# letitiabanana/PnP-OVSS

Hardware: AMD Instinct MI355X
Metric: images/sec (336^2, drop_iter=4, blur+CRF) (higher is better)
Workload: dtype bf16x3

## Files before the change

### pnp-ovss_amd/csrc/engine.hip

```cpp
#include <hip/hip_runtime.h>

#include <cmath>
#include <cstdarg>
#include <cstring>
#include <map>
#include <memory>
#include <string>
#include <utility>
#include <vector>

#include "../../include/pnp_hip.h"
#include "common.h"
#include "kernels.h"

using namespace pnp;

namespace {

struct Buf {
    void* p = nullptr;
    size_t bytes = 0;
};

struct Weight {
    void* p = nullptr;
    int rows = 0, cols = 0;
    int esz = 0;
    bool pair = false;
    void* hi(int r0 = 0) const { return (char*)p + (size_t)r0 * cols * esz; }
    void* lo(int r0 = 0) const { return pair ? (char*)p + ((size_t)rows + r0) * cols * esz : nullptr; }
};

struct Act {
    void* hi = nullptr;
    void* lo = nullptr;
};

struct TextLayerW {
    Weight qkv_w, so_w, cq_w, co_w, i_w, o_w;
    float *qkv_b = nullptr, *so_b = nullptr, *sln_w = nullptr, *sln_b = nullptr, *cq_b = nullptr, *co_b = nullptr,
          *cln_w = nullptr, *cln_b = nullptr, *i_b = nullptr, *o_b = nullptr, *oln_w = nullptr, *oln_b = nullptr;
    Weight o_wT, i_wT, co_wT, cq_wT, so_wT, qkv_wT;
};

struct TextLayerA {
    void* qkv = nullptr;
    float* Ps = nullptr;
    float *a_hat = nullptr, *a_rstd = nullptr, *a_out = nullptr;
    void* a_outT = nullptr;
    void* qc = nullptr;
    float* Pc = nullptr;
    float *c_hat = nullptr, *c_rstd = nullptr, *c_out = nullptr;
    void* c_outT = nullptr;
    float* u = nullptr;
    float *o_hat = nullptr, *o_rstd = nullptr, *h_out = nullptr;
    void* h_outT = nullptr;
};

struct VitLayerW {
    float *n1w, *n1b, *n2w, *n2b, *qkv_b, *proj_b, *fc1_b, *fc2_b;
    Weight qkv_w, proj_w, fc1_w, fc2_w;
};

struct WeightStore {
    int device = 0;
    std::vector<void*> allocs;
    size_t bytes = 0;
    ~WeightStore() {
        (void)hipSetDevice(device);
        for (void* p : allocs) (void)hipFree(p);
    }
};

}

struct pnp_engine {
    pnp_config c{};
    std::shared_ptr<WeightStore> wstore;
    bool to_store = false;
    bool shares_weights = false;
    int bf = 0;
    int x3 = 0;
    size_t esz = 4;
    int P = 0, PP = 0, N = 0, Npad = 0, D = 0, H = 0, I = 0, TL = 0, nh = 0, Nst = 0, SL = 0;
    char err[512] = {0};
    std::vector<void*> allocs;
    size_t alloc_bytes = 0;
    std::map<std::string, Buf> named;
    std::map<std::string, bool> loaded;
    bool finalized = false;

    float *cls = nullptr, *pos = nullptr, *patch_b = nullptr, *vnorm_w = nullptr, *vnorm_b = nullptr;
    Weight patch_w;
    std::vector<VitLayerW> vit;
    float *word = nullptr, *tpos = nullptr, *eln_w = nullptr, *eln_b = nullptr, *itm_w = nullptr, *itm_b = nullptr;
    std::vector<TextLayerW> txt;
    Weight proj_w[2];
    float* proj_b[2] = {nullptr, nullptr};
    int proj_E[2] = {0, 0};
    Weight ck_w, cv_w;
    float *ck_b = nullptr, *cv_b = nullptr;
    std::vector<Buf> staging;

    int ldq = 0;
    float* x0 = nullptr;
    struct { const float* images = nullptr; const int64_t* ids = nullptr; const int64_t* mask = nullptr; int B = 0, L = 0, ld = 0;
             bool vit = false, text = false; } reuse;
    void *patches = nullptr, *vt = nullptr;
    Act xn, qk, ctx, h1, embT;
    float *x = nullptr, *emb32 = nullptr;
    void *Knat = nullptr, *Vnat = nullptr, *Kt = nullptr, *Vt = nullptr;
    std::vector<TextLayerA> ta;
    float *temb = nullptr, *h0 = nullptr, *tmp = nullptr;
    void *h0T = nullptr, *ctx_s = nullptr, *ctx_c = nullptr, *g = nullptr;
    float *dh = nullptr, *d_pre = nullptr, *dc = nullptr, *d_cpre = nullptr, *da = nullptr, *d_apre = nullptr,
          *dctx_s = nullptr, *dS = nullptr, *dPc = nullptr;
    void *d_preT = nullptr, *dg = nullptr, *d_cpreT = nullptr, *dctxc = nullptr, *dqc = nullptr, *d_apreT = nullptr,
         *dqkv = nullptr;
    int grad_layer = -1;
    bool acts_text_only = false;
    float* G = nullptr;
    uint8_t* dropped = nullptr;
    float* logits_scratch = nullptr;

    struct Post {
        bool reserved = false, prepared = false, has_crf = false;
        int groups_cap = 1;
        int maxB = 0, maxK = 0, max_pix_img = 0, chunk = 0;
        int64_t max_total_pix = 0;
        int B = 0, Cmax = 0, Kmax = 0, maxHW = 0;
        int64_t total_pix = 0;
        std::vector<PostDesc> desc, desc_pair;
        PostDesc* d_desc = nullptr;
        PostDesc* d_desc_pair = nullptr;
        int32_t *d_img_cls_off = nullptr, *d_cls_off = nullptr, *d_tok_idx = nullptr, *d_cls_div = nullptr, *d_lut = nullptr;
        int lut_stride = 0;
        size_t* d_label_off = nullptr;
        double* d_wts = nullptr;
        int32_t* d_wt_off = nullptr;
        float *merged = nullptr, *thr = nullptr, *maps = nullptr, *maps2 = nullptr, *maps3 = nullptr, *stats = nullptr;
        float *unary = nullptr, *Q = nullptr, *va = nullptr, *vb = nullptr, *vga = nullptr, *vgb = nullptr, *norm[2] = {nullptr, nullptr};
        int Kpmax = 0, Kpmax_pair = 0, maxH = 0, maxW = 0, max_radius = 0, maxKp = 0;
        size_t valg_cap = 0;
        std::vector<int> gauss_sig;
        const uint8_t* d_rgb = nullptr;
        const float* d_gt = nullptr;
        CrfLattice lat[2]{};
        uint64_t *keys_a = nullptr, *keys_b = nullptr;
        uint32_t* vals_a = nullptr;
        int *n1k = nullptr, *n2k = nullptr;
        int *head = nullptr, *incl = nullptr, *range_err = nullptr;
        int range_err_host = 0;
        int lat_points[2] = {0, 0};
        std::vector<size_t> h_label_off;
        std::vector<int32_t> h_wt_off;
        std::vector<double> h_wts;
        void* sort_tmp = nullptr;
        size_t sort_tmp_bytes = 0;
        size_t cap[2] = {0, 0};
        size_t val_cap = 0;
        int lut_cap = 0, cls_cap = 0, tok_cap = 0, wts_cap = 0;
        bool maps_in_2 = false;
    } post;

    GemmProfile* gemm_prof = nullptr;
    StreamKWs sk_ws;
    struct StageProfile {
        bool on = false;
        std::vector<hipEvent_t> ev0, ev1;
        int used = 0;
        long long launches = 0;
        double work = 0;
        double lattice = 0;
    } crf_prof;
};

namespace {

int fail(pnp_engine* e, int code, const char* fmt, ...) {
    va_list ap;
    va_start(ap, fmt);
    vsnprintf(e->err, sizeof(e->err), fmt, ap);
    va_end(ap);
    return code;
}

#define HIPCHK(e, call)                                                                      \
    do {                                                                                     \
        hipError_t _s = (call);                                                              \
        if (_s != hipSuccess) return fail(e, PNP_ERR_HIP, "%s: %s", #call, hipGetErrorString(_s)); \
    } while (0)
#define KCHK(e, call)                                                         \
    do {                                                                      \
        int _r = (call);                                                      \
        if (_r != PNP_OK) return fail(e, _r, "%s failed (%d): %s", #call, _r, hipGetErrorString(hipGetLastError())); \
    } while (0)

template <typename T>
int dalloc(pnp_engine* e, T** out, size_t count, bool zero = false) {
    void* p = nullptr;
    const size_t bytes = (count * sizeof(T) + 255) / 256 * 256;
    if (hipMalloc(&p, bytes ? bytes : 256) != hipSuccess) return fail(e, PNP_ERR_NOMEM, "hipMalloc(%zu) failed", bytes);
    if (zero && hipMemset(p, 0, bytes ? bytes : 256) != hipSuccess) return fail(e, PNP_ERR_HIP, "hipMemset failed");
    if (e->to_store && e->wstore) {
        e->wstore->allocs.push_back(p);
        e->wstore->bytes += bytes;
    } else {
        e->allocs.push_back(p);
    }
    e->alloc_bytes += bytes;
    *out = reinterpret_cast<T*>(p);
    return PNP_OK;
}
int dalloc_t(pnp_engine* e, void** out, size_t count, bool zero = false) {
    char* p = nullptr;
    int r = dalloc<char>(e, &p, count * e->esz, zero);
    *out = p;
    return r;
}
int alloc_act(pnp_engine* e, Act* a, size_t rows, size_t ld) {
    KCHK(e, dalloc_t(e, &a->hi, rows * ld));
    a->lo = e->x3 ? (char*)a->hi + rows * ld * 2 : nullptr;
    return PNP_OK;
}
int launched() { return hipPeekAtLastError() == hipSuccess ? PNP_OK : PNP_ERR_HIP; }

bool ends_with(const std::string& s, const char* suf) {
    const size_t n = strlen(suf);
    return s.size() >= n && s.compare(s.size() - n, n, suf) == 0;
}

__global__ void transpose_cast_kernel_f32(const float* __restrict__ in, float* __restrict__ out, int rows, int cols) {
    __shared__ float t[32][33];
    const int bx = blockIdx.x * 32, by = blockIdx.y * 32;
    for (int i = threadIdx.y; i < 32; i += 8) {
        const int r = by + i, c = bx + threadIdx.x;
        t[i][threadIdx.x] = (r < rows && c < cols) ? in[(size_t)r * cols + c] : 0.f;
    }
    __syncthreads();
    for (int i = threadIdx.y; i < 32; i += 8) {
        const int c = bx + i, r = by + threadIdx.x;
        if (r < rows && c < cols) out[(size_t)c * rows + r] = t[threadIdx.x][i];
    }
}

__global__ void feat_to_tok_kernel(const float* __restrict__ src, int ld_src, int n_pad, float* __restrict__ dst, int R, int N) {
    __shared__ float t[32][33];
    const int b = blockIdx.z, r0 = blockIdx.x * 32, t0 = blockIdx.y * 32;
    for (int i = threadIdx.y; i < 32; i += 8) {
        const int r = r0 + i, tok = t0 + threadIdx.x;
        t[i][threadIdx.x] = (r < R && tok < N) ? src[(size_t)r * ld_src + (size_t)b * n_pad + tok] : 0.f;
    }
    __syncthreads();
    for (int i = threadIdx.y; i < 32; i += 8) {
        const int tok = t0 + i, r = r0 + threadIdx.x;
        if (r < R && tok < N) dst[((size_t)b * N + tok) * R + r] = t[threadIdx.x][i];
    }
}
__global__ void tok_to_feat_kernel(const float* __restrict__ src, int ld_src, float* __restrict__ dst, int ld_dst, int n_pad, int R, int N) {
    __shared__ float t[32][33];
    const int b = blockIdx.z, r0 = blockIdx.x * 32, t0 = blockIdx.y * 32;
    for (int i = threadIdx.y; i < 32; i += 8) {
        const int tok = t0 + i, r = r0 + threadIdx.x;
        t[i][threadIdx.x] = (r < R && tok < N) ? src[((size_t)b * N + tok) * ld_src + r] : 0.f;
    }
    __syncthreads();
    for (int i = threadIdx.y; i < 32; i += 8) {
        const int r = r0 + i, tok = t0 + threadIdx.x;
        if (r < R && tok < N) dst[(size_t)r * ld_dst + (size_t)b * n_pad + tok] = t[threadIdx.x][i];
    }
}

__global__ void embed_reuse_kernel(const float* __restrict__ x0, const uint8_t* __restrict__ dropped, const float* __restrict__ bias,
                                   const float* __restrict__ pos, float* __restrict__ x, int rows, int N, int D4) {
    const size_t total = (size_t)rows * D4;
    for (size_t i = (size_t)blockIdx.x * blockDim.x + threadIdx.x; i < total; i += (size_t)gridDim.x * blockDim.x) {
        const int m = (int)(i / D4), c = (int)(i - (size_t)m * D4);
        const int b = m / N, t = m - b * N;
        f32x4 v;
        if (t > 0 && dropped[(size_t)b * (N - 1) + (t - 1)]) {
            const f32x4 bv = reinterpret_cast<const f32x4*>(bias)[c];
            const f32x4 pv = reinterpret_cast<const f32x4*>(pos)[(size_t)t * D4 + c];
#pragma unroll
            for (int e = 0; e < 4; e++) v[e] = __fadd_rn(__fadd_rn(0.0f, bv[e]), pv[e]);
        } else {
            v = reinterpret_cast<const f32x4*>(x0)[i];
        }
        reinterpret_cast<f32x4*>(x)[i] = v;
    }
}

int new_weight(pnp_engine* e, int rows, int cols, bool pair, Weight* w) {
    *w = Weight{nullptr, rows, cols, pair ? 2 : (int)e->esz, pair};
    return dalloc_t(e, &w->p, (size_t)rows * cols);
}
int fill_weight(pnp_engine* e, const float* src32, const Weight& w, int r0, int n) {
    const size_t count = (size_t)n * w.cols;
    return w.pair ? split_f32(src32, w.hi(r0), w.lo(r0), count, 0) : cast_f32(e->bf, src32, w.hi(r0), count, 0);
}
int make_weight(pnp_engine* e, const float* src32, int rows, int cols, bool transpose, Weight* out, bool pair = false) {
    KCHK(e, new_weight(e, transpose ? cols : rows, transpose ? rows : cols, pair, out));
    const float* s = src32;
    float* tmp = nullptr;
    if (transpose) {
        HIPCHK(e, hipMalloc((void**)&tmp, (size_t)rows * cols * 4));
        hipLaunchKernelGGL(transpose_cast_kernel_f32, dim3((cols + 31) / 32, (rows + 31) / 32), dim3(32, 8), 0, 0, src32, tmp,
                           rows, cols);
        s = tmp;
    }
    int r = transpose ? launched() : PNP_OK;
    if (r == PNP_OK) r = fill_weight(e, s, *out, 0, out->rows);
    hipError_t st = hipDeviceSynchronize();
    if (tmp) (void)hipFree(tmp);
    if (r != PNP_OK || st != hipSuccess) return fail(e, PNP_ERR_HIP, "weight conversion failed");
    return PNP_OK;
}

GemmArgs G_(const void* A, int lda, const void* B, int ldb, int M, int N, int K) {
    GemmArgs g;
    g.A = A; g.lda = lda; g.B = B; g.ldb = ldb; g.M = M; g.N = N; g.K = K;
    return g;
}

GemmArgs linear(const void* a, int lda, const Weight& w, int M, int r0 = 0, int n = 0) {
    GemmArgs g = G_(a, lda, w.hi(r0), w.cols, M, n ? n : w.rows, w.cols);
    g.B_lo = w.lo(r0);
    g.a_f32 = w.pair;
    return g;
}
GemmArgs linear(const Act& a, int lda, const Weight& w, int M, int r0 = 0, int n = 0) {
    GemmArgs g = linear(a.hi, lda, w, M, r0, n);
    g.A_lo = a.lo;
    g.a_f32 = w.pair && !a.lo;
    return g;
}
GemmArgs linear_t(const Act& a, int lda, const Weight& w, int M, int r0 = 0, int n = 0) {
    GemmArgs g = linear(a, lda, w, M, r0, n);
    std::swap(g.A, g.B); std::swap(g.A_lo, g.B_lo); std::swap(g.lda, g.ldb); std::swap(g.M, g.N);
    return g;
}

int egemm(pnp_engine* e, GemmArgs g, hipStream_t s) {
    g.prof = e->gemm_prof;
    g.sk = e->sk_ws.part ? &e->sk_ws : nullptr;
    return gemm_nt(e->bf, g, s);
}

}


extern "C" size_t pnp_workspace_bytes(const pnp_config* c) {
    if (!c) return 0;
    const size_t es = c->compute_bf16 == 1 ? 2 : 4;
    const size_t P = c->img_size / c->patch, N = P * P + 1, Npad = (N + 63) / 64 * 64, D = c->vit_dim, H = c->txt_hidden,
                 I = c->txt_inter, TL = c->txt_layers, B = c->max_batch, L = c->max_text_len;
    const size_t M = B * N, R = B * L;
    size_t w = (size_t)c->vit_depth * (12 * D * D) * es + TL * (4 * H * H + 2 * H * D + 2 * H * I) * es * 2 +
               ((size_t)c->vocab + c->max_pos) * H * 4 + 256 * (D + H) * es + 2 * 256 * 4;
    size_t a = M * (768 + D * 2 + 3 * D + 64 + D + 4 * D) * es + M * D * 12 + D * B * Npad * es + M * TL * H * es * 2 +
               2 * TL * H * B * Npad * es;
    size_t t = TL * (R * (3 * H + 2 * H) * es + R * (H * 8 + I) * 4 + B * (H / 64) * L * (L + Npad) * 4) + R * I * (4 + es) * 2 +
               R * H * 64;
    return w + a + t + (64u << 20);
}

extern "C" const char* pnp_last_error(const pnp_engine* e) { return e ? e->err : "null engine"; }

extern "C" void pnp_destroy(pnp_engine* e) {
    if (!e) return;
    (void)hipSetDevice(e->c.device);
    (void)hipDeviceSynchronize();
    for (void* p : e->allocs) (void)hipFree(p);
    for (auto& b : e->staging) if (b.p) (void)hipFree(b.p);
    if (e->gemm_prof) {
        for (int i = 0; i < e->gemm_prof->created; i++) {
            (void)hipEventDestroy(e->gemm_prof->ev0[i]);
            (void)hipEventDestroy(e->gemm_prof->ev1[i]);
        }
        delete e->gemm_prof;
    }
    for (hipEvent_t ev : e->crf_prof.ev0) (void)hipEventDestroy(ev);
    for (hipEvent_t ev : e->crf_prof.ev1) (void)hipEventDestroy(ev);
    streamk_ws_destroy(&e->sk_ws);
    delete e;
}

static int create_impl(const pnp_config* cfg, pnp_engine* donor, pnp_engine** out) {
    if (!cfg || !out) return PNP_ERR_ARG;
    pnp_engine* e = new pnp_engine();
    *out = e;
    e->c = *cfg;
    if (donor) {
        const pnp_config& d = donor->c;
        if (!donor->finalized) return fail(e, PNP_ERR_STATE, "pnp_create_shared: the donor's weights are not finalized");
        if (d.device != cfg->device || d.compute_bf16 != cfg->compute_bf16 || d.img_size != cfg->img_size || d.patch != cfg->patch ||
            d.vit_dim != cfg->vit_dim || d.vit_depth != cfg->vit_depth || d.vit_heads != cfg->vit_heads ||
            d.vit_mlp_ratio != cfg->vit_mlp_ratio || d.txt_hidden != cfg->txt_hidden || d.txt_layers != cfg->txt_layers ||
            d.txt_heads != cfg->txt_heads || d.txt_inter != cfg->txt_inter || d.vocab != cfg->vocab || d.max_pos != cfg->max_pos ||
            d.vit_ln_eps != cfg->vit_ln_eps || d.txt_ln_eps != cfg->txt_ln_eps)
            return fail(e, PNP_ERR_ARG, "pnp_create_shared: device, compute mode and model geometry must equal the donor's");
        if (cfg->stash_layer < d.stash_layer)
            return fail(e, PNP_ERR_ARG, "pnp_create_shared: stash_layer %d below the donor's %d (its transposed backward weights "
                        "exist for layers >= %d only)", cfg->stash_layer, d.stash_layer, d.stash_layer);
    }
    const pnp_config& c = e->c;
    if (c.compute_bf16 < 0 || c.compute_bf16 > 2) return fail(e, PNP_ERR_ARG, "compute_bf16 must be 0 (fp32), 1 (bf16) or 2 (split-bf16)");
    e->bf = c.compute_bf16 == 1 ? 1 : 0;
    e->x3 = c.compute_bf16 == 2 ? 1 : 0;
    e->esz = e->bf ? 2 : 4;
    if (c.patch != 16) return fail(e, PNP_ERR_ARG, "patch must be 16");
    if (c.img_size % 16 || c.img_size <= 0) return fail(e, PNP_ERR_ARG, "img_size must be a positive multiple of 16");
    if (c.vit_dim != c.vit_heads * 64 || c.txt_hidden != c.txt_heads * 64)
        return fail(e, PNP_ERR_ARG, "head_dim must be 64 (vit_dim=%d heads=%d, txt_hidden=%d heads=%d)", c.vit_dim,
                    c.vit_heads, c.txt_hidden, c.txt_heads);
    if (c.vit_dim % 128 || c.txt_hidden % 128 || c.txt_inter % 128 || (c.vit_dim * c.vit_mlp_ratio) % 128)
        return fail(e, PNP_ERR_ARG, "widths must be multiples of 128");
    if (c.vit_dim > 1024 || c.txt_hidden > 1024) return fail(e, PNP_ERR_ARG, "LayerNorm width > 1024 unsupported");
    if (c.max_text_len < 5 || c.max_text_len > 512 || c.max_text_len > c.max_pos)
        return fail(e, PNP_ERR_ARG, "max_text_len must be in [5, min(512, max_pos = %d)]", c.max_pos);
    if (c.stash_layer < 0 || c.stash_layer >= c.txt_layers) return fail(e, PNP_ERR_ARG, "stash_layer out of range");
    if (c.max_batch <= 0) return fail(e, PNP_ERR_ARG, "max_batch must be positive");
    HIPCHK(e, hipSetDevice(c.device));
    e->P = c.img_size / 16;
    e->PP = e->P * e->P;
    e->N = e->PP + 1;
    e->Npad = (e->N + 63) / 64 * 64;
    e->Nst = e->Npad;
    e->D = c.vit_dim;
    e->H = c.txt_hidden;
    e->I = c.txt_inter;
    e->TL = c.txt_layers;
    e->nh = c.txt_heads;
    e->SL = c.stash_layer;
    if ((e->N + 15) / 16 > 160) return fail(e, PNP_ERR_ARG, "too many image tokens (%d) for the cross-attention kernel", e->N);
    const size_t B = c.max_batch, M = B * e->N, D = e->D, H = e->H, I = e->I, L = c.max_text_len, R = B * L, TL = e->TL;
    const size_t ldv = B * e->Npad;
    e->vit.resize(c.vit_depth);
    e->txt.resize(TL);
    e->ta.resize(TL);
    if (e->x3) {
        const int n_cu = device_cu_count();
        if (!n_cu || streamk_ws_create(&e->sk_ws, n_cu) != PNP_OK) return fail(e, PNP_ERR_HIP, "stream-K workspace allocation failed");
        e->alloc_bytes += (size_t)n_cu * 256 * 256 * 4;
    }
    KCHK(e, dalloc_t(e, &e->patches, B * e->PP * 768));
    KCHK(e, dalloc(e, &e->x, M * D));
    KCHK(e, dalloc(e, &e->x0, M * D));
    KCHK(e, alloc_act(e, &e->xn, M, D));
    e->ldq = 3 * (int)D + 64;
    KCHK(e, alloc_act(e, &e->qk, M, e->ldq));
    KCHK(e, dalloc_t(e, &e->vt, D * ldv, true));
    KCHK(e, alloc_act(e, &e->ctx, M, D));
    KCHK(e, alloc_act(e, &e->h1, M, D * c.vit_mlp_ratio));
    KCHK(e, alloc_act(e, &e->embT, M, D));
    KCHK(e, dalloc(e, &e->emb32, M * D));
    const int nVn = e->TL - e->SL, nKt = e->TL - e->SL - 1;
    KCHK(e, dalloc_t(e, &e->Knat, M * TL * H));
    KCHK(e, dalloc_t(e, &e->Vnat, M * (size_t)nVn * H));
    KCHK(e, dalloc_t(e, &e->Vt, TL * H * ldv, true));
    if (nKt > 0) KCHK(e, dalloc_t(e, &e->Kt, (size_t)nKt * H * ldv, true));
    KCHK(e, dalloc(e, &e->temb, R * H));
    KCHK(e, dalloc(e, &e->h0, R * H));
    KCHK(e, dalloc_t(e, &e->h0T, R * H));
    KCHK(e, dalloc(e, &e->tmp, R * H));
    KCHK(e, dalloc_t(e, &e->ctx_s, R * H));
    KCHK(e, dalloc_t(e, &e->ctx_c, R * H));
    KCHK(e, dalloc_t(e, &e->g, R * I));
    for (size_t i = 0; i < TL; i++) {
        TextLayerA& a = e->ta[i];
        KCHK(e, dalloc_t(e, &a.qkv, R * 3 * H));
        KCHK(e, dalloc(e, &a.a_hat, R * H));
        KCHK(e, dalloc(e, &a.a_rstd, R));
        KCHK(e, dalloc(e, &a.a_out, R * H));
        KCHK(e, dalloc_t(e, &a.a_outT, R * H));
        KCHK(e, dalloc_t(e, &a.qc, R * H));
        KCHK(e, dalloc(e, &a.c_hat, R * H));
        KCHK(e, dalloc(e, &a.c_rstd, R));
        KCHK(e, dalloc(e, &a.c_out, R * H));
        KCHK(e, dalloc_t(e, &a.c_outT, R * H));
        KCHK(e, dalloc(e, &a.u, R * I));
        KCHK(e, dalloc(e, &a.o_hat, R * H));
        KCHK(e, dalloc(e, &a.o_rstd, R));
        KCHK(e, dalloc(e, &a.h_out, R * H));
        KCHK(e, dalloc_t(e, &a.h_outT, R * H));
        if ((int)i >= e->SL) {
            KCHK(e, dalloc(e, &a.Ps, B * e->nh * L * L));
            KCHK(e, dalloc(e, &a.Pc, B * e->nh * L * (size_t)e->Nst, true));
        }
    }
    KCHK(e, dalloc(e, &e->dh, R * H));
    KCHK(e, dalloc(e, &e->d_pre, R * H));
    KCHK(e, dalloc_t(e, &e->d_preT, R * H));
    KCHK(e, dalloc_t(e, &e->dg, R * I));
    KCHK(e, dalloc(e, &e->dc, R * H));
    KCHK(e, dalloc(e, &e->d_cpre, R * H));
    KCHK(e, dalloc_t(e, &e->d_cpreT, R * H));
    KCHK(e, dalloc_t(e, &e->dctxc, R * H));
    KCHK(e, dalloc_t(e, &e->dqc, R * H));
    KCHK(e, dalloc(e, &e->da, R * H));
    KCHK(e, dalloc(e, &e->d_apre, R * H));
    KCHK(e, dalloc_t(e, &e->d_apreT, R * H));
    KCHK(e, dalloc(e, &e->dctx_s, R * H));
    KCHK(e, dalloc(e, &e->dS, B * e->nh * L * L));
    KCHK(e, dalloc(e, &e->dPc, B * e->nh * L * (size_t)e->Nst, true));
    KCHK(e, dalloc_t(e, &e->dqkv, R * 3 * H));
    KCHK(e, dalloc(e, &e->G, B * L * (size_t)e->PP));
    KCHK(e, dalloc(e, &e->dropped, B * (size_t)e->PP, true));
    KCHK(e, dalloc(e, &e->logits_scratch, B * 2));
    if (donor) {
        e->wstore = donor->wstore;
        e->shares_weights = true;
        e->cls = donor->cls; e->pos = donor->pos; e->patch_b = donor->patch_b; e->vnorm_w = donor->vnorm_w; e->vnorm_b = donor->vnorm_b;
        e->word = donor->word; e->tpos = donor->tpos; e->eln_w = donor->eln_w; e->eln_b = donor->eln_b;
        e->itm_w = donor->itm_w; e->itm_b = donor->itm_b; e->ck_b = donor->ck_b; e->cv_b = donor->cv_b;
        e->patch_w = donor->patch_w; e->ck_w = donor->ck_w; e->cv_w = donor->cv_w;
        e->vit = donor->vit;
        e->txt = donor->txt;
        for (int i = 0; i < 2; i++) { e->proj_w[i] = donor->proj_w[i]; e->proj_b[i] = donor->proj_b[i]; e->proj_E[i] = donor->proj_E[i]; }
        e->finalized = true;
        return PNP_OK;
    }
    e->wstore = std::make_shared<WeightStore>();
    e->wstore->device = c.device;
    e->to_store = true;
    KCHK(e, dalloc(e, &e->cls, D));
    KCHK(e, dalloc(e, &e->pos, (size_t)e->N * D));
    KCHK(e, dalloc(e, &e->patch_b, D));
    KCHK(e, dalloc(e, &e->vnorm_w, D));
    KCHK(e, dalloc(e, &e->vnorm_b, D));
    KCHK(e, dalloc(e, &e->word, (size_t)c.vocab * H));
    KCHK(e, dalloc(e, &e->tpos, (size_t)c.max_pos * H));
    KCHK(e, dalloc(e, &e->eln_w, H));
    KCHK(e, dalloc(e, &e->eln_b, H));
    KCHK(e, dalloc(e, &e->itm_w, 2 * H));
    KCHK(e, dalloc(e, &e->itm_b, 2));
    KCHK(e, dalloc(e, &e->ck_b, TL * H));
    KCHK(e, dalloc(e, &e->cv_b, TL * H));
    for (auto& v : e->vit) {
        KCHK(e, dalloc(e, &v.n1w, D)); KCHK(e, dalloc(e, &v.n1b, D)); KCHK(e, dalloc(e, &v.n2w, D)); KCHK(e, dalloc(e, &v.n2b, D));
        KCHK(e, dalloc(e, &v.qkv_b, 3 * D)); KCHK(e, dalloc(e, &v.proj_b, D));
        KCHK(e, dalloc(e, &v.fc1_b, D * c.vit_mlp_ratio)); KCHK(e, dalloc(e, &v.fc2_b, D));
    }
    for (auto& t : e->txt) {
        KCHK(e, dalloc(e, &t.qkv_b, 3 * H)); KCHK(e, dalloc(e, &t.so_b, H)); KCHK(e, dalloc(e, &t.sln_w, H)); KCHK(e, dalloc(e, &t.sln_b, H));
        KCHK(e, dalloc(e, &t.cq_b, H)); KCHK(e, dalloc(e, &t.co_b, H)); KCHK(e, dalloc(e, &t.cln_w, H)); KCHK(e, dalloc(e, &t.cln_b, H));
        KCHK(e, dalloc(e, &t.i_b, I)); KCHK(e, dalloc(e, &t.o_b, H)); KCHK(e, dalloc(e, &t.oln_w, H)); KCHK(e, dalloc(e, &t.oln_b, H));
    }
    e->to_store = false;
    return PNP_OK;
}
extern "C" int pnp_create(const pnp_config* cfg, pnp_engine** out) { return create_impl(cfg, nullptr, out); }
extern "C" int pnp_create_shared(const pnp_config* cfg, pnp_engine* donor, pnp_engine** out) {
    if (!donor) return PNP_ERR_ARG;
    return create_impl(cfg, donor, out);
}


namespace {

struct Key {
    const char* name = "";
    float* small = nullptr;
    size_t small_off = 0;
    int rows = 1, cols = 0;
    int id = 0;
};
Key small(const char* name, float* p, int count, size_t off = 0) { return {name, p, off, 1, count, 0}; }
Key gemm(const char* name, int id, int rows, int cols) { return {name, nullptr, 0, rows, cols, id}; }

enum { W_PATCH };
enum { W_QKV, W_PROJ, W_FC1, W_FC2 };
enum { W_Q, W_K, W_V, W_SO, W_CQ, W_CK, W_CV, W_CO, W_I, W_O, W_MAX };

std::vector<Key> top_keys(pnp_engine* e) {
    const int D = e->D, H = e->H;
    return {small("visual_encoder.cls_token", e->cls, D),
            small("visual_encoder.pos_embed", e->pos, e->N * D),
            gemm("visual_encoder.patch_embed.proj.weight", W_PATCH, D, 768),
            small("visual_encoder.patch_embed.proj.bias", e->patch_b, D),
            small("visual_encoder.norm.weight", e->vnorm_w, D),
            small("visual_encoder.norm.bias", e->vnorm_b, D),
            small("text_encoder.embeddings.word_embeddings.weight", e->word, e->c.vocab * H),
            small("text_encoder.embeddings.position_embeddings.weight", e->tpos, e->c.max_pos * H),
            small("text_encoder.embeddings.LayerNorm.weight", e->eln_w, H),
            small("text_encoder.embeddings.LayerNorm.bias", e->eln_b, H),
            small("itm_head.weight", e->itm_w, 2 * H),
            small("itm_head.bias", e->itm_b, 2)};
}
const char* const kVitPrefix = "visual_encoder.blocks.";
std::vector<Key> vit_keys(pnp_engine* e, int li) {
    VitLayerW& v = e->vit[li];
    const int D = e->D, F = D * e->c.vit_mlp_ratio;
    return {small("norm1.weight", v.n1w, D),       small("norm1.bias", v.n1b, D),
            gemm("attn.qkv.weight", W_QKV, 3 * D, D),   small("attn.qkv.bias", v.qkv_b, 3 * D),
            gemm("attn.proj.weight", W_PROJ, D, D),     small("attn.proj.bias", v.proj_b, D),
            small("norm2.weight", v.n2w, D),       small("norm2.bias", v.n2b, D),
            gemm("mlp.fc1.weight", W_FC1, F, D),        small("mlp.fc1.bias", v.fc1_b, F),
            gemm("mlp.fc2.weight", W_FC2, D, F),        small("mlp.fc2.bias", v.fc2_b, D)};
}
const char* const kTextPrefix = "text_encoder.encoder.layer.";
std::vector<Key> text_keys(pnp_engine* e, int li) {
    TextLayerW& t = e->txt[li];
    const int D = e->D, H = e->H, I = e->I;
    const size_t l = (size_t)li * H;
    return {gemm("attention.self.query.weight", W_Q, H, H),            small("attention.self.query.bias", t.qkv_b, H, 0),
            gemm("attention.self.key.weight", W_K, H, H),              small("attention.self.key.bias", t.qkv_b, H, H),
            gemm("attention.self.value.weight", W_V, H, H),            small("attention.self.value.bias", t.qkv_b, H, 2 * H),
            gemm("attention.output.dense.weight", W_SO, H, H),         small("attention.output.dense.bias", t.so_b, H),
            small("attention.output.LayerNorm.weight", t.sln_w, H),    small("attention.output.LayerNorm.bias", t.sln_b, H),
            gemm("crossattention.self.query.weight", W_CQ, H, H),      small("crossattention.self.query.bias", t.cq_b, H),
            gemm("crossattention.self.key.weight", W_CK, H, D),        small("crossattention.self.key.bias", e->ck_b, H, l),
            gemm("crossattention.self.value.weight", W_CV, H, D),      small("crossattention.self.value.bias", e->cv_b, H, l),
            gemm("crossattention.output.dense.weight", W_CO, H, H),    small("crossattention.output.dense.bias", t.co_b, H),
            small("crossattention.output.LayerNorm.weight", t.cln_w, H), small("crossattention.output.LayerNorm.bias", t.cln_b, H),
            gemm("intermediate.dense.weight", W_I, I, H),              small("intermediate.dense.bias", t.i_b, I),
            gemm("output.dense.weight", W_O, H, I),                    small("output.dense.bias", t.o_b, H),
            small("output.LayerNorm.weight", t.oln_w, H),              small("output.LayerNorm.bias", t.oln_b, H)};
}

bool find_key(const std::vector<Key>& keys, const char* name, Key& out) {
    for (const Key& k : keys)
        if (!strcmp(k.name, name)) {
            out = k;
            return true;
        }
    return false;
}

bool resolve(pnp_engine* e, const std::string& n, Key& s) {
    int li = -1;
    char rest[128];
    auto layer_of = [&](const char* prefix, int depth) {
        const size_t len = strlen(prefix);
        return n.compare(0, len, prefix) == 0 && sscanf(n.c_str() + len, "%d.%127s", &li, rest) == 2 && li >= 0 && li < depth;
    };
    if (layer_of(kVitPrefix, e->c.vit_depth)) return find_key(vit_keys(e, li), rest, s);
    if (layer_of(kTextPrefix, e->TL)) return find_key(text_keys(e, li), rest, s);
    return find_key(top_keys(e), n.c_str(), s);
}

const char* const kProj[2] = {"vision_proj", "text_proj"};
int resolve_proj(pnp_engine* e, const std::string& n, const int64_t* shape, int ndim, Key& s) {
    int which = -1;
    bool bias = false;
    for (int i = 0; i < 2; i++) {
        if (n == std::string(kProj[i]) + ".weight") which = i;
        if (n == std::string(kProj[i]) + ".bias") which = i, bias = true;
    }
    if (which < 0) return 0;
    const int K = which == 0 ? e->D : e->H;
    if (ndim != (bias ? 1 : 2) || (!bias && shape[1] != K))
        return fail(e, PNP_ERR_ARG, "%s: expected %s, second dimension %d", n.c_str(), bias ? "a vector" : "a matrix", K);
    const int64_t E = shape[0];
    if (E <= 0 || E > 1024 || E % 64) return fail(e, PNP_ERR_ARG, "%s: embedding width %lld must be a multiple of 64 up to 1024", n.c_str(), (long long)E);
    if (e->proj_E[which] && e->proj_E[which] != (int)E)
        return fail(e, PNP_ERR_ARG, "%s: %lld rows, but the other tensor of this projection has %d", n.c_str(), (long long)E, e->proj_E[which]);
    e->proj_E[which] = (int)E;
    s.rows = (int)E;
    s.cols = bias ? 1 : K;
    return 1;
}

const float* staged(pnp_engine* e, const std::string& n) {
    auto it = e->named.find("stage:" + n);
    return it == e->named.end() ? nullptr : (const float*)it->second.p;
}

int collect(pnp_engine* e, const std::string& prefix, const std::vector<Key>& keys, const float** st) {
    for (const Key& k : keys) {
        const std::string n = prefix + k.name;
        if (k.small ? !e->loaded.count(n) : !(st[k.id] = staged(e, n))) return fail(e, PNP_ERR_STATE, "missing weight %s", n.c_str());
    }
    return PNP_OK;
}

}

extern "C" int pnp_load_weight(pnp_engine* e, const char* name, const float* data, const int64_t* shape, int32_t ndim,
                               int32_t on_device) {
    if (!e || !name || !data || !shape) return PNP_ERR_ARG;
    if (e->shares_weights) return fail(e, PNP_ERR_STATE, "this engine uses a donor's weights (pnp_create_shared)");
    if (e->finalized) return fail(e, PNP_ERR_STATE, "weights already finalized");
    HIPCHK(e, hipSetDevice(e->c.device));
    Key s;
    const int pj = resolve_proj(e, name, shape, ndim, s);
    if (pj < 0) return pj;
    if (!pj && !resolve(e, name, s)) return PNP_OK;
    size_t count = 1;
    for (int i = 0; i < ndim; i++) count *= (size_t)shape[i];
    if (count != (size_t)s.rows * s.cols) return fail(e, PNP_ERR_ARG, "%s: expected %d elements, got %zu", name, s.rows * s.cols, count);
    const hipMemcpyKind kind = on_device ? hipMemcpyDeviceToDevice : hipMemcpyHostToDevice;
    if (s.small) {
        HIPCHK(e, hipMemcpy(s.small + s.small_off, data, count * 4, kind));
    } else {
        Buf b;
        b.bytes = count * 4;
        HIPCHK(e, hipMalloc(&b.p, b.bytes));
        HIPCHK(e, hipMemcpy(b.p, data, b.bytes, kind));
        e->staging.push_back(b);
        e->named[std::string("stage:") + name] = b;
    }
    e->loaded[name] = true;
    return PNP_OK;
}

extern "C" int pnp_finalize_weights(pnp_engine* e) {
    if (!e) return PNP_ERR_ARG;
    if (e->finalized) return PNP_OK;
    HIPCHK(e, hipSetDevice(e->c.device));
    e->to_store = true;
    struct StoreOff { pnp_engine* e; ~StoreOff() { e->to_store = false; } } store_off{e};
    const int D = e->D, H = e->H, I = e->I, TL = e->TL, F = D * e->c.vit_mlp_ratio;
    const float* st[W_MAX];
    if (int r = collect(e, "", top_keys(e), st)) return r;
    KCHK(e, make_weight(e, st[W_PATCH], D, 768, false, &e->patch_w));
    for (int i = 0; i < e->c.vit_depth; i++) {
        VitLayerW& v = e->vit[i];
        if (int r = collect(e, kVitPrefix + std::to_string(i) + ".", vit_keys(e, i), st)) return r;
        KCHK(e, make_weight(e, st[W_QKV], 3 * D, D, false, &v.qkv_w, e->x3));
        KCHK(e, make_weight(e, st[W_PROJ], D, D, false, &v.proj_w, e->x3));
        KCHK(e, make_weight(e, st[W_FC1], F, D, false, &v.fc1_w, e->x3));
        KCHK(e, make_weight(e, st[W_FC2], D, F, false, &v.fc2_w, e->x3));
    }
    KCHK(e, new_weight(e, TL * H, D, e->x3, &e->ck_w));
    KCHK(e, new_weight(e, TL * H, D, e->x3, &e->cv_w));
    for (int i = 0; i < TL; i++) {
        TextLayerW& t = e->txt[i];
        if (int r = collect(e, kTextPrefix + std::to_string(i) + ".", text_keys(e, i), st)) return r;
        float* fused = nullptr;
        HIPCHK(e, hipMalloc((void**)&fused, (size_t)3 * H * H * 4));
        HIPCHK(e, hipMemcpy(fused, st[W_Q], (size_t)H * H * 4, hipMemcpyDeviceToDevice));
        HIPCHK(e, hipMemcpy(fused + (size_t)H * H, st[W_K], (size_t)H * H * 4, hipMemcpyDeviceToDevice));
        HIPCHK(e, hipMemcpy(fused + (size_t)2 * H * H, st[W_V], (size_t)H * H * 4, hipMemcpyDeviceToDevice));
        int r = make_weight(e, fused, 3 * H, H, false, &t.qkv_w, e->x3);
        if (r == PNP_OK && i > e->SL) r = make_weight(e, fused, 3 * H, H, true, &t.qkv_wT, e->x3);
        (void)hipFree(fused);
        if (r != PNP_OK) return r;
        KCHK(e, make_weight(e, st[W_SO], H, H, false, &t.so_w, e->x3));
        KCHK(e, make_weight(e, st[W_CQ], H, H, false, &t.cq_w, e->x3));
        KCHK(e, make_weight(e, st[W_CO], H, H, false, &t.co_w, e->x3));
        KCHK(e, make_weight(e, st[W_I], I, H, false, &t.i_w, e->x3));
        KCHK(e, make_weight(e, st[W_O], H, I, false, &t.o_w, e->x3));
        KCHK(e, fill_weight(e, st[W_CK], e->ck_w, i * H, H));
        KCHK(e, fill_weight(e, st[W_CV], e->cv_w, i * H, H));
        if (i >= e->SL) {
            KCHK(e, make_weight(e, st[W_O], H, I, true, &t.o_wT, e->x3));
            KCHK(e, make_weight(e, st[W_I], I, H, true, &t.i_wT, e->x3));
            KCHK(e, make_weight(e, st[W_CO], H, H, true, &t.co_wT, e->x3));
        }
        if (i > e->SL) {
            KCHK(e, make_weight(e, st[W_CQ], H, H, true, &t.cq_wT, e->x3));
            KCHK(e, make_weight(e, st[W_SO], H, H, true, &t.so_wT, e->x3));
        }
    }
    for (int i = 0; i < 2; i++) {
        const float *w = staged(e, std::string(kProj[i]) + ".weight"), *bs = staged(e, std::string(kProj[i]) + ".bias");
        if (!w || !bs) {
            e->proj_E[i] = 0;
            continue;
        }
        KCHK(e, make_weight(e, w, e->proj_E[i], i == 0 ? D : H, false, &e->proj_w[i], e->x3));
        KCHK(e, dalloc(e, &e->proj_b[i], (size_t)e->proj_E[i]));
        HIPCHK(e, hipMemcpy(e->proj_b[i], bs, (size_t)e->proj_E[i] * 4, hipMemcpyDeviceToDevice));
    }
    HIPCHK(e, hipDeviceSynchronize());
    for (auto& b : e->staging) if (b.p) (void)hipFree(b.p);
    e->staging.clear();
    for (auto it = e->named.begin(); it != e->named.end();) {
        if (it->first.rfind("stage:", 0) == 0) it = e->named.erase(it);
        else ++it;
    }
    e->finalized = true;
    return PNP_OK;
}


static int vit_forward_impl(pnp_engine* e, const float* d_images, const uint8_t* d_dropped, int32_t B, void* stream, int embed) {
    if (!e || !d_images) return PNP_ERR_ARG;
    if (!e->finalized) return fail(e, PNP_ERR_STATE, "weights not finalized");
    if (B <= 0 || B > e->c.max_batch) return fail(e, PNP_ERR_ARG, "batch %d out of range (max %d)", B, e->c.max_batch);
    hipStream_t s = (hipStream_t)stream;
    const int D = e->D, N = e->N, M = B * N, F = D * e->c.vit_mlp_ratio, bf = e->bf;
    const int ldv = e->c.max_batch * e->Npad;
    if (embed == 2 && !(e->reuse.vit && e->reuse.images == d_images && e->reuse.B == B)) embed = 0;
    if (embed == 2 && d_dropped) {
        hipLaunchKernelGGL(embed_reuse_kernel, dim3(2048), dim3(256), 0, s, (const float*)e->x0, d_dropped, (const float*)e->patch_b,
                           (const float*)e->pos, e->x, M, N, D / 4);
        KCHK(e, launched());
    } else {
        KCHK(e, patchify(bf, d_images, d_dropped, e->patches, B, e->c.img_size, e->P, s));
        KCHK(e, cls_rows(e->cls, e->pos, e->x, B, N, D, s));
        {
            GemmArgs g = linear(e->patches, 768, e->patch_w, B * e->PP);
            g.bias = e->patch_b; g.resid = e->pos; g.ldr = D; g.out_f32 = e->x; g.ldo = D; g.row_div = e->PP;
            KCHK(e, egemm(e, g, s));
        }
        if (embed == 1) {
            HIPCHK(e, hipMemcpyAsync(e->x0, e->x, (size_t)M * D * sizeof(float), hipMemcpyDeviceToDevice, s));
            e->reuse.images = d_images;
            e->reuse.B = B;
            e->reuse.vit = true;
        }
    }
    const float scale = 1.0f / sqrtf(64.f);
    const int ln = bf | e->x3;
    for (int l = 0; l < e->c.vit_depth; l++) {
        const VitLayerW& w = e->vit[l];
        KCHK(e, layernorm(ln, e->x, w.n1w, w.n1b, e->c.vit_ln_eps, M, D, nullptr, e->xn.hi, nullptr, nullptr, s, e->xn.lo));
        if (bf || e->x3) {
            GemmArgs g = linear(e->xn, D, w.qkv_w, M);
            g.bias = w.qkv_b; g.out_t = e->qk.hi; g.out_lo = e->qk.lo; g.ldo_t = e->ldq;
            KCHK(e, egemm(e, g, s));
            if (e->x3)
                KCHK(e, vit_attention_x3(e->qk.hi, e->qk.lo, e->ldq, D, e->ctx.hi, e->ctx.lo, B, e->c.vit_heads, N, scale, s));
            else
                KCHK(e, vit_attention(bf, e->qk.hi, e->ldq, D, (const char*)e->qk.hi + (size_t)2 * D * e->esz, e->ldq, e->Npad, e->ctx.hi,
                                      B, e->c.vit_heads, N, scale, s));
        } else {
            {
                GemmArgs g = linear(e->xn, D, w.qkv_w, M, 0, 2 * D);
                g.bias = w.qkv_b; g.out_t = e->qk.hi; g.ldo_t = 2 * D;
                KCHK(e, egemm(e, g, s));
            }
            {
                GemmArgs g = linear_t(e->xn, D, w.qkv_w, M, 2 * D, D);
                g.bias = w.qkv_b + 2 * D; g.bias_on_rows = 1; g.out_t = e->vt; g.ldo_t = ldv; g.col_div = N; g.col_pad = e->Npad;
                KCHK(e, egemm(e, g, s));
            }
            KCHK(e, vit_attention(bf, e->qk.hi, 2 * D, D, e->vt, ldv, e->Npad, e->ctx.hi, B, e->c.vit_heads, N, scale, s));
        }
        {
            GemmArgs g = linear(e->ctx, D, w.proj_w, M);
            g.bias = w.proj_b; g.resid = e->x; g.ldr = D; g.out_f32 = e->x; g.ldo = D;
            KCHK(e, egemm(e, g, s));
        }
        KCHK(e, layernorm(ln, e->x, w.n2w, w.n2b, e->c.vit_ln_eps, M, D, nullptr, e->xn.hi, nullptr, nullptr, s, e->xn.lo));
        {
            GemmArgs g = linear(e->xn, D, w.fc1_w, M);
            g.bias = w.fc1_b; g.mode = GEMM_EPI_GELU; g.out_t = e->h1.hi; g.out_lo = e->h1.lo; g.ldo_t = F;
            KCHK(e, egemm(e, g, s));
        }
        {
            GemmArgs g = linear(e->h1, F, w.fc2_w, M);
            g.bias = w.fc2_b; g.resid = e->x; g.ldr = D; g.out_f32 = e->x; g.ldo = D;
            KCHK(e, egemm(e, g, s));
        }
    }
    KCHK(e, layernorm(ln, e->x, e->vnorm_w, e->vnorm_b, e->c.vit_ln_eps, M, D, e->emb32, e->embT.hi, nullptr, nullptr, s, e->embT.lo));
    return pnp_cross_kv(e, B, stream);
}
extern "C" int pnp_vit_forward(pnp_engine* e, const float* d_images, const uint8_t* d_dropped, int32_t B, void* stream) {
    if (e) e->reuse.vit = false;
    return vit_forward_impl(e, d_images, d_dropped, B, stream, 0);
}

extern "C" int pnp_cross_kv(pnp_engine* e, int32_t B, void* stream) {
    if (!e) return PNP_ERR_ARG;
    if (!e->finalized) return fail(e, PNP_ERR_STATE, "weights not finalized");
    if (B <= 0 || B > e->c.max_batch) return fail(e, PNP_ERR_ARG, "batch %d out of range (max %d)", B, e->c.max_batch);
    hipStream_t s = (hipStream_t)stream;
    const int D = e->D, N = e->N, M = B * N;
    const int ldv = e->c.max_batch * e->Npad;
    const int H = e->H, TL = e->TL, SL = e->SL, nVn = TL - SL, nKt = TL - SL - 1;
    auto out = [&](GemmArgs& g, void* p, int ld) {
        if (e->x3) { g.out_f32 = (float*)p; g.ldo = ld; }
        else { g.out_t = p; g.ldo_t = ld; }
    };
    {
        GemmArgs g = linear(e->embT, D, e->ck_w, M);
        g.bias = e->ck_b; out(g, e->Knat, TL * H);
        KCHK(e, egemm(e, g, s));
    }
    {
        GemmArgs g = linear_t(e->embT, D, e->cv_w, M);
        g.bias = e->cv_b; g.bias_on_rows = 1; out(g, e->Vt, ldv); g.col_div = N; g.col_pad = e->Npad;
        KCHK(e, egemm(e, g, s));
    }
    if (e->x3) {
        hipLaunchKernelGGL(feat_to_tok_kernel, dim3((nVn * H + 31) / 32, (N + 31) / 32, B), dim3(32, 8), 0, s,
                           (const float*)e->Vt + (size_t)SL * H * ldv, ldv, e->Npad, (float*)e->Vnat, nVn * H, N);
        KCHK(e, launched());
        if (nKt > 0) {
            hipLaunchKernelGGL(tok_to_feat_kernel, dim3((nKt * H + 31) / 32, (N + 31) / 32, B), dim3(32, 8), 0, s,
                               (const float*)e->Knat + (size_t)(SL + 1) * H, TL * H, (float*)e->Kt, ldv, e->Npad, nKt * H, N);
            KCHK(e, launched());
        }
        return PNP_OK;
    }
    {
        GemmArgs g = linear(e->embT, D, e->cv_w, M, SL * H, nVn * H);
        g.bias = e->cv_b + (size_t)SL * H; g.out_t = e->Vnat; g.ldo_t = nVn * H;
        KCHK(e, egemm(e, g, s));
    }
    if (nKt > 0) {
        GemmArgs g = linear_t(e->embT, D, e->ck_w, M, (SL + 1) * H, nKt * H);
        g.bias = e->ck_b + (size_t)(SL + 1) * H; g.bias_on_rows = 1; g.out_t = e->Kt; g.ldo_t = ldv; g.col_div = N; g.col_pad = e->Npad;
        KCHK(e, egemm(e, g, s));
    }
    return PNP_OK;
}

static int text_layer(pnp_engine* e, int i, const int64_t* d_mask, int32_t ld, int32_t B, int32_t L, bool cross, bool self_in_place,
                      hipStream_t s) {
    const int H = e->H, I = e->I, TL = e->TL, R = B * L, bf = e->bf, N = e->N;
    const int ldv = e->c.max_batch * e->Npad;
    const TextLayerW& w = e->txt[i];
    TextLayerA& a = e->ta[i];
    const float* h = i ? e->ta[i - 1].h_out : e->h0;
    const void* hT = i ? e->ta[i - 1].h_outT : e->h0T;
    const bool keep_p = cross && i >= e->SL;
    auto keep = [&](float* p) -> float* { return cross ? p : nullptr; };
    if (!self_in_place) {
        {
            GemmArgs g = linear(hT, H, w.qkv_w, R);
            g.bias = w.qkv_b; g.out_t = a.qkv; g.ldo_t = 3 * H;
            KCHK(e, egemm(e, g, s));
        }
        KCHK(e, text_self_attn(bf, a.qkv, d_mask, ld, e->ctx_s, keep_p ? a.Ps : nullptr, e->dS, B, L, H, s));
        {
            GemmArgs g = linear(e->ctx_s, H, w.so_w, R);
            g.bias = w.so_b; g.resid = h; g.ldr = H; g.out_f32 = e->tmp; g.ldo = H;
            KCHK(e, egemm(e, g, s));
        }
        KCHK(e, layernorm(bf, e->tmp, w.sln_w, w.sln_b, e->c.txt_ln_eps, R, H, a.a_out, a.a_outT, keep(a.a_hat), keep(a.a_rstd), s));
    }
    const float* f = a.a_out;
    const void* fT = a.a_outT;
    if (cross) {
        {
            GemmArgs g = linear(a.a_outT, H, w.cq_w, R);
            g.bias = w.cq_b; g.out_t = a.qc; g.ldo_t = H;
            KCHK(e, egemm(e, g, s));
        }
        KCHK(e, xattn(bf, 0, (const char*)e->Knat + (size_t)i * H * e->esz, TL * H,
                      (const char*)e->Vt + (size_t)i * H * ldv * e->esz, ldv, e->Npad, a.qc, H, e->ctx_c, H,
                      keep_p ? a.Pc : nullptr, e->Nst, B, L, N, e->nh, s));
        {
            GemmArgs g = linear(e->ctx_c, H, w.co_w, R);
            g.bias = w.co_b; g.resid = a.a_out; g.ldr = H; g.out_f32 = e->tmp; g.ldo = H;
            KCHK(e, egemm(e, g, s));
        }
        KCHK(e, layernorm(bf, e->tmp, w.cln_w, w.cln_b, e->c.txt_ln_eps, R, H, a.c_out, a.c_outT, a.c_hat, a.c_rstd, s));
        f = a.c_out;
        fT = a.c_outT;
    }
    {
        GemmArgs g = linear(fT, H, w.i_w, R);
        g.bias = w.i_b; g.mode = GEMM_EPI_GELU; g.out_t = e->g; g.ldo_t = I;
        if (cross) { g.aux = a.u; g.ld_aux = I; }
        KCHK(e, egemm(e, g, s));
    }
    {
        GemmArgs g = linear(e->g, I, w.o_w, R);
        g.bias = w.o_b; g.resid = f; g.ldr = H; g.out_f32 = e->tmp; g.ldo = H;
        KCHK(e, egemm(e, g, s));
    }
    KCHK(e, layernorm(bf, e->tmp, w.oln_w, w.oln_b, e->c.txt_ln_eps, R, H, a.h_out, a.h_outT, keep(a.o_hat), keep(a.o_rstd), s));
    return PNP_OK;
}

static int text_forward_impl(pnp_engine* e, const int64_t* d_ids, const int64_t* d_mask, int32_t ld, int32_t B, int32_t L,
                             float* d_logits, void* stream, bool reuse_prefix) {
    if (!e || !d_ids || !d_mask) return PNP_ERR_ARG;
    if (!e->finalized) return fail(e, PNP_ERR_STATE, "weights not finalized");
    if (B <= 0 || B > e->c.max_batch || L < 5 || L > e->c.max_text_len || ld < L)
        return fail(e, PNP_ERR_ARG, "text batch %d x %d (ld %d) out of range (max %d x %d)", B, L, ld, e->c.max_batch, e->c.max_text_len);
    hipStream_t s = (hipStream_t)stream;
    const int H = e->H, TL = e->TL, R = B * L;
    e->acts_text_only = false;
    if (reuse_prefix && !(e->reuse.text && e->reuse.ids == d_ids && e->reuse.mask == d_mask && e->reuse.B == B && e->reuse.L == L &&
                          e->reuse.ld == ld))
        reuse_prefix = false;
    if (!reuse_prefix) {
        KCHK(e, text_embed(d_ids, ld, e->word, e->tpos, e->temb, B, L, H, e->c.enc_token_id, e->c.vocab, s));
        KCHK(e, layernorm(e->bf, e->temb, e->eln_w, e->eln_b, e->c.txt_ln_eps, R, H, e->h0, e->h0T, nullptr, nullptr, s));
    }
    for (int i = 0; i < TL; i++) {
        int r = text_layer(e, i, d_mask, ld, B, L, true, reuse_prefix && i == 0, s);
        if (r) return r;
    }
    KCHK(e, itm_head(e->ta[TL - 1].h_out, e->itm_w, e->itm_b, d_logits ? d_logits : e->logits_scratch, B, L, H, s));
    return PNP_OK;
}
extern "C" int pnp_text_forward_xattn(pnp_engine* e, const int64_t* d_ids, const int64_t* d_mask, int32_t ld, int32_t B,
                                      int32_t L, float* d_logits, void* stream) {
    if (e) e->reuse.text = false;
    return text_forward_impl(e, d_ids, d_mask, ld, B, L, d_logits, stream, false);
}

extern "C" int pnp_text_forward_text(pnp_engine* e, const int64_t* d_ids, const int64_t* d_mask, int32_t ld, int32_t T, int32_t L,
                                     float* d_hidden, void* stream) {
    if (!e || !d_ids || !d_mask) return PNP_ERR_ARG;
    if (T <= 0 || L < 2 || L > e->c.max_text_len || ld < L)
        return fail(e, PNP_ERR_ARG, "text batch %d x %d (ld %d) out of range (2 <= L <= %d, T > 0)", T, L, ld, e->c.max_text_len);
    if (!e->finalized) return fail(e, PNP_ERR_STATE, "weights not finalized");
    hipStream_t s = (hipStream_t)stream;
    const int H = e->H, TL = e->TL;
    e->reuse.text = false;
    e->grad_layer = -1;
    e->acts_text_only = true;
    for (int t0 = 0; t0 < T; t0 += e->c.max_batch) {
        const int B = T - t0 < e->c.max_batch ? T - t0 : e->c.max_batch, R = B * L;
        const int64_t* ids = d_ids + (size_t)t0 * ld;
        const int64_t* mask = d_mask + (size_t)t0 * ld;
        KCHK(e, text_embed(ids, ld, e->word, e->tpos, e->temb, B, L, H, -1, e->c.vocab, s));
        KCHK(e, layernorm(e->bf, e->temb, e->eln_w, e->eln_b, e->c.txt_ln_eps, R, H, e->h0, e->h0T, nullptr, nullptr, s));
        for (int i = 0; i < TL; i++) {
            int r = text_layer(e, i, mask, ld, B, L, false, false, s);
            if (r) return r;
        }
        if (d_hidden)
            HIPCHK(e, hipMemcpyAsync(d_hidden + (size_t)t0 * L * H, e->ta[TL - 1].h_out, (size_t)R * H * sizeof(float),
                                     hipMemcpyDeviceToDevice, s));
    }
    return PNP_OK;
}

extern "C" int pnp_project_normalize(pnp_engine* e, int32_t which, const float* d_x, int64_t row_stride, int32_t rows, float* d_out,
                                     void* stream) {
    if (!e || !d_x || !d_out) return PNP_ERR_ARG;
    if (which < 0 || which > 1) return fail(e, PNP_ERR_ARG, "which = %d: 0 (vision_proj) or 1 (text_proj)", which);
    if (rows <= 0) return fail(e, PNP_ERR_ARG, "rows = %d", rows);
    const int K = which == 0 ? e->D : e->H;
    if (row_stride < K || row_stride % 4 || row_stride > (int64_t)1 << 30)
        return fail(e, PNP_ERR_ARG, "row_stride %lld: a multiple of 4 elements, at least %d", (long long)row_stride, K);
    if ((int64_t)rows * row_stride * 4 >= (int64_t)1 << 32)
        return fail(e, PNP_ERR_ARG, "rows %d x row_stride %lld: the input must span less than 4 GiB", rows, (long long)row_stride);
    if (!e->finalized) return fail(e, PNP_ERR_STATE, "weights not finalized");
    const Weight& w = e->proj_w[which];
    if (!w.p || !e->proj_b[which])
        return fail(e, PNP_ERR_STATE, "missing weight %s.weight (the state dict held no %s.weight / .bias)", kProj[which], kProj[which]);
    hipStream_t s = (hipStream_t)stream;
    const int E = e->proj_E[which];
    if (e->bf) {
        size_t cap = (size_t)e->c.max_batch * e->N * e->D / K;
        cap = cap < 16384 ? cap : 16384;
        for (size_t r0 = 0; r0 < (size_t)rows; r0 += cap) {
            const int n = (int)((size_t)rows - r0 < cap ? (size_t)rows - r0 : cap);
            KCHK(e, cast_rows_bf16(d_x + r0 * row_stride, (int)row_stride, e->xn.hi, n, K, s));
            GemmArgs g = linear(e->xn.hi, K, w, n);
            g.bias = e->proj_b[which]; g.out_f32 = d_out + r0 * E; g.ldo = E;
            KCHK(e, egemm(e, g, s));
        }
    } else {
        GemmArgs g = linear(d_x, (int)row_stride, w, rows);
        g.bias = e->proj_b[which]; g.out_f32 = d_out; g.ldo = E;
        KCHK(e, egemm(e, g, s));
    }
    KCHK(e, l2_normalize_rows(d_out, rows, E, 1e-12f, s));
    return PNP_OK;
}

extern "C" int pnp_itc_similarity(const float* d_img_feat, const float* d_txt_feat, int32_t B, int32_t T, int32_t E, float* d_sim,
                                  void* stream) {
    if (!d_img_feat || !d_txt_feat || !d_sim || B <= 0 || T <= 0 || E <= 0 || E % 4) return PNP_ERR_ARG;
    return itc_similarity(d_img_feat, d_txt_feat, d_sim, B, T, E, (hipStream_t)stream);
}

extern "C" int pnp_xattn_grad(pnp_engine* e, int32_t B, int32_t L, void* stream) {
    return pnp_xattn_grad_layer(e, B, L, e ? e->SL : 0, stream);
}

extern "C" int pnp_xattn_grad_layer(pnp_engine* e, int32_t B, int32_t L, int32_t layer, void* stream) {
    if (!e) return PNP_ERR_ARG;
    if (!e->finalized) return fail(e, PNP_ERR_STATE, "weights not finalized");
    if (B <= 0 || B > e->c.max_batch || L < 5 || L > e->c.max_text_len) return fail(e, PNP_ERR_ARG, "bad B/L");
    if (layer < e->SL || layer >= e->TL)
        return fail(e, PNP_ERR_ARG, "layer %d: cross-attention maps are kept for text layers %d..%d (stash_layer)", layer, e->SL, e->TL - 1);
    if (e->acts_text_only)
        return fail(e, PNP_ERR_STATE, "the text activations in place are those of pnp_text_forward_text: run pnp_text_forward_xattn first");
    hipStream_t s = (hipStream_t)stream;
    const int H = e->H, I = e->I, TL = e->TL, R = B * L, bf = e->bf, N = e->N, SL = e->SL;
    const int ldv = e->c.max_batch * e->Npad, nVn = TL - SL;
    e->grad_layer = layer;
    KCHK(e, itm_grad_seed(e->itm_w, e->dh, B, L, H, s));
    for (int i = TL - 1; i >= layer; i--) {
        const TextLayerW& w = e->txt[i];
        TextLayerA& a = e->ta[i];
        KCHK(e, layernorm_bwd(bf, e->dh, w.oln_w, a.o_hat, a.o_rstd, R, H, e->d_pre, e->d_preT, s));
        {
            GemmArgs g = linear(e->d_preT, H, w.o_wT, R);
            g.mode = GEMM_EPI_GELU_GRAD; g.aux = a.u; g.ld_aux = I; g.out_t = e->dg; g.ldo_t = I;
            KCHK(e, egemm(e, g, s));
        }
        {
            GemmArgs g = linear(e->dg, I, w.i_wT, R);
            g.resid = e->d_pre; g.ldr = H; g.out_f32 = e->dc; g.ldo = H;
            KCHK(e, egemm(e, g, s));
        }
        KCHK(e, layernorm_bwd(bf, e->dc, w.cln_w, a.c_hat, a.c_rstd, R, H, e->d_cpre, e->d_cpreT, s));
        {
            GemmArgs g = linear(e->d_cpreT, H, w.co_wT, R);
            g.out_t = e->dctxc; g.ldo_t = H;
            KCHK(e, egemm(e, g, s));
        }
        const char* vnat = (const char*)e->Vnat + (size_t)(i - SL) * H * e->esz;
        if (i == layer) {
            KCHK(e, xattn(bf, 2, vnat, nVn * H, nullptr, 0, e->Npad, e->dctxc, H, nullptr, 0, e->dPc, e->Nst, B, L, N, e->nh, s));
            break;
        }
        KCHK(e, xattn(bf, 1, vnat, nVn * H, (const char*)e->Kt + (size_t)(i - SL - 1) * H * ldv * e->esz, ldv, e->Npad,
                      e->dctxc, H, e->dqc, H, a.Pc, e->Nst, B, L, N, e->nh, s));
        {
            GemmArgs g = linear(e->dqc, H, w.cq_wT, R);
            g.resid = e->d_cpre; g.ldr = H; g.out_f32 = e->da; g.ldo = H;
            KCHK(e, egemm(e, g, s));
        }
        KCHK(e, layernorm_bwd(bf, e->da, w.sln_w, a.a_hat, a.a_rstd, R, H, e->d_apre, e->d_apreT, s));
        {
            GemmArgs g = linear(e->d_apreT, H, w.so_wT, R);
            g.out_f32 = e->dctx_s; g.ldo = H;
            KCHK(e, egemm(e, g, s));
        }
        KCHK(e, text_self_attn_bwd(bf, a.qkv, e->dctx_s, a.Ps, e->dS, e->dqkv, B, L, H, s));
        {
            GemmArgs g = linear(e->dqkv, 3 * H, w.qkv_wT, R);
            g.resid = e->d_apre; g.ldr = H; g.out_f32 = e->dh; g.ldo = H;
            KCHK(e, egemm(e, g, s));
        }
    }
    return PNP_OK;
}

extern "C" int pnp_gradcam_gather(pnp_engine* e, const int64_t* d_mask, int32_t ld, int32_t B, int32_t L, int32_t head,
                                  float* d_out, void* stream) {
    if (!e || !d_mask || !d_out) return PNP_ERR_ARG;
    if (head < 0 || head >= e->nh) return fail(e, PNP_ERR_ARG, "head %d out of range", head);
    if (B <= 0 || B > e->c.max_batch || L < 5 || L > e->c.max_text_len || ld < L) return fail(e, PNP_ERR_ARG, "bad B/L/ld");
    if (e->grad_layer < 0) return fail(e, PNP_ERR_STATE, "call pnp_xattn_grad first");
    KCHK(e, gradcam_gather(e->ta[e->grad_layer].Pc, e->dPc, d_mask, ld, d_out, B, e->nh, head, L, e->Nst, e->PP, (hipStream_t)stream));
    return PNP_OK;
}

static int compute_gradcam_impl(pnp_engine* e, const float* d_images, const uint8_t* d_dropped, const int64_t* d_ids,
                                const int64_t* d_mask, int32_t ld, int32_t B, int32_t L, int32_t layer, int32_t head,
                                float* d_out, float* d_logits, void* stream, int embed) {
    int r = vit_forward_impl(e, d_images, d_dropped, B, stream, embed);
    if (r) return r;
    r = text_forward_impl(e, d_ids, d_mask, ld, B, L, d_logits, stream, embed == 2);
    if (r) return r;
    if (embed == 1) {
        e->reuse.ids = d_ids; e->reuse.mask = d_mask; e->reuse.L = L; e->reuse.ld = ld;
        e->reuse.text = true;
    } else if (embed == 0) {
        e->reuse.text = false;
    }
    r = pnp_xattn_grad_layer(e, B, L, layer, stream);
    if (r) return r;
    return pnp_gradcam_gather(e, d_mask, ld, B, L, head, d_out, stream);
}
extern "C" int pnp_compute_gradcam_layer(pnp_engine* e, const float* d_images, const uint8_t* d_dropped, const int64_t* d_ids,
                                         const int64_t* d_mask, int32_t ld, int32_t B, int32_t L, int32_t layer, int32_t head,
                                         float* d_out, float* d_logits, void* stream) {
    return compute_gradcam_impl(e, d_images, d_dropped, d_ids, d_mask, ld, B, L, layer, head, d_out, d_logits, stream, 0);
}

extern "C" int pnp_compute_gradcam(pnp_engine* e, const float* d_images, const uint8_t* d_dropped, const int64_t* d_ids,
                                   const int64_t* d_mask, int32_t ld, int32_t B, int32_t L, int32_t head, float* d_out,
                                   float* d_logits, void* stream) {
    return pnp_compute_gradcam_layer(e, d_images, d_dropped, d_ids, d_mask, ld, B, L, e ? e->SL : 0, head, d_out, d_logits, stream);
}

extern "C" int pnp_drop_step(pnp_engine* e, const float* d_gradcam, float* d_g0, float* d_agg, uint8_t* d_dropped,
                             int32_t* d_picks, int32_t iter, int32_t B, int32_t T, int32_t npick, int32_t max_picks,
                             void* stream) {
    if (!e || !d_gradcam || !d_agg || !d_dropped || (npick > 0 && !d_picks)) return PNP_ERR_ARG;
    if (T < 4) return fail(e, PNP_ERR_ARG, "T=%d too short", T);
    KCHK(e, drop_step(d_gradcam, d_g0, d_agg, d_dropped, d_picks, iter, B, T, e->PP, npick, max_picks, (hipStream_t)stream));
    return PNP_OK;
}

extern "C" int pnp_drop_loop(pnp_engine* e, const float* d_images, const int64_t* d_ids, const int64_t* d_mask, int32_t ld,
                             int32_t B, int32_t L, int32_t head, int32_t drop_iter, int32_t npick, float* d_g0,
                             float* d_agg, int32_t* d_picks, float* d_logits, void* stream) {
    return pnp_drop_loop_layer(e, d_images, d_ids, d_mask, ld, B, L, e ? e->SL : 0, head, drop_iter, npick, d_g0, d_agg, d_picks,
                               d_logits, stream);
}

extern "C" int pnp_drop_loop_layer(pnp_engine* e, const float* d_images, const int64_t* d_ids, const int64_t* d_mask, int32_t ld,
                                   int32_t B, int32_t L, int32_t layer, int32_t head, int32_t drop_iter, int32_t npick, float* d_g0,
                                   float* d_agg, int32_t* d_picks, float* d_logits, void* stream) {
    if (!e || !d_images || !d_ids || !d_mask || !d_g0) return PNP_ERR_ARG;
    if (drop_iter < 1) return fail(e, PNP_ERR_ARG, "drop_iter must be >= 1");
    if (drop_iter == 1)
        return pnp_compute_gradcam_layer(e, d_images, nullptr, d_ids, d_mask, ld, B, L, layer, head, d_g0, d_logits, stream);
    if (!d_agg || !d_picks) return PNP_ERR_ARG;
    hipStream_t s = (hipStream_t)stream;
    HIPCHK(e, hipMemsetAsync(e->dropped, 0, (size_t)B * e->PP, s));
    for (int it = 0; it < drop_iter; it++) {
        int r = compute_gradcam_impl(e, d_images, e->dropped, d_ids, d_mask, ld, B, L, layer, head, e->G, d_logits, stream, it == 0 ? 1 : 2);
        if (r) return r;
        r = pnp_drop_step(e, e->G, d_g0, d_agg, e->dropped, d_picks, it, B, L - 1, npick, drop_iter * npick, stream);
        if (r) return r;
    }
    return PNP_OK;
}


extern "C" int pnp_post_reserve(pnp_engine* e, int32_t max_batch, int64_t max_total_pixels, int32_t max_pixels_per_image,
                                int32_t max_channels, int32_t crf_chunk) {
    if (!e) return PNP_ERR_ARG;
    if (e->post.reserved) return fail(e, PNP_ERR_STATE, "post-process workspace already reserved");
    if (max_batch <= 0 || max_batch > 64 || max_total_pixels <= 0 || max_pixels_per_image <= 0 || max_channels <= 0 ||
        max_channels > 255)
        return fail(e, PNP_ERR_ARG, "bad post-process bounds (at most 64 images per batch, 255 channels)");
    HIPCHK(e, hipSetDevice(e->c.device));
    auto& p = e->post;
    p.maxB = max_batch;
    p.max_total_pix = max_total_pixels;
    p.max_pix_img = max_pixels_per_image;
    p.maxK = max_channels;
    p.chunk = crf_chunk > 0 ? crf_chunk : max_batch;
    const size_t TP = (size_t)max_total_pixels, K = max_channels, B = max_batch;
    KCHK(e, dalloc(e, &p.d_desc, B));
    KCHK(e, dalloc(e, &p.d_desc_pair, B));
    KCHK(e, dalloc(e, &p.d_img_cls_off, B + 1));
    p.cls_cap = (int)(B * K + 1);
    p.tok_cap = (int)(B * e->c.max_text_len + 1);
    KCHK(e, dalloc(e, &p.d_cls_off, p.cls_cap + 1));
    KCHK(e, dalloc(e, &p.d_cls_div, p.cls_cap));
    KCHK(e, dalloc(e, &p.d_tok_idx, p.tok_cap));
    p.lut_cap = (int)(B * (K + 1));
    KCHK(e, dalloc(e, &p.d_lut, p.lut_cap));
    KCHK(e, dalloc(e, &p.d_label_off, B + 1));
    p.wts_cap = (int)(B * 4096);
    KCHK(e, dalloc(e, &p.d_wts, p.wts_cap));
    KCHK(e, dalloc(e, &p.d_wt_off, B + 1));
    KCHK(e, dalloc(e, &p.merged, B * K * e->PP));
    KCHK(e, dalloc(e, &p.thr, B * K * e->PP));
    KCHK(e, dalloc(e, &p.maps, TP * K));
    KCHK(e, dalloc(e, &p.maps2, TP * K));
    KCHK(e, dalloc(e, &p.maps3, TP * K));
    KCHK(e, dalloc(e, &p.stats, B * K * 2));
    const size_t Kp = (K + 3) / 4 * 4;
    p.maxKp = (int)Kp;
    {
        const size_t chunk_pix0 = (size_t)std::min<int64_t>((int64_t)(crf_chunk > 0 ? crf_chunk : B) * max_pixels_per_image, max_total_pixels);
        const size_t single = (2 * TP * Kp + 2 * chunk_pix0 * 6 * Kp + 2 * chunk_pix0 * 3 * Kp) * sizeof(float);
        size_t free_b = 0, total_b = 0;
        if (hipMemGetInfo(&free_b, &total_b) != hipSuccess) free_b = (size_t)96 << 30;
        p.groups_cap = 2 * single <= free_b / 3 ? 2 : 1;
    }
    const size_t G2 = (size_t)p.groups_cap;
    KCHK(e, dalloc(e, &p.unary, TP * Kp * G2));
    KCHK(e, dalloc(e, &p.Q, TP * Kp * G2));
    KCHK(e, dalloc(e, &p.norm[0], TP));
    KCHK(e, dalloc(e, &p.norm[1], TP));
    for (int t = 0; t < 2; t++) {
        const int D1 = t == 0 ? 3 : 6;
        const size_t cap = TP * D1;
        p.cap[t] = cap;
        CrfLattice& L = p.lat[t];
        L.D1 = D1;
        L.which = t;
        L.cap = cap;
        KCHK(e, dalloc(e, &L.bary, cap));
        KCHK(e, dalloc(e, &L.vals, cap));
        KCHK(e, dalloc(e, &L.ent, cap));
        KCHK(e, dalloc(e, &L.offset, cap));
        KCHK(e, dalloc(e, &L.seg_start, cap + 1));
        KCHK(e, dalloc(e, &L.seg_lo, cap));
        KCHK(e, dalloc(e, &L.seg_hi, cap));
        KCHK(e, dalloc(e, &L.ukeys, cap));
        KCHK(e, dalloc(e, &L.idbase, B + 1));
        KCHK(e, dalloc(e, &L.n1, cap * D1));
        KCHK(e, dalloc(e, &L.n2, cap * D1));
        KCHK(e, dalloc(e, &L.nbr8, cap * (D1 / 2)));
    }
    const size_t cap6 = p.cap[1];
    KCHK(e, dalloc(e, &p.keys_a, cap6));
    KCHK(e, dalloc(e, &p.keys_b, cap6));
    KCHK(e, dalloc(e, &p.vals_a, cap6));
    KCHK(e, dalloc(e, &p.head, cap6));
    KCHK(e, dalloc(e, &p.incl, cap6));
    KCHK(e, dalloc(e, &p.n1k, cap6 * 6));
    KCHK(e, dalloc(e, &p.n2k, cap6 * 6));
    KCHK(e, dalloc(e, &p.range_err, 1, true));
    p.sort_tmp_bytes = crf_sort_temp_bytes(cap6, max_batch);
    char* st = nullptr;
    KCHK(e, dalloc(e, &st, p.sort_tmp_bytes));
    p.sort_tmp = st;
    const size_t chunk_pix = (size_t)std::min<int64_t>((int64_t)p.chunk * max_pixels_per_image, max_total_pixels);
    p.val_cap = std::max(chunk_pix * 6 * Kp * G2, cap6);
    KCHK(e, dalloc(e, &p.va, p.val_cap));
    KCHK(e, dalloc(e, &p.vb, p.val_cap));
    p.valg_cap = chunk_pix * 3 * Kp * G2;
    KCHK(e, dalloc(e, &p.vga, p.valg_cap));
    KCHK(e, dalloc(e, &p.vgb, p.valg_cap));
    p.reserved = true;
    return PNP_OK;
}

extern "C" int pnp_post_prepare(pnp_engine* e, const pnp_post_batch* b, int32_t want_crf, void* stream) {
    if (!e || !b) return PNP_ERR_ARG;
    auto& p = e->post;
    if (!p.reserved) return fail(e, PNP_ERR_STATE, "call pnp_post_reserve first");
    if (b->B <= 0 || b->B > p.maxB) return fail(e, PNP_ERR_ARG, "post batch %d out of range", b->B);
    if (!b->H || !b->W || !b->n_classes || !b->has_bg || !b->img_cls_off || !b->cls_off || !b->tok_idx || !b->cls_div || !b->lut)
        return fail(e, PNP_ERR_ARG, "post batch has null tables");
    if (want_crf && !b->d_rgb) return fail(e, PNP_ERR_ARG, "CRF needs d_rgb");
    hipStream_t s = (hipStream_t)stream;
    const int B = b->B;
    p.prepared = false;
    p.desc.assign(B, PostDesc{});
    std::vector<size_t>& label_off = p.h_label_off;
    std::vector<int32_t>& wt_off = p.h_wt_off;
    std::vector<double>& wts = p.h_wts;
    label_off.assign(B + 1, 0);
    wt_off.assign(B + 1, 0);
    wts.clear();
    size_t off = 0, qoff = 0;
    int64_t pix = 0;
    p.Cmax = p.Kmax = p.maxHW = p.Kpmax = p.maxH = p.maxW = p.max_radius = 0;
    for (int i = 0; i < B; i++) {
        PostDesc& d = p.desc[i];
        d.H = b->H[i]; d.W = b->W[i]; d.C = b->n_classes[i]; d.has_bg = b->has_bg[i] ? 1 : 0; d.K = d.C + d.has_bg;
        if (d.H <= 0 || d.W <= 0 || d.C <= 0 || d.K > p.maxK) return fail(e, PNP_ERR_ARG, "image %d: bad H/W/classes (K=%d max %d)", i, d.K, p.maxK);
        if ((int64_t)d.H * d.W > p.max_pix_img) return fail(e, PNP_ERR_ARG, "image %d: %dx%d exceeds max_pixels_per_image", i, d.H, d.W);
        if (b->img_cls_off[i + 1] - b->img_cls_off[i] != d.C) return fail(e, PNP_ERR_ARG, "image %d: merge plan has %d classes, expected %d", i, b->img_cls_off[i + 1] - b->img_cls_off[i], d.C);
        d.pix0 = (int)pix;
        d.off = off;
        d.Kp = (d.K + 3) / 4 * 4;
        d.G = 1;
        d.Kg = d.K;
        d.qoff = qoff;
        label_off[i] = (size_t)pix;
        off += (size_t)d.K * d.H * d.W;
        qoff += (size_t)d.Kp * d.H * d.W;
        p.Kpmax = std::max(p.Kpmax, d.Kp);
        p.maxH = std::max(p.maxH, d.H);
        p.maxW = std::max(p.maxW, d.W);
        pix += (int64_t)d.H * d.W;
        p.Cmax = std::max(p.Cmax, d.C);
        p.Kmax = std::max(p.Kmax, d.K);
        p.maxHW = std::max(p.maxHW, d.H * d.W);
        const double sigma = 0.05 * (double)std::max(d.H, d.W);
        const int radius = (int)(4.0 * sigma + 0.5);
        std::vector<double> phi(2 * radius + 1);
        double sum = 0;
        for (int x = -radius; x <= radius; x++) {
            phi[x + radius] = std::exp(-0.5 / (sigma * sigma) * (double)(x * x));
            sum += phi[x + radius];
        }
        p.max_radius = std::max(p.max_radius, (b->blur_wts && b->blur_wt_off) ? b->blur_wt_off[i + 1] - b->blur_wt_off[i] - 1 : radius);
        wt_off[i] = (int32_t)wts.size();
        if (b->blur_wts && b->blur_wt_off) {
            for (int j = b->blur_wt_off[i]; j < b->blur_wt_off[i + 1]; j++) wts.push_back(b->blur_wts[j]);
        } else {
            for (int j = 0; j <= radius; j++) wts.push_back(phi[radius - j] / sum);
        }
    }
    wt_off[B] = (int32_t)wts.size();
    label_off[B] = (size_t)pix;
    if (pix > p.max_total_pix) return fail(e, PNP_ERR_ARG, "batch has %lld pixels, reserved %lld", (long long)pix, (long long)p.max_total_pix);
    if ((int)wts.size() > p.wts_cap) return fail(e, PNP_ERR_ARG, "blur taps exceed reserved capacity");
    const int ncls = b->img_cls_off[B], ntok = b->cls_off[ncls];
    if (ncls > p.cls_cap || ntok > p.tok_cap) return fail(e, PNP_ERR_ARG, "merge plan exceeds reserved capacity");
    if (b->lut_stride < p.Kmax || B * b->lut_stride > p.lut_cap) return fail(e, PNP_ERR_ARG, "bad lut_stride");
    std::vector<size_t> voff_pair(2 * (size_t)B, 0);
    for (int c0 = 0; c0 < B; c0 += p.chunk) {
        size_t v[2] = {0, 0}, v2[2] = {0, 0};
        for (int i = c0; i < std::min(B, c0 + p.chunk); i++)
            for (int t = 0; t < 2; t++) {
                p.desc[i].voff[t] = v[t];
                v[t] += (size_t)p.desc[i].H * p.desc[i].W * (t == 0 ? 3 : 6) * p.desc[i].Kp;
                voff_pair[2 * (size_t)i + t] = v2[t];
                v2[t] += (size_t)p.desc[i].H * p.desc[i].W * (t == 0 ? 3 : 6) * ((2 * p.desc[i].K + 3) / 4 * 4);
            }
        if (p.groups_cap * v[1] > p.val_cap || p.groups_cap * v[0] > p.valg_cap)
            return fail(e, PNP_ERR_ARG, "CRF chunk needs %zu value floats, reserved %zu", p.groups_cap * v[1], p.val_cap);
    }
    p.B = B;
    p.total_pix = pix;
    p.lut_stride = b->lut_stride;
    p.d_rgb = b->d_rgb;
    p.d_gt = b->d_gt;
    HIPCHK(e, hipMemcpyAsync(p.d_desc, p.desc.data(), sizeof(PostDesc) * B, hipMemcpyHostToDevice, s));
    p.desc_pair = p.desc;
    p.Kpmax_pair = 0;
    {
        size_t qoff2 = 0;
        for (int i = 0; i < B; i++) {
            PostDesc& d = p.desc_pair[i];
            d.G = 2;
            d.Kp = (2 * d.K + 3) / 4 * 4;
            d.qoff = qoff2;
            qoff2 += (size_t)d.Kp * d.H * d.W;
            d.voff[0] = voff_pair[2 * (size_t)i];
            d.voff[1] = voff_pair[2 * (size_t)i + 1];
            p.Kpmax_pair = std::max(p.Kpmax_pair, d.Kp);
        }
    }
    HIPCHK(e, hipMemcpyAsync(p.d_desc_pair, p.desc_pair.data(), sizeof(PostDesc) * B, hipMemcpyHostToDevice, s));
    HIPCHK(e, hipMemcpyAsync(p.d_img_cls_off, b->img_cls_off, 4 * (B + 1), hipMemcpyHostToDevice, s));
    HIPCHK(e, hipMemcpyAsync(p.d_cls_off, b->cls_off, 4 * (ncls + 1), hipMemcpyHostToDevice, s));
    HIPCHK(e, hipMemcpyAsync(p.d_cls_div, b->cls_div, 4 * std::max(ncls, 1), hipMemcpyHostToDevice, s));
    HIPCHK(e, hipMemcpyAsync(p.d_tok_idx, b->tok_idx, 4 * std::max(ntok, 1), hipMemcpyHostToDevice, s));
    HIPCHK(e, hipMemcpyAsync(p.d_lut, b->lut, 4 * (size_t)B * b->lut_stride, hipMemcpyHostToDevice, s));
    HIPCHK(e, hipMemcpyAsync(p.d_label_off, label_off.data(), sizeof(size_t) * (B + 1), hipMemcpyHostToDevice, s));
    HIPCHK(e, hipMemcpyAsync(p.d_wts, wts.data(), 8 * wts.size(), hipMemcpyHostToDevice, s));
    HIPCHK(e, hipMemcpyAsync(p.d_wt_off, wt_off.data(), 4 * (B + 1), hipMemcpyHostToDevice, s));
    p.has_crf = false;
    bool synced = false;
    if (want_crf) {
        std::vector<int> sig;
        for (int i = 0; i < B; i++) { sig.push_back(p.desc[i].H); sig.push_back(p.desc[i].W); }
        for (int t = 0; t < 2; t++) {
            if (t == 0 && sig == p.gauss_sig) continue;
            const int D1 = t == 0 ? 3 : 6;
            KCHK(e, crf_build_lattice(D1 - 1, p.lat[t], p.d_desc, p.desc.data(), p.d_rgb, t == 0 ? 3.0f : 50.0f, 5.0f, B, (size_t)pix * D1,
                                      p.maxHW, p.keys_a, p.keys_b, p.vals_a, p.head, p.incl,
                                      p.n1k, p.n2k, p.sort_tmp, p.sort_tmp_bytes, p.range_err, &p.range_err_host, &p.lat_points[t], s));
            KCHK(e, crf_lattice_norm(p.lat[t], p.d_desc, B, p.maxHW, (size_t)pix * D1, p.va, p.vb, p.norm[t], s));
            synced = true;
        }
        if (p.range_err_host) {
            p.range_err_host = 0;
            p.gauss_sig.clear();
            (void)hipMemsetAsync(p.range_err, 0, 4, s);
            return fail(e, PNP_ERR_ARG, "lattice key out of packing range (image too large for the 64-bit key)");
        }
        p.gauss_sig = sig;
        p.has_crf = true;
    }
    if (!synced) HIPCHK(e, hipStreamSynchronize(s));
    p.prepared = true;
    return PNP_OK;
}

#define POST_READY(e)                                                                     \
    if (!(e)) return PNP_ERR_ARG;                                                         \
    if (!(e)->post.prepared) return fail(e, PNP_ERR_STATE, "call pnp_post_prepare first");

extern "C" int pnp_merge_tokens(pnp_engine* e, const float* d_gradcam, int32_t T, void* stream) {
    POST_READY(e);
    auto& p = e->post;
    if (!d_gradcam || T < 5) return fail(e, PNP_ERR_ARG, "bad gradcam / T");
    KCHK(e, merge_tokens(d_gradcam, p.d_cls_off, p.d_tok_idx, p.d_cls_div, p.d_img_cls_off, p.merged, p.B, T, e->PP, p.Cmax,
                         (hipStream_t)stream));
    return PNP_OK;
}

extern "C" int pnp_threshold_upsample(pnp_engine* e, float threshold, int32_t scale01, void* stream) {
    POST_READY(e);
    auto& p = e->post;
    hipStream_t s = (hipStream_t)stream;
    KCHK(e, threshold_maps(p.merged, p.d_img_cls_off, p.thr, threshold, p.B, e->PP, p.Cmax, s));
    KCHK(e, upsample_maps(p.thr, p.d_desc, p.maps, p.B, e->P, p.Cmax, p.maxHW, s));
    if (scale01) KCHK(e, minmax_normalize(p.maps, p.d_desc, p.stats, p.B, p.Cmax, p.maxHW, 1, s));
    KCHK(e, background_channel(p.maps, p.d_desc, p.B, p.maxHW, s));
    p.maps_in_2 = false;
    return PNP_OK;
}

extern "C" int pnp_blur_minmax(pnp_engine* e, void* stream) {
    POST_READY(e);
    auto& p = e->post;
    hipStream_t s = (hipStream_t)stream;
    KCHK(e, blur_maps(p.maps, p.maps3, p.maps2, p.d_desc, p.d_wts, p.d_wt_off, p.B, p.Kmax, p.maxH, p.maxW, p.max_radius, s));
    KCHK(e, minmax_normalize(p.maps2, p.d_desc, p.stats, p.B, p.Kmax, p.maxHW, 0, s));
    p.maps_in_2 = true;
    return PNP_OK;
}

static int crf_iterate_body(pnp_engine* e, const PostDesc* desc, int kp_max, int32_t iters, float pos_w, float bi_w, hipStream_t s,
                            const CrfLabelOut& labels);

static int crf_iterate(pnp_engine* e, const PostDesc* desc, int kp_max, int32_t iters, float pos_w, float bi_w, hipStream_t s,
                       const CrfLabelOut& labels = CrfLabelOut()) {
    auto& pf = e->crf_prof;
    const bool timed = pf.on && pf.used < 4096;
    if (timed) {
        if ((int)pf.ev0.size() <= pf.used) {
            hipEvent_t a, b;
            if (hipEventCreate(&a) != hipSuccess || hipEventCreate(&b) != hipSuccess) return fail(e, PNP_ERR_HIP, "hipEventCreate failed");
            pf.ev0.push_back(a);
            pf.ev1.push_back(b);
        }
        (void)hipEventRecord(pf.ev0[pf.used], s);
    }
    const int r = crf_iterate_body(e, desc, kp_max, iters, pos_w, bi_w, s, labels);
    if (timed) {
        (void)hipEventRecord(pf.ev1[pf.used], s);
        pf.used++;
        pf.launches++;
        const auto& p = e->post;
        const int groups = desc == p.d_desc_pair ? 2 : 1;
        double kpix = 0, pix = 0;
        for (int i = 0; i < p.B; i++) {
            kpix += (double)p.desc[i].K * p.desc[i].H * p.desc[i].W;
            pix += (double)p.desc[i].H * p.desc[i].W;
        }
        const double kavg = pix > 0 ? kpix / pix : 0;
        pf.work += (double)iters * 20.0 * 4.0 * groups * kpix;
        pf.lattice += (double)iters * 2.0 * 4.0 * groups * kavg * (2.0 * p.lat_points[0] + 3.0 * p.lat_points[1]);
    }
    return r;
}

static int crf_iterate_body(pnp_engine* e, const PostDesc* desc, int kp_max, int32_t iters, float pos_w, float bi_w, hipStream_t s,
                            const CrfLabelOut& labels) {
    auto& p = e->post;
    const int groups = desc == p.d_desc_pair ? 2 : 1;
    for (int c0 = 0; c0 < p.B; c0 += p.chunk) {
        const int n = std::min(p.chunk, p.B - c0);
        KCHK(e, crf_update(p.lat[0], p.lat[1], desc, c0, n, p.vga, p.va, p.norm[0], p.norm[1], p.unary, p.Q, pos_w, bi_w, 0,
                           p.maxHW, kp_max, groups, s));
        for (int it = 0; it < iters; it++) {
            const float *rg = nullptr, *rb = nullptr;
            KCHK(e, crf_filter(p.lat[0], desc, c0, n, p.Q, p.vga, p.vgb, &rg, kp_max, s));
            KCHK(e, crf_filter(p.lat[1], desc, c0, n, p.Q, p.va, p.vb, &rb, kp_max, s));
            KCHK(e, crf_update(p.lat[0], p.lat[1], desc, c0, n, rg, rb, p.norm[0], p.norm[1], p.unary, p.Q, pos_w, bi_w, 1,
                               p.maxHW, kp_max, groups, s, it == iters - 1 ? labels : CrfLabelOut()));
        }
    }
    return PNP_OK;
}

extern "C" int pnp_densecrf(pnp_engine* e, int32_t iters, float pos_w, float pos_xy, float bi_w, float bi_xy, float bi_rgb,
                            void* stream) {
    POST_READY(e);
    auto& p = e->post;
    if (!p.has_crf) return fail(e, PNP_ERR_STATE, "batch was prepared without CRF lattices");
    if (pos_xy != 3.0f || bi_xy != 50.0f || bi_rgb != 5.0f)
        return fail(e, PNP_ERR_ARG, "lattices are built for sxy=3 / sxy=50, srgb=5 (PnP.py:1036-1041)");
    hipStream_t s = (hipStream_t)stream;
    const float* maps = p.maps_in_2 ? p.maps2 : p.maps;
    KCHK(e, unary_from_maps(maps, p.d_desc, p.unary, p.B, p.maxHW, p.maxKp, 0, s));
    return crf_iterate(e, p.d_desc, p.Kpmax, iters, pos_w, bi_w, s);
}

extern "C" int pnp_remap_hist(pnp_engine* e, int32_t from_crf, uint8_t* d_labels, unsigned long long* d_hist, int32_t n_class,
                              void* stream) {
    POST_READY(e);
    auto& p = e->post;
    if (!d_labels) return fail(e, PNP_ERR_ARG, "d_labels is null");
    hipStream_t s = (hipStream_t)stream;
    const float* src = from_crf ? p.Q : (p.maps_in_2 ? p.maps2 : p.maps);
    KCHK(e, argmax_remap(src, p.d_desc, p.d_lut, p.lut_stride, d_labels, p.d_label_off, from_crf ? 1 : 0, 0, p.B, p.maxHW, s));
    if (d_hist && p.d_gt) KCHK(e, confusion_hist(d_labels, p.d_gt, p.d_desc, p.d_label_off, d_hist, n_class, p.B, p.maxHW, s));
    return PNP_OK;
}

extern "C" int pnp_postprocess(pnp_engine* e, const float* d_gradcam, int32_t T, float threshold, int32_t scale01, int32_t mode,
                               uint8_t* d_labels, unsigned long long* d_hist, int32_t n_class, void* stream) {
    int r = pnp_merge_tokens(e, d_gradcam, T, stream);
    if (r) return r;
    r = pnp_threshold_upsample(e, threshold, scale01, stream);
    if (r) return r;
    if (mode & 1) {
        r = pnp_blur_minmax(e, stream);
        if (r) return r;
    }
    if (mode & 2) {
        r = pnp_densecrf(e, 10, 7.0f, 3.0f, 10.0f, 50.0f, 5.0f, stream);
        if (r) return r;
    }
    return pnp_remap_hist(e, (mode & 2) ? 1 : 0, d_labels, d_hist, n_class, stream);
}

extern "C" int pnp_postprocess_pair(pnp_engine* e, const float* d_gradcam_1drop, const float* d_gradcam_ndrop, int32_t T,
                                    float threshold, int32_t scale01_mask, uint8_t* d_labels_1drop, unsigned long long* d_hist_1drop,
                                    uint8_t* d_labels_ndrop, unsigned long long* d_hist_ndrop, int32_t n_class, void* stream) {
    POST_READY(e);
    auto& p = e->post;
    if (!p.has_crf) return fail(e, PNP_ERR_STATE, "batch was prepared without CRF lattices");
    if (!d_labels_1drop || !d_labels_ndrop) return fail(e, PNP_ERR_ARG, "label outputs are null");
    if (p.groups_cap < 2) {
        int r = pnp_postprocess(e, d_gradcam_1drop, T, threshold, scale01_mask & 1, 3, d_labels_1drop, d_hist_1drop, n_class, stream);
        if (r) return r;
        return pnp_postprocess(e, d_gradcam_ndrop, T, threshold, (scale01_mask >> 1) & 1, 3, d_labels_ndrop, d_hist_ndrop, n_class, stream);
    }
    hipStream_t s = (hipStream_t)stream;
    for (int grp = 0; grp < 2; grp++) {
        int r = pnp_merge_tokens(e, grp == 0 ? d_gradcam_1drop : d_gradcam_ndrop, T, stream);
        if (r) return r;
        r = pnp_threshold_upsample(e, threshold, (scale01_mask >> grp) & 1, stream);
        if (r) return r;
        r = pnp_blur_minmax(e, stream);
        if (r) return r;
        KCHK(e, unary_from_maps(p.maps2, p.d_desc_pair, p.unary, p.B, p.maxHW, p.maxKp, grp, s));
    }
    CrfLabelOut lout;
    lout.lab[0] = d_labels_1drop;
    lout.lab[1] = d_labels_ndrop;
    lout.lut = p.d_lut;
    lout.lut_stride = p.lut_stride;
    lout.label_off = p.d_label_off;
    int r = crf_iterate(e, p.d_desc_pair, p.Kpmax_pair, 10, 7.0f, 10.0f, s, lout);
    if (r) return r;
    for (int grp = 0; grp < 2; grp++) {
        uint8_t* lab = grp == 0 ? d_labels_1drop : d_labels_ndrop;
        unsigned long long* hist = grp == 0 ? d_hist_1drop : d_hist_ndrop;
        if (hist && p.d_gt) KCHK(e, confusion_hist(lab, p.d_gt, p.d_desc, p.d_label_off, hist, n_class, p.B, p.maxHW, s));
    }
    return PNP_OK;
}


extern "C" int pnp_get_buffer(pnp_engine* e, const char* name, void** d_ptr, size_t* bytes) {
    if (!e || !name || !d_ptr || !bytes) return PNP_ERR_ARG;
    const std::string n(name);
    const size_t B = e->c.max_batch, L = e->c.max_text_len;
    auto& p = e->post;
    auto set = [&](void* ptr, size_t b) { *d_ptr = ptr; *bytes = b; return PNP_OK; };
    if (n == "image_embeds") return set(e->emb32, B * e->N * (size_t)e->D * 4);
    if (n == "image_embeds_t") return set(e->embT.hi, B * e->N * (size_t)e->D * e->esz);
    if (n == "x") return set(e->x, B * e->N * (size_t)e->D * 4);
    if (n == "P") return set(e->ta[e->grad_layer >= 0 ? e->grad_layer : e->SL].Pc, B * e->nh * L * (size_t)e->Nst * 4);
    if (n == "dP") return set(e->dPc, B * e->nh * L * (size_t)e->Nst * 4);
    if (n == "text_hidden") return set(e->ta[e->TL - 1].h_out, B * L * (size_t)e->H * 4);
    if (n == "h_last") return set(e->ta[e->TL - 1].h_out, B * L * (size_t)e->H * 4);
    if (n == "dropped") return set(e->dropped, B * (size_t)e->PP);
    if (n == "P_last" && e->ta[e->TL - 1].Pc) return set(e->ta[e->TL - 1].Pc, B * e->nh * L * (size_t)e->Nst * 4);
    if (n == "Kt" && e->Kt) return set(e->Kt, (size_t)(e->TL - e->SL - 1) * e->H * B * e->Npad * e->esz);
    if (n == "Vt") return set(e->Vt, (size_t)e->TL * e->H * B * e->Npad * e->esz);
    if (n == "dq_xattn") return set(e->dqc, B * L * (size_t)e->H * e->esz);
    if (n == "dctx_xattn") return set(e->dctxc, B * L * (size_t)e->H * e->esz);
    if (p.reserved) {
        const size_t mk = (size_t)p.max_total_pix * p.maxK * 4;
        const size_t mq = (size_t)p.max_total_pix * p.maxKp * 4 * p.groups_cap;
        if (n == "merged") return set(p.merged, (size_t)p.maxB * p.maxK * e->PP * 4);
        if (n == "maps") return set(p.maps_in_2 ? p.maps2 : p.maps, mk);
        if (n == "maps_pre_blur") return set(p.maps, mk);
        if (n == "unary") return set(p.unary, mq);
        if (n == "crf_q") return set(p.Q, mq);
        if (n == "crf_idbase_gauss") return set(p.lat[0].idbase, ((size_t)p.maxB + 1) * 4);
        if (n == "crf_idbase_bilateral") return set(p.lat[1].idbase, ((size_t)p.maxB + 1) * 4);
        if (n == "crf_norm_gauss") return set(p.norm[0], (size_t)p.max_total_pix * 4);
        if (n == "crf_norm_bilateral") return set(p.norm[1], (size_t)p.max_total_pix * 4);
        if (n == "crf_offset_gauss") return set(p.lat[0].offset, (size_t)p.max_total_pix * 3 * 4);
        if (n == "crf_offset_bilateral") return set(p.lat[1].offset, (size_t)p.max_total_pix * 6 * 4);
        if (n == "crf_nbr8_gauss") return set(p.lat[0].nbr8, (size_t)(p.lat[0].D1 / 2) * p.lat[0].cap * sizeof(CrfNbr8));
        if (n == "crf_nbr8_bilateral") return set(p.lat[1].nbr8, (size_t)(p.lat[1].D1 / 2) * p.lat[1].cap * sizeof(CrfNbr8));
    }
    return fail(e, PNP_ERR_ARG, "unknown buffer %s", name);
}

extern "C" size_t pnp_allocated_bytes(const pnp_engine* e) { return e ? e->alloc_bytes : 0; }

extern "C" int pnp_profile_enable(pnp_engine* e, int32_t on) {
    if (!e) return PNP_ERR_ARG;
    if (!e->gemm_prof) {
        if (!on) {
            e->crf_prof.on = false;
            return PNP_OK;
        }
        e->gemm_prof = new GemmProfile();
    }
    GemmProfile& pf = *e->gemm_prof;
    pf.on = on != 0;
    pf.period = on > 1 ? on : 1;
    pf.seq = 0;
    pf.used = 0;
    pf.launches = 0;
    pf.flops = 0;
    e->crf_prof.on = on != 0;
    e->crf_prof.used = 0;
    e->crf_prof.launches = 0;
    e->crf_prof.work = 0;
    e->crf_prof.lattice = 0;
    return PNP_OK;
}

extern "C" int pnp_profile_read_stage(pnp_engine* e, int32_t stage, int64_t* launches, double* work, double* ms) {
    if (!e || !launches || !work || !ms) return PNP_ERR_ARG;
    if (stage == 0) return pnp_profile_read(e, launches, work, ms);
    if (stage != 1 && stage != 2) return fail(e, PNP_ERR_ARG, "unknown profile stage %d", stage);
    auto& pf = e->crf_prof;
    double total = 0;
    for (int i = 0; i < pf.used; i++) {
        HIPCHK(e, hipEventSynchronize(pf.ev1[i]));
        float t = 0;
        HIPCHK(e, hipEventElapsedTime(&t, pf.ev0[i], pf.ev1[i]));
        total += t;
    }
    *launches = pf.launches;
    *work = stage == 1 ? pf.work : pf.lattice;
    *ms = total;
    return PNP_OK;
}

extern "C" int pnp_profile_read(pnp_engine* e, int64_t* launches, double* flops, double* ms) {
    if (!e || !launches || !flops || !ms) return PNP_ERR_ARG;
    if (!e->gemm_prof) {
        *launches = 0; *flops = 0; *ms = 0;
        return PNP_OK;
    }
    GemmProfile& pf = *e->gemm_prof;
    double total = 0;
    for (int i = 0; i < pf.used; i++) {
        HIPCHK(e, hipEventSynchronize(pf.ev1[i]));
        float t = 0;
        HIPCHK(e, hipEventElapsedTime(&t, pf.ev0[i], pf.ev1[i]));
        total += t;
    }
    *launches = pf.launches;
    *flops = pf.flops;
    *ms = total;
    return PNP_OK;
}

extern "C" int pnp_op_gemm(int32_t bf, const void* d_A, int32_t lda, const void* d_B, int32_t ldb, int32_t M, int32_t N,
                           int32_t K, const float* d_bias, const float* d_resid, int32_t ldr, float* d_out_f32, int32_t ldo,
                           int32_t gelu, void* stream) {
    GemmArgs g = G_(d_A, lda, d_B, ldb, M, N, K);
    g.bias = d_bias; g.resid = d_resid; g.ldr = ldr; g.out_f32 = d_out_f32; g.ldo = ldo;
    g.mode = gelu ? GEMM_EPI_GELU : GEMM_EPI_LINEAR;
    return gemm_nt(bf, g, (hipStream_t)stream);
}

extern "C" int pnp_op_gemm_ex(int32_t bf, const void* d_A, int32_t lda, const void* d_B, int32_t ldb, int32_t M, int32_t N,
                              int32_t K, const float* d_bias, const float* d_resid, int32_t ldr, float* d_out_f32, int32_t ldo,
                              void* d_out_t, int32_t ldo_t, int32_t mode, void* stream) {
    GemmArgs g = G_(d_A, lda, d_B, ldb, M, N, K);
    g.bias = d_bias; g.resid = d_resid; g.ldr = ldr; g.out_f32 = d_out_f32; g.ldo = ldo; g.out_t = d_out_t; g.ldo_t = ldo_t;
    g.mode = mode ? GEMM_EPI_GELU : GEMM_EPI_LINEAR;
    return gemm_nt(bf, g, (hipStream_t)stream);
}

extern "C" int pnp_op_split(const float* d_in, void* d_hi, void* d_lo, int64_t n, void* stream) {
    if (!d_in || !d_hi || !d_lo || n <= 0) return PNP_ERR_ARG;
    return split_f32(d_in, d_hi, d_lo, (size_t)n, (hipStream_t)stream);
}

extern "C" int pnp_op_gemm_x3(const void* d_A_hi, const void* d_A_lo, int32_t lda, const void* d_B_hi, const void* d_B_lo,
                              int32_t ldb, int32_t M, int32_t N, int32_t K, const float* d_bias, int32_t bias_on_rows,
                              const float* d_resid, int32_t ldr, float* d_out_f32, int32_t ldo, void* d_out_hi, void* d_out_lo,
                              int32_t ldo_t, int32_t gelu, int32_t col_div, int32_t col_pad, void* stream) {
    if (!d_A_hi || !d_A_lo || !d_B_hi || !d_B_lo) return PNP_ERR_ARG;
    GemmArgs g = G_(d_A_hi, lda, d_B_hi, ldb, M, N, K);
    g.A_lo = d_A_lo; g.B_lo = d_B_lo;
    g.bias = d_bias; g.bias_on_rows = bias_on_rows; g.resid = d_resid; g.ldr = ldr; g.out_f32 = d_out_f32; g.ldo = ldo;
    g.out_t = d_out_hi; g.out_lo = d_out_lo; g.ldo_t = ldo_t; g.col_div = col_div; g.col_pad = col_pad;
    g.mode = gelu ? GEMM_EPI_GELU : GEMM_EPI_LINEAR;
    g.sk = streamk_mode() ? streamk_ws_default() : nullptr;
    return gemm_nt(1, g, (hipStream_t)stream);
}

extern "C" int pnp_set_tuning(const char* key, int32_t value) {
    if (!key) return PNP_ERR_ARG;
    if (!strcmp(key, "streamk")) {
        if (value < 0 || value > 2) return PNP_ERR_ARG;
        set_streamk_mode(value);
        return PNP_OK;
    }
    if (!strcmp(key, "text_rows")) {
        if (value < 0 || value > 4) return PNP_ERR_ARG;
        set_text_rows(value);
        return PNP_OK;
    }
    if (!strcmp(key, "gemm_stamps")) {
        if (value < 0 || value > 1) return PNP_ERR_ARG;
        return gemm_set_stamps(value);
    }
    return PNP_ERR_ARG;
}

extern "C" int pnp_streamk_status(pnp_engine* e, int64_t* launches, uint32_t* gave_up) {
    if (!launches || !gave_up) return PNP_ERR_ARG;
    StreamKWs* ws = e ? &e->sk_ws : streamk_ws_default();
    *launches = ws ? ws->launches : 0;
    *gave_up = 0;
    if (!ws || !ws->part) return PNP_OK;
    if (e) HIPCHK(e, hipSetDevice(e->c.device));
    if (hipDeviceSynchronize() != hipSuccess) return PNP_ERR_HIP;
    return streamk_ws_timeouts(ws, gave_up);
}

extern "C" int pnp_op_gemm_x3a(const float* d_A, int32_t lda, const void* d_B_hi, const void* d_B_lo, int32_t ldb, int32_t M,
                               int32_t N, int32_t K, const float* d_bias, const float* d_resid, int32_t ldr, float* d_out_f32,
                               int32_t ldo, int32_t mode, float* d_aux, int32_t ld_aux, void* stream) {
    if (!d_A || !d_B_hi || !d_B_lo || !d_out_f32 || mode < 0 || mode > 2) return PNP_ERR_ARG;
    GemmArgs g = G_(d_A, lda, d_B_hi, ldb, M, N, K);
    g.B_lo = d_B_lo; g.a_f32 = 1;
    g.bias = d_bias; g.resid = d_resid; g.ldr = ldr; g.out_f32 = d_out_f32; g.ldo = ldo;
    g.mode = mode; g.aux = d_aux; g.ld_aux = ld_aux;
    return gemm_nt(0, g, (hipStream_t)stream);
}

extern "C" int pnp_op_gemm_tokcols(int32_t bf, const void* d_A, int32_t lda, const void* d_B, int32_t ldb, int32_t M, int32_t N,
                                   int32_t K, const float* d_bias_rows, void* d_out_t, int32_t ldo_t, int32_t col_div,
                                   int32_t col_pad, void* stream) {
    if (!d_out_t || col_div < 0 || (col_div > 0 && col_pad < col_div)) return PNP_ERR_ARG;
    GemmArgs g = G_(d_A, lda, d_B, ldb, M, N, K);
    g.bias = d_bias_rows; g.bias_on_rows = 1; g.out_t = d_out_t; g.ldo_t = ldo_t; g.col_div = col_div; g.col_pad = col_pad;
    return gemm_nt(bf, g, (hipStream_t)stream);
}

extern "C" int pnp_op_gemm_args(int32_t bf, const void* d_A, int32_t lda, const void* d_B, int32_t ldb, int32_t M, int32_t N,
                                int32_t K, const float* d_bias, int32_t bias_on_rows, const float* d_resid, int32_t ldr,
                                float* d_out_f32, int32_t ldo, void* d_out_t, int32_t ldo_t, int32_t mode, float* d_aux,
                                int32_t ld_aux, int32_t row_div, int32_t col_div, int32_t col_pad, void* stream) {
    if (!d_A || !d_B || (!d_out_f32 && !d_out_t) || M <= 0 || N <= 0 || K <= 0 || lda < K || ldb < K) return PNP_ERR_ARG;
    if (mode < 0 || mode > 2 || (mode == GEMM_EPI_GELU_GRAD && !d_aux)) return PNP_ERR_ARG;
    if (row_div < 0 || col_div < 0 || (col_div > 0 && col_pad < col_div)) return PNP_ERR_ARG;
    GemmArgs g = G_(d_A, lda, d_B, ldb, M, N, K);
    g.bias = d_bias; g.bias_on_rows = bias_on_rows ? 1 : 0; g.resid = d_resid; g.ldr = ldr;
    g.out_f32 = d_out_f32; g.ldo = ldo; g.out_t = d_out_t; g.ldo_t = ldo_t;
    g.mode = mode; g.aux = d_aux; g.ld_aux = ld_aux; g.row_div = row_div; g.col_div = col_div; g.col_pad = col_pad;
    return gemm_nt(bf ? 1 : 0, g, (hipStream_t)stream);
}

extern "C" int pnp_op_vit_attention(int32_t bf, const void* d_qk, int32_t ld_qk, int32_t D, const void* d_vt, int32_t ld_vt,
                                    int32_t n_pad, void* d_ctx, int32_t B, int32_t heads, int32_t N, float scale, void* stream) {
    if (!d_qk || !d_vt || !d_ctx || B <= 0 || heads <= 0 || N <= 0) return PNP_ERR_ARG;
    return vit_attention(bf, d_qk, ld_qk, D, d_vt, ld_vt, n_pad, d_ctx, B, heads, N, scale, (hipStream_t)stream);
}

extern "C" int pnp_op_vit_attention_x3(const void* d_qkv_hi, const void* d_qkv_lo, int32_t ld_qkv, int32_t D, void* d_ctx_hi,
                                       void* d_ctx_lo, int32_t B, int32_t heads, int32_t N, float scale, void* stream) {
    if (B <= 0 || heads <= 0 || N <= 0 || ld_qkv < 3 * D) return PNP_ERR_ARG;
    return vit_attention_x3(d_qkv_hi, d_qkv_lo, ld_qkv, D, d_ctx_hi, d_ctx_lo, B, heads, N, scale, (hipStream_t)stream);
}

extern "C" int pnp_op_layernorm(const float* d_x, const float* d_w, const float* d_b, float eps, int32_t rows, int32_t D,
                                float* d_y, void* stream) {
    return layernorm(0, d_x, d_w, d_b, eps, rows, D, d_y, nullptr, nullptr, nullptr, (hipStream_t)stream);
}

extern "C" int pnp_op_xattn(int32_t bf16, int32_t mode, const void* d_nat, int32_t ld_nat, const void* d_tr, int32_t ld_tr,
                            int32_t n_pad, const void* d_x, int32_t ldx, void* d_out, int32_t ldo, float* d_probs,
                            int32_t n_stride, int32_t B, int32_t L, int32_t N, int32_t heads, void* stream) {
    if (!d_nat || !d_x || !d_probs || mode < 0 || mode > 2 || (mode != 2 && (!d_tr || !d_out))) return PNP_ERR_ARG;
    if (B <= 0 || L <= 0 || N <= 0 || heads <= 0) return PNP_ERR_ARG;
    return xattn(bf16, mode, d_nat, ld_nat, d_tr, ld_tr, n_pad, d_x, ldx, d_out, ldo, d_probs, n_stride, B, L, N, heads,
                 (hipStream_t)stream);
}

extern "C" int pnp_op_text_self_attn(int32_t bf16, const void* d_qkv, const int64_t* d_mask, int32_t ld_mask, void* d_ctx,
                                     float* d_probs, float* d_scratch, int32_t B, int32_t L, int32_t H, void* stream) {
    if (!d_qkv || !d_mask || !d_ctx || B <= 0 || L <= 0 || H <= 0 || ld_mask < L) return PNP_ERR_ARG;
    return text_self_attn(bf16, d_qkv, d_mask, ld_mask, d_ctx, d_probs, d_scratch, B, L, H, (hipStream_t)stream);
}

extern "C" int pnp_op_text_self_attn_bwd(int32_t bf16, const void* d_qkv, const float* d_dctx, const float* d_probs,
                                         float* d_ds_scratch, void* d_dqkv, int32_t B, int32_t L, int32_t H, void* stream) {
    if (!d_qkv || !d_dctx || !d_probs || !d_ds_scratch || !d_dqkv || B <= 0 || L <= 0 || H <= 0) return PNP_ERR_ARG;
    return text_self_attn_bwd(bf16, d_qkv, d_dctx, d_probs, d_ds_scratch, d_dqkv, B, L, H, (hipStream_t)stream);
}

extern "C" int pnp_op_layernorm_ex(int32_t bf16, const float* d_x, const float* d_w, const float* d_b, float eps, int32_t rows,
                                   int32_t D, float* d_y, void* d_yt, void* d_yt_lo, float* d_xhat, float* d_rstd, void* stream) {
    if (!d_x || !d_w || !d_b || rows <= 0 || D <= 0 || (d_yt_lo && !d_yt)) return PNP_ERR_ARG;
    return layernorm(bf16, d_x, d_w, d_b, eps, rows, D, d_y, d_yt, d_xhat, d_rstd, (hipStream_t)stream, d_yt_lo);
}

extern "C" int pnp_op_layernorm_bwd(int32_t bf16, const float* d_dy, const float* d_w, const float* d_xhat, const float* d_rstd,
                                    int32_t rows, int32_t D, float* d_dx, void* d_dxt, void* stream) {
    if (!d_dy || !d_w || !d_xhat || !d_rstd || rows <= 0 || D <= 0) return PNP_ERR_ARG;
    return layernorm_bwd(bf16, d_dy, d_w, d_xhat, d_rstd, rows, D, d_dx, d_dxt, (hipStream_t)stream);
}

extern "C" int pnp_op_text_embed(const int64_t* d_ids, int32_t ld_ids, const float* d_word, const float* d_pos, float* d_out,
                                 int32_t B, int32_t L, int32_t H, int32_t enc_id, int32_t vocab, void* stream) {
    if (!d_ids || !d_word || !d_pos || !d_out || B <= 0 || L <= 0 || H <= 0 || H % 4 || vocab <= 0 || ld_ids < L || enc_id >= vocab)
        return PNP_ERR_ARG;
    return text_embed(d_ids, ld_ids, d_word, d_pos, d_out, B, L, H, enc_id, vocab, (hipStream_t)stream);
}

extern "C" int pnp_op_itm_head(const float* d_hlast, const float* d_w, const float* d_bias, float* d_logits, int32_t B, int32_t L,
                               int32_t H, void* stream) {
    if (!d_hlast || !d_w || !d_bias || !d_logits || B <= 0 || L <= 0 || H <= 0) return PNP_ERR_ARG;
    return itm_head(d_hlast, d_w, d_bias, d_logits, B, L, H, (hipStream_t)stream);
}

extern "C" int pnp_op_itm_grad_seed(const float* d_w, float* d_dh, int32_t B, int32_t L, int32_t H, void* stream) {
    if (!d_w || !d_dh || B <= 0 || L <= 0 || H <= 0) return PNP_ERR_ARG;
    return itm_grad_seed(d_w, d_dh, B, L, H, (hipStream_t)stream);
}

extern "C" int pnp_op_patchify(int32_t bf16, const float* d_img, const uint8_t* d_dropped, void* d_out, int32_t B, int32_t S,
                               int32_t P, void* stream) {
    if (!d_img || !d_out || B <= 0 || P <= 0 || S != P * 16) return PNP_ERR_ARG;
    return patchify(bf16, d_img, d_dropped, d_out, B, S, P, (hipStream_t)stream);
}

extern "C" int pnp_op_cls_rows(const float* d_cls, const float* d_pos, float* d_x, int32_t B, int32_t N, int32_t D, void* stream) {
    if (!d_cls || !d_pos || !d_x || B <= 0 || N <= 0 || D <= 0) return PNP_ERR_ARG;
    return cls_rows(d_cls, d_pos, d_x, B, N, D, (hipStream_t)stream);
}

extern "C" int pnp_dbg_gemm_stamps(uint64_t* host_out, int32_t max_blocks) {
    return gemm_read_stamps((unsigned long long*)host_out, max_blocks);
}

extern "C" int pnp_preprocess_images(const uint8_t* d_rgb, const pnp_pre_image* d_desc, int32_t B, int32_t S, int32_t max_H,
                                     const int32_t* d_coef, uint8_t* d_tmp, const float* mean3, const float* std3,
                                     float* d_out, void* stream) {
    if (!d_rgb || !d_desc || !d_coef || !d_tmp || !mean3 || !std3 || !d_out) return PNP_ERR_ARG;
    static_assert(sizeof(pnp_pre_image) == 40, "pnp_pre_image layout is part of the ABI");
    return preprocess_images(d_rgb, d_desc, B, S, max_H, d_coef, d_tmp, mean3, std3, d_out, (hipStream_t)stream);
}

extern "C" int pnp_jpeg_decode(const uint8_t* d_data, const pnp_jpeg_image* d_images, const pnp_jpeg_tables* d_tables,
                               const pnp_jpeg_segment* d_segments, int32_t n_images, int32_t n_segments, uint8_t* d_clean,
                               int32_t* d_seg_bits, int16_t* d_coef, int64_t coef_elems, uint8_t* d_planes, uint8_t* d_rgb,
                               int32_t max_blocks_per_image, int32_t max_pixels_per_image, int32_t* d_err, void* stream) {
    if (!d_data || !d_images || !d_tables || !d_segments || !d_clean || !d_seg_bits || !d_coef || !d_planes || !d_rgb || !d_err ||
        coef_elems <= 0)
        return PNP_ERR_ARG;
    static_assert(sizeof(pnp_jpeg_image) == sizeof(JpegImage) && sizeof(pnp_jpeg_tables) == sizeof(JpegTables) &&
                      sizeof(pnp_jpeg_segment) == sizeof(JpegSegment), "JPEG descriptor layouts are part of the ABI");
    return jpeg_decode(d_data, reinterpret_cast<const JpegImage*>(d_images), reinterpret_cast<const JpegTables*>(d_tables),
                       reinterpret_cast<const JpegSegment*>(d_segments), n_images, n_segments, d_clean, d_seg_bits, d_coef,
                       (size_t)coef_elems, d_planes, d_rgb, max_blocks_per_image, max_pixels_per_image, d_err, (hipStream_t)stream);
}

extern "C" int pnp_op_sort_pairs(uint64_t* d_keys_in, uint64_t* d_keys_out, uint32_t* d_vals_in, uint32_t* d_vals_out, int64_t n,
                                 int32_t begin_bit, int32_t end_bit, const size_t* h_seg_off, int32_t n_seg, void* stream) {
    if (n < 0 || (n && (!d_keys_in || !d_keys_out || !d_vals_in || !d_vals_out))) return PNP_ERR_ARG;
    if (!n) return PNP_OK;
    const size_t tb = sort_temp_bytes((size_t)n);
    void* temp = nullptr;
    if (hipMalloc(&temp, tb) != hipSuccess) return PNP_ERR_NOMEM;
    int r = radix_sort_pairs(d_keys_in, d_keys_out, d_vals_in, d_vals_out, (size_t)n, begin_bit, end_bit, h_seg_off, n_seg, temp, tb, (hipStream_t)stream);
    if (hipStreamSynchronize((hipStream_t)stream) != hipSuccess && r == PNP_OK) r = PNP_ERR_HIP;
    (void)hipFree(temp);
    return r;
}
extern "C" int pnp_op_scan_i32(const int32_t* d_in, int32_t* d_out, int64_t n, int32_t inclusive, void* stream) {
    if (n < 0 || (n && (!d_in || !d_out))) return PNP_ERR_ARG;
    if (!n) return PNP_OK;
    const size_t tb = sort_temp_bytes((size_t)n);
    void* temp = nullptr;
    if (hipMalloc(&temp, tb) != hipSuccess) return PNP_ERR_NOMEM;
    int r = device_scan_i32(d_in, d_out, (size_t)n, inclusive != 0, temp, tb, (hipStream_t)stream);
    if (hipStreamSynchronize((hipStream_t)stream) != hipSuccess && r == PNP_OK) r = PNP_ERR_HIP;
    (void)hipFree(temp);
    return r;
}

extern "C" int pnp_op_cast(int32_t to_bf16, const float* d_in, void* d_out, int64_t n, void* stream) {
    return cast_f32(to_bf16, d_in, d_out, (size_t)n, (hipStream_t)stream);
}
```

### pnp-ovss_amd/csrc/kernels.h

```cpp
#pragma once
#include <hip/hip_runtime.h>
#include <stdint.h>
#include <stddef.h>
#include "gemm.h"

namespace pnp {

struct PostDesc {
    int H, W, K, C, has_bg, pix0;
    int Kp;
    int G, Kg;
    size_t off;
    size_t qoff;
    size_t voff[2];
};

struct alignas(16) CrfEntry {
    uint32_t pixel;
    float w;
    float nr;
    uint32_t pad;
};

struct alignas(16) CrfNbr8 {
    int ia, id;
    int pa, pd;
    int aa, ad;
    int da, dd;
};

struct CrfLattice {
    int D1;
    int which;
    size_t cap;
    float* bary;
    uint32_t* vals;
    CrfEntry* ent;
    int* offset;
    int* seg_start;
    int* seg_lo;
    int* seg_hi;
    uint64_t* ukeys;
    int* idbase;
    int* n1;
    int* n2;
    CrfNbr8* nbr8;
};

int patchify(int bf, const float* img, const uint8_t* dropped, void* out, int B, int S, int P, hipStream_t s);
int cls_rows(const float* cls, const float* pos, float* x, int B, int N, int D, hipStream_t s);
int layernorm(int bf, const float* x, const float* w, const float* b, float eps, int rows, int D, float* y, void* yt,
              float* xhat, float* rstd, hipStream_t s, void* yt_lo = nullptr);
int vit_attention(int bf, const void* qk, int ld_qk, int D, const void* vt, int ld_vt, int Npad, void* ctx, int B,
                  int H, int N, float scale, hipStream_t s, void* ctx_lo = nullptr);

int vit_attention_x3(const void* qkv_hi, const void* qkv_lo, int ld_qk, int D, void* ctx_hi, void* ctx_lo, int B, int H, int N,
                     float scale, hipStream_t s);

int text_embed(const int64_t* ids, int ld_ids, const float* word, const float* pos, float* out, int B, int L, int H,
               int enc_id, int vocab, hipStream_t s);
int text_self_attn(int bf, const void* qkv, const int64_t* mask, int ld_mask, void* ctx, float* probs, float* scratch, int B, int L,
                   int H, hipStream_t s);
void set_text_rows(int n);
int text_self_attn_bwd(int bf, const void* qkv, const float* dctx, const float* probs, float* ds_scratch, void* dqkv,
                       int B, int L, int H, hipStream_t s);
int xattn(int bf, int mode, const void* a1, int ld1, const void* a2t, int ld2, int Npad, const void* x, int ldx,
          void* out, int ldo, float* pbuf, int Nst, int B, int L, int N, int nheads, hipStream_t s);
int layernorm_bwd(int bf, const float* dy, const float* w, const float* xhat, const float* rstd, int rows, int D,
                  float* dx, void* dxt, hipStream_t s);
int itm_head(const float* hlast, const float* w, const float* bias, float* logits, int B, int L, int H, hipStream_t s);
int itm_grad_seed(const float* w, float* dh, int B, int L, int H, hipStream_t s);
int cast_f32(int bf, const float* in, void* out, size_t n, hipStream_t s);
int split_f32(const float* in, void* hi, void* lo, size_t n, hipStream_t s);

int l2_normalize_rows(float* x, int rows, int E, float eps, hipStream_t s);
int itc_similarity(const float* img, const float* txt, float* sim, int B, int T, int E, hipStream_t s);
int cast_rows_bf16(const float* in, int ld_in, void* out, int rows, int K, hipStream_t s);

int gradcam_gather(const float* P, const float* dP, const int64_t* mask, int ld_mask, float* out, int B, int nheads,
                   int head, int L, int Nst, int PP, hipStream_t s);
int drop_step(const float* G, float* g0, float* agg, uint8_t* dropped, int32_t* picks, int iter, int B, int T, int PP,
              int npick, int max_picks, hipStream_t s);
int merge_tokens(const float* src, const int32_t* cls_off, const int32_t* tok_idx, const int32_t* cls_div,
                 const int32_t* img_cls_off, float* out, int B, int T, int PP, int Cmax, hipStream_t s);
int threshold_maps(const float* merged, const int32_t* img_cls_off, float* out, float threshold, int B, int PP, int Cmax,
                   hipStream_t s);
int upsample_maps(const float* src, const PostDesc* desc, float* maps, int B, int P, int Cmax, int maxHW, hipStream_t s);
int minmax_normalize(float* maps, const PostDesc* desc, float* stats, int B, int Kmax, int maxHW, int class_channels_only,
                     hipStream_t s);
int background_channel(float* maps, const PostDesc* desc, int B, int maxHW, hipStream_t s);
int blur_maps(const float* in, float* tmp, float* out, const PostDesc* desc, const double* wts, const int32_t* wt_off,
              int B, int Kmax, int maxH, int maxW, int max_radius, hipStream_t s);
int preprocess_images(const uint8_t* rgb, const void* desc, int B, int S, int max_H, const int32_t* coef, uint8_t* tmp,
                      const float* mean3, const float* std3, float* out, hipStream_t s);
int unary_from_maps(const float* maps, const PostDesc* desc, float* unary, int B, int maxHW, int max_kp, int group, hipStream_t s);
int argmax_remap(const float* q, const PostDesc* desc, const int32_t* lut, int lut_stride, uint8_t* labels,
                 const size_t* label_off, int pixel_major, int group, int B, int maxHW, hipStream_t s);
int confusion_hist(const uint8_t* labels, const float* gt, const PostDesc* desc, const size_t* label_off,
                   unsigned long long* hist, int n_class, int B, int maxHW, hipStream_t s);

struct JpegImage {
    int64_t data_off;
    int64_t coef_off[3];
    int64_t plane_off[3];
    int64_t rgb_off;
    int32_t data_len, H, W, ncomp, hmax, vmax, mcux, mcuy;
    int32_t h[3], v[3], tq[3], td[3], ta[3], bx[3], by[3];
    int32_t tab, pad[2];
};
struct JpegTables {
    uint8_t counts[4][16];
    uint8_t vals[4][256];
    int32_t quant[4][64];
};
struct JpegSegment {
    int64_t byte_off;
    int64_t clean_off;
    int32_t image, mcu0, nmcu;
    int32_t raw_len;
    int32_t clean_cap;
    int32_t sub_bits;
    int32_t pad[2];
};
int jpeg_decode(const uint8_t* d_data, const JpegImage* d_imgs, const JpegTables* d_tabs, const JpegSegment* d_segs, int n_images,
                int n_segments, uint8_t* d_clean, int* d_seg_bits, int16_t* d_coef, size_t coef_elems, uint8_t* d_planes, uint8_t* d_rgb,
                int max_blocks, int max_pixels, int* d_err, hipStream_t s);

size_t sort_temp_bytes(size_t n);
int radix_sort_pairs(uint64_t* keys_in, uint64_t* keys_out, uint32_t* vals_in, uint32_t* vals_out, size_t n, int begin_bit, int end_bit,
                     const size_t* seg_off, int nseg, void* temp, size_t temp_bytes, hipStream_t s);
int device_scan_i32(const int* in, int* out, size_t n, bool inclusive, void* temp, size_t temp_bytes, hipStream_t s);
size_t crf_sort_temp_bytes(size_t max_entries, int max_images);
int crf_build_lattice(int D, const CrfLattice& L, const PostDesc* d_imgs, const PostDesc* h_imgs, const uint8_t* d_rgb, float sxy, float srgb,
                      int B, size_t ent_total, int max_pixels,
                      uint64_t* keys_a, uint64_t* keys_b, uint32_t* vals_a, int* head, int* incl, int* n1k, int* n2k,
                      void* temp, size_t temp_bytes, int* d_range_err, int* h_range_err, int* h_points, hipStream_t s);
int crf_lattice_norm(const CrfLattice& L, const PostDesc* d_imgs, int B, int max_pixels, size_t ent_total, float* va, float* vb,
                     float* norm_out, hipStream_t s);
int crf_filter(const CrfLattice& L, const PostDesc* d_imgs, int img0, int nimg, const float* Q,
               float* va, float* vb, const float** result, int max_kp, hipStream_t s);
struct CrfLabelOut {
    uint8_t* lab[2] = {nullptr, nullptr};
    const int32_t* lut = nullptr;
    int lut_stride = 0;
    const size_t* label_off = nullptr;
};
int crf_update(const CrfLattice& Lg, const CrfLattice& Lb, const PostDesc* d_imgs, int img0, int nimg, const float* vg,
               const float* vb, const float* norm_g, const float* norm_b, const float* unary, float* Q, float w_g,
               float w_b, int pairwise, int max_pixels, int max_kp, int groups, hipStream_t s, const CrfLabelOut& labels = CrfLabelOut());

}
```

### pnp-ovss_amd/csrc/pipeline_kernels.hip

```cpp
#include "common.h"
#include "kernels.h"
#include "../../include/pnp_math.h"

namespace pnp {

__global__ void gradcam_gather_kernel(const float* __restrict__ P, const float* __restrict__ dP,
                                      const int64_t* __restrict__ mask, int ld_mask, float* __restrict__ out, int B,
                                      int nheads, int head, int L, int Nst, int PP) {
    const int idx = blockIdx.x * blockDim.x + threadIdx.x;
    const int T = L - 1;
    if (idx >= B * T * PP) return;
    const int p = idx % PP, t = (idx / PP) % T, b = idx / (PP * T);
    const size_t o = (((size_t)b * nheads + head) * L + (t + 1)) * Nst + 1 + p;
    const float g = P[o] * fmaxf(dP[o], 0.f) * (float)mask[(size_t)b * ld_mask + t + 1];
    out[idx] = g < 0.f ? 0.f : g;
}

__device__ __forceinline__ uint64_t sal_key(float v, int idx) {
    uint32_t u = __float_as_uint(v);
    u = (v != v) ? 0xffffffffu : ((u & 0x80000000u) ? ~u : (u | 0x80000000u));
    return ((uint64_t)u << 32) | (uint32_t)idx;
}

__global__ __launch_bounds__(256) void drop_accumulate_kernel(const float* __restrict__ G, float* __restrict__ g0,
                                                              float* __restrict__ agg, const uint8_t* __restrict__ dropped,
                                                              int iter, int T, int PP) {
    const int b = blockIdx.y;
    const uint8_t* dr = dropped + (size_t)b * PP;
    for (int i = blockIdx.x * 256 + threadIdx.x; i < T * PP; i += gridDim.x * 256) {
        const int p = i % PP;
        const size_t o = (size_t)b * T * PP + i;
        const float v = dr[p] ? 0.f : G[o];
        if (iter == 0) {
            if (g0) g0[o] = v;
            agg[o] = v + v;
        } else {
            agg[o] += v;
        }
    }
}

__global__ __launch_bounds__(256) void drop_step_kernel(const float* __restrict__ G, uint8_t* __restrict__ dropped,
                                                        int32_t* __restrict__ picks, int iter, int T, int PP,
                                                        int npick, int max_picks) {
    extern __shared__ __attribute__((aligned(16))) char smem[];
    float* sal = reinterpret_cast<float*>(smem);
    __shared__ uint64_t red[4];
    const int b = blockIdx.x, tid = threadIdx.x;
    const float* Gb = G + (size_t)b * T * PP;
    uint8_t* dr = dropped + (size_t)b * PP;
    for (int p = tid; p < PP; p += 256) {
        float s = 0.f;
        int t = 3;
        for (; t + 8 <= T - 1; t += 8) {
            float v[8];
#pragma unroll
            for (int u = 0; u < 8; u++) v[u] = Gb[(size_t)(t + u) * PP + p];
#pragma unroll
            for (int u = 0; u < 8; u++) s += v[u];
        }
        for (; t < T - 1; t++) s += Gb[(size_t)t * PP + p];
        sal[p] = dr[p] ? 0.f : s;
    }
    __syncthreads();
    if (npick <= 0) return;
    for (int k = 0; k < npick; k++) {
        uint64_t best = 0;
        for (int p = tid; p < PP; p += 256) {
            const uint64_t key = sal_key(sal[p], p);
            const bool taken = (__float_as_uint(sal[p]) == 0xffc00001u);
            if (!taken && key > best) best = key;
        }
        for (int o = 32; o > 0; o >>= 1) {
            const uint64_t other = __shfl_xor(best, o, 64);
            best = other > best ? other : best;
        }
        if ((tid & 63) == 0) red[tid >> 6] = best;
        __syncthreads();
        if (tid == 0) {
            uint64_t m = red[0];
            for (int w = 1; w < 4; w++) m = red[w] > m ? red[w] : m;
            const int p = (int)(m & 0xffffffffu);
            const int slot = iter * npick + (npick - 1 - k);
            if (slot < max_picks) picks[(size_t)b * max_picks + slot] = p;
            sal[p] = __uint_as_float(0xffc00001u);
        }
        __syncthreads();
    }
    for (int k = tid; k < npick; k += 256) {
        const int slot = iter * npick + k;
        if (slot < max_picks) dr[picks[(size_t)b * max_picks + slot]] = 1;
    }
}

__global__ void merge_tokens_kernel(const float* __restrict__ src, const int32_t* __restrict__ cls_off,
                                    const int32_t* __restrict__ tok_idx, const int32_t* __restrict__ cls_div,
                                    const int32_t* __restrict__ img_cls_off, float* __restrict__ out, int T, int PP,
                                    int Cmax) {
    const int b = blockIdx.y, c = blockIdx.x;
    const int c0 = img_cls_off[b], nc = img_cls_off[b + 1] - c0;
    if (c >= nc) return;
    const int k0 = cls_off[c0 + c], k1 = cls_off[c0 + c + 1];
    const int div = cls_div[c0 + c];
    const float* sb = src + (size_t)b * T * PP;
    for (int p = threadIdx.x; p < PP; p += blockDim.x) {
        float acc = 0.f;
        if (k1 > k0) {
            acc = sb[(size_t)(3 + tok_idx[k0]) * PP + p];
            for (int k = k0 + 1; k < k1; k++) acc += sb[(size_t)(3 + tok_idx[k]) * PP + p];
            if (div != 1) acc = acc / (float)div;
        }
        out[((size_t)b * Cmax + c) * PP + p] = acc;
    }
}

__global__ __launch_bounds__(256) void threshold_kernel(const float* __restrict__ merged, const int32_t* __restrict__ img_cls_off,
                                                        float* __restrict__ out, float threshold, int PP, int Cmax) {
    const int b = blockIdx.y, c = blockIdx.x, tid = threadIdx.x;
    const int nc = img_cls_off[b + 1] - img_cls_off[b];
    if (c >= nc) return;
    __shared__ float smn[4], smx[4];
    const float* m = merged + ((size_t)b * Cmax + c) * PP;
    float mn = INFINITY, mx = -INFINITY;
    int nan = 0;
    for (int p = tid; p < PP; p += 256) {
        const float v = m[p];
        nan |= (v != v);
        mn = fminf(mn, v);
        mx = fmaxf(mx, v);
    }
    for (int o = 32; o > 0; o >>= 1) {
        mn = fminf(mn, __shfl_xor(mn, o, 64));
        mx = fmaxf(mx, __shfl_xor(mx, o, 64));
    }
    if ((tid & 63) == 0) { smn[tid >> 6] = mn; smx[tid >> 6] = mx; }
    nan = __syncthreads_or(nan);
    mn = fminf(fminf(smn[0], smn[1]), fminf(smn[2], smn[3]));
    mx = fmaxf(fmaxf(smx[0], smx[1]), fmaxf(smx[2], smx[3]));
    const float den = nan ? __uint_as_float(0x7fc00000u) : mx - mn;
    for (int p = tid; p < PP; p += 256) {
        const float v = m[p];
        const float nrm = (v - mn) / den;
        out[((size_t)b * Cmax + c) * PP + p] = (nrm >= threshold) ? v : v * 0.0f;
    }
}

__device__ __forceinline__ void src_index(int dst, int in_size, float scale, int& i0, int& i1, float& w0, float& w1) {
    const float real = __fmul_rn(scale, (float)dst);
    int f = (int)floorf(real);
    f = f < in_size - 1 ? f : in_size - 1;
    float lam = __fsub_rn(real, (float)f);
    lam = fminf(fmaxf(lam, 0.f), 1.f);
    i0 = f;
    i1 = f + (f < in_size - 1 ? 1 : 0);
    w1 = lam;
    w0 = __fsub_rn(1.f, lam);
}

__global__ void upsample_kernel(const float* __restrict__ src, const PostDesc* __restrict__ desc, float* __restrict__ maps,
                                int P, int Cmax) {
    const int b = blockIdx.z, c = blockIdx.y;
    const PostDesc d = desc[b];
    if (c >= d.C) return;
    const int H = d.H, W = d.W;
    const float sh = H > 1 ? __fdiv_rn((float)(P - 1), (float)(H - 1)) : 0.f;
    const float sw = W > 1 ? __fdiv_rn((float)(P - 1), (float)(W - 1)) : 0.f;
    const float* s = src + ((size_t)b * Cmax + c) * P * P;
    float* o = maps + d.off + (size_t)(c + d.has_bg) * H * W;
    for (int i = blockIdx.x * blockDim.x + threadIdx.x; i < H * W; i += gridDim.x * blockDim.x) {
        const int y = i / W, x = i - y * W;
        int h0, h1, w0i, w1i;
        float a, bb, cc, dd;
        src_index(y, P, sh, h0, h1, a, bb);
        src_index(x, P, sw, w0i, w1i, cc, dd);
        const float v00 = s[h0 * P + w0i], v01 = s[h0 * P + w1i], v10 = s[h1 * P + w0i], v11 = s[h1 * P + w1i];
        const float top = fmaf(v00, cc, __fmul_rn(v01, dd));
        const float bot = fmaf(v10, cc, __fmul_rn(v11, dd));
        o[i] = fmaf(top, a, __fmul_rn(bot, bb));
    }
}

__global__ __launch_bounds__(256) void minmax_kernel(const float* __restrict__ maps, const PostDesc* __restrict__ desc,
                                                     float* __restrict__ stats, int Kmax, int first_k_is_class) {
    const int b = blockIdx.y, k = blockIdx.x, tid = threadIdx.x;
    const PostDesc d = desc[b];
    const int kk = first_k_is_class ? k + d.has_bg : k;
    if (kk >= d.K) return;
    if (first_k_is_class && d.C == 1) return;
    __shared__ float smn[4], smx[4];
    const float* m = maps + d.off + (size_t)kk * d.H * d.W;
    float mn = INFINITY, mx = -INFINITY;
    bool nan = false;
    const int n = d.H * d.W;
    for (int p0 = tid; p0 < n; p0 += 8 * 256) {
        float v[8];
#pragma unroll
        for (int u = 0; u < 8; u++) {
            const int p = p0 + u * 256;
            v[u] = p < n ? m[p] : m[p0];
        }
#pragma unroll
        for (int u = 0; u < 8; u++) {
            nan |= (v[u] != v[u]);
            mn = fminf(mn, v[u]);
            mx = fmaxf(mx, v[u]);
        }
    }
    for (int o = 32; o > 0; o >>= 1) {
        mn = fminf(mn, __shfl_xor(mn, o, 64));
        mx = fmaxf(mx, __shfl_xor(mx, o, 64));
        nan |= (bool)__shfl_xor((int)nan, o, 64);
    }
    __shared__ int snan[4];
    if ((tid & 63) == 0) { smn[tid >> 6] = mn; smx[tid >> 6] = mx; snan[tid >> 6] = nan; }
    __syncthreads();
    if (tid == 0) {
        mn = fminf(fminf(smn[0], smn[1]), fminf(smn[2], smn[3]));
        mx = fmaxf(fmaxf(smx[0], smx[1]), fmaxf(smx[2], smx[3]));
        if (snan[0] | snan[1] | snan[2] | snan[3]) mn = mx = __uint_as_float(0x7fc00000u);
        stats[((size_t)b * Kmax + kk) * 2 + 0] = mn;
        stats[((size_t)b * Kmax + kk) * 2 + 1] = mx;
    }
}

__global__ void normalize_kernel(float* __restrict__ maps, const PostDesc* __restrict__ desc, const float* __restrict__ stats,
                                 int Kmax, int first_k_is_class) {
    const int b = blockIdx.z, k = blockIdx.y;
    const PostDesc d = desc[b];
    const int kk = first_k_is_class ? k + d.has_bg : k;
    if (kk >= d.K) return;
    if (first_k_is_class && d.C == 1) return;
    const float mn = stats[((size_t)b * Kmax + kk) * 2], mx = stats[((size_t)b * Kmax + kk) * 2 + 1];
    const float den = __fsub_rn(mx, mn);
    float* m = maps + d.off + (size_t)kk * d.H * d.W;
    const int n = d.H * d.W;
    for (int i = blockIdx.x * blockDim.x + threadIdx.x; i < n; i += gridDim.x * blockDim.x)
        m[i] = __fdiv_rn(__fsub_rn(m[i], mn), den);
}

__global__ void background_kernel(float* __restrict__ maps, const PostDesc* __restrict__ desc) {
    const int b = blockIdx.y;
    const PostDesc d = desc[b];
    if (!d.has_bg) return;
    const int n = d.H * d.W;
    float* m = maps + d.off;
    for (int i = blockIdx.x * blockDim.x + threadIdx.x; i < n; i += gridDim.x * blockDim.x) {
        float mx = m[(size_t)n + i];
        bool nan = mx != mx;
        int c = 1;
        for (; c + 8 <= d.C; c += 8) {
            float v[8];
#pragma unroll
            for (int u = 0; u < 8; u++) v[u] = m[(size_t)(1 + c + u) * n + i];
#pragma unroll
            for (int u = 0; u < 8; u++) {
                nan |= (v[u] != v[u]);
                mx = fmaxf(mx, v[u]);
            }
        }
        for (; c < d.C; c++) {
            const float v = m[(size_t)(1 + c) * n + i];
            nan |= (v != v);
            mx = fmaxf(mx, v);
        }
        m[i] = (!nan && mx == 0.f) ? 1.f : 0.f;
    }
}

__device__ __forceinline__ int reflect_idx(int i, int n) {
    const int period = 2 * n;
    int m = i % period;
    if (m < 0) m += period;
    return m >= n ? period - 1 - m : m;
}

__device__ __forceinline__ void blur_window8(const float* __restrict__ ctr, int S, const double* __restrict__ wl, int radius,
                                             double* __restrict__ acc) {
    constexpr int R = 8;
    double lo[R], hi[R];
#pragma unroll
    for (int i = 0; i < R; i++) {
        acc[i] = __dmul_rn((double)ctr[i * S], wl[0]);
        lo[i] = (double)ctr[(i - radius) * S];
        hi[i] = (double)ctr[(i + radius) * S];
    }
    for (int j = radius; j >= 1; j -= R) {
#pragma unroll
        for (int jj = 0; jj < R; jj++) {
            const int jc = j - jj;
            if (jc >= 1) {
                const double wj = wl[jc];
                double t8[R];
#pragma unroll
                for (int i = 0; i < R; i++)
                    t8[i] = __dadd_rn(lo[(i + jj) % R], hi[(i - jj + R) % R]);
#pragma unroll
                for (int i = 0; i < R; i++) t8[i] = __dmul_rn(t8[i], wj);
#pragma unroll
                for (int i = 0; i < R; i++) acc[i] = __dadd_rn(acc[i], t8[i]);
                lo[jj % R] = (double)ctr[(R - jc) * S];
                hi[(R - 1 - jj) % R] = (double)ctr[(jc - 1) * S];
            }
        }
    }
}

__device__ __forceinline__ int reflect_fast(int i, int n) {
    if (i >= 0 && i < n) return i;
    const int m = i < 0 ? -i - 1 : 2 * n - 1 - i;
    return (m >= 0 && m < n) ? m : reflect_idx(i, n);
}

template <int AXIS>
__global__ __launch_bounds__(1024) void blur_axis_kernel(const float* __restrict__ in, float* __restrict__ out,
                                                        const PostDesc* __restrict__ desc, const double* __restrict__ wts,
                                                        const int32_t* __restrict__ wt_off, int max_radius, int NT) {
    constexpr int axis = AXIS;
    constexpr int TH = 32, TW = 64;
    extern __shared__ __attribute__((aligned(16))) double tile[];
    double* wl = tile;
    float* xs = reinterpret_cast<float*>(tile + ((max_radius + 3) & ~1));
    const int b = blockIdx.z, k = blockIdx.y;
    const PostDesc d = desc[b];
    if (k >= d.K) return;
    const int H = d.H, W = d.W;
    const int THe = axis == 0 ? TH * NT : TH, TWe = axis == 1 ? TW * NT : TW;
    const int tiles_x = (W + TWe - 1) / TWe, tiles_y = (H + THe - 1) / THe;
    const double* w = wts + wt_off[b];
    const int radius = wt_off[b + 1] - wt_off[b] - 1;
    const float* src = in + d.off + (size_t)k * H * W;
    float* dst = out + d.off + (size_t)k * H * W;
    const int tid = threadIdx.x, nthr = blockDim.x;
    const int sub = tid >> 8, t = tid & 255;
    for (int j = tid; j <= radius; j += nthr) wl[j] = w[j];
    const int colsP = (TWe + 2 * radius) | 1;
    for (int tl = blockIdx.x; tl < tiles_x * tiles_y; tl += gridDim.x) {
        const int ty = tl / tiles_x, tx = tl - ty * tiles_x;
        const int y0 = ty * THe, x0 = tx * TWe;
        __syncthreads();
        double acc[8];
        if constexpr (AXIS == 0) {
            const int rows = THe + 2 * radius;
            const int c = tid & 63;
            const int x = x0 + c < W ? x0 + c : W - 1;
            if ((W & 3) == 0 && x0 + TW <= W && (reinterpret_cast<uintptr_t>(src) & 15) == 0) {
                const int c4 = (tid & 15) * 4;
                const int rp = nthr >> 4;
                for (int r0 = tid >> 4; r0 < rows; r0 += 8 * rp) {
                    f32x4 v[8];
#pragma unroll
                    for (int u = 0; u < 8; u++) {
                        const int r = r0 + rp * u;
                        v[u] = r < rows ? *reinterpret_cast<const f32x4*>(src + (size_t)reflect_fast(y0 - radius + r, H) * W + x0 + c4)
                                        : f32x4{0.f, 0.f, 0.f, 0.f};
                    }
#pragma unroll
                    for (int u = 0; u < 8; u++) {
                        const int r = r0 + rp * u;
                        if (r < rows) *reinterpret_cast<f32x4*>(xs + r * TW + c4) = v[u];
                    }
                }
            } else {
            const int rp = nthr >> 6;
            for (int r0 = tid >> 6; r0 < rows; r0 += 8 * rp) {
                float v[8];
#pragma unroll
                for (int u = 0; u < 8; u++) {
                    const int r = r0 + rp * u;
                    v[u] = r < rows ? src[(size_t)reflect_fast(y0 - radius + r, H) * W + x] : 0.f;
                }
#pragma unroll
                for (int u = 0; u < 8; u++) {
                    const int r = r0 + rp * u;
                    if (r < rows) xs[r * TW + c] = v[u];
                }
            }
            }
            __syncthreads();
            {
                const int rg = sub * 4 + (t >> 6);
                if (y0 + rg * 8 >= H) continue;
                blur_window8(xs + (size_t)(rg * 8 + radius) * TW + c, TW, wl, radius, acc);
                if (x0 + c < W) {
#pragma unroll
                    for (int i = 0; i < 8; i++)
                        if (y0 + rg * 8 + i < H) dst[(size_t)(y0 + rg * 8 + i) * W + x0 + c] = (float)acc[i];
                }
            }
        } else {
            const int total = TH * colsP;
            constexpr int NF = 16;
            for (int i0 = tid; i0 < total; i0 += NF * nthr) {
                float v[NF];
#pragma unroll
                for (int u = 0; u < NF; u++) {
                    const int i = i0 + u * nthr;
                    const int r = i / colsP, c = i - r * colsP;
                    const int y = y0 + r < H ? y0 + r : H - 1;
                    v[u] = i < total ? src[(size_t)y * W + reflect_fast(x0 - radius + c, W)] : 0.f;
                }
#pragma unroll
                for (int u = 0; u < NF; u++) {
                    const int i = i0 + u * nthr;
                    if (i < total) xs[i] = v[u];
                }
            }
            __syncthreads();
            const int rr = t & 31;
            {
                const int cg = sub * 8 + (t >> 5);
                if (x0 + cg * 8 >= W) continue;
                blur_window8(xs + (size_t)rr * colsP + radius + cg * 8, 1, wl, radius, acc);
                if (y0 + rr < H) {
                    float* o = dst + (size_t)(y0 + rr) * W + x0 + cg * 8;
                    if (x0 + cg * 8 + 7 < W && ((reinterpret_cast<uintptr_t>(o) & 15) == 0)) {
                        reinterpret_cast<f32x4*>(o)[0] = f32x4{(float)acc[0], (float)acc[1], (float)acc[2], (float)acc[3]};
                        reinterpret_cast<f32x4*>(o)[1] = f32x4{(float)acc[4], (float)acc[5], (float)acc[6], (float)acc[7]};
                    } else {
#pragma unroll
                        for (int i = 0; i < 8; i++)
                            if (x0 + cg * 8 + i < W) o[i] = (float)acc[i];
                    }
                }
            }
        }
    }
}

struct PreImage {
    int64_t src_off, tmp_off;
    int32_t H, W, kx_off, kx_size, ky_off, ky_size;
};
__device__ __forceinline__ int clip8_fixed(int acc) {
    const int v = (acc + (1 << 21)) >> 22;
    return v < 0 ? 0 : (v > 255 ? 255 : v);
}
__global__ __launch_bounds__(256) void pre_resize_h_kernel(const uint8_t* __restrict__ rgb, const PreImage* __restrict__ desc,
                                                           int S, const int32_t* __restrict__ coef, uint8_t* __restrict__ tmp) {
    const PreImage d = desc[blockIdx.z];
    const int xo = blockIdx.x * 64 + (threadIdx.x & 63), y = blockIdx.y * 4 + (threadIdx.x >> 6);
    if (xo >= S || y >= d.H) return;
    const int32_t* t = coef + d.kx_off + (size_t)xo * (2 + d.kx_size);
    const int x0 = t[0], n = t[1];
    const uint8_t* row = rgb + d.src_off + ((size_t)y * d.W + x0) * 3;
    int a0 = 0, a1 = 0, a2 = 0;
    for (int i = 0; i < n; i++) {
        const int w = t[2 + i];
        a0 += w * row[3 * i];
        a1 += w * row[3 * i + 1];
        a2 += w * row[3 * i + 2];
    }
    uint8_t* o = tmp + d.tmp_off + ((size_t)y * S + xo) * 3;
    o[0] = (uint8_t)clip8_fixed(a0);
    o[1] = (uint8_t)clip8_fixed(a1);
    o[2] = (uint8_t)clip8_fixed(a2);
}
__global__ __launch_bounds__(256) void pre_resize_v_kernel(const uint8_t* __restrict__ tmp, const PreImage* __restrict__ desc,
                                                           int S, const int32_t* __restrict__ coef, float m0, float m1, float m2,
                                                           float s0, float s1, float s2, float* __restrict__ out) {
    const PreImage d = desc[blockIdx.z];
    const int xo = blockIdx.x * 64 + (threadIdx.x & 63), yo = blockIdx.y * 4 + (threadIdx.x >> 6);
    if (xo >= S || yo >= S) return;
    const int32_t* t = coef + d.ky_off + (size_t)yo * (2 + d.ky_size);
    const int y0 = t[0], n = t[1];
    const uint8_t* col = tmp + d.tmp_off + ((size_t)y0 * S + xo) * 3;
    int a0 = 0, a1 = 0, a2 = 0;
    for (int i = 0; i < n; i++) {
        const int w = t[2 + i];
        const uint8_t* p = col + (size_t)i * S * 3;
        a0 += w * p[0];
        a1 += w * p[1];
        a2 += w * p[2];
    }
    float* o = out + (size_t)blockIdx.z * 3 * S * S + (size_t)yo * S + xo;
    o[0] = __fdiv_rn(__fsub_rn(__fdiv_rn((float)clip8_fixed(a0), 255.0f), m0), s0);
    o[(size_t)S * S] = __fdiv_rn(__fsub_rn(__fdiv_rn((float)clip8_fixed(a1), 255.0f), m1), s1);
    o[(size_t)2 * S * S] = __fdiv_rn(__fsub_rn(__fdiv_rn((float)clip8_fixed(a2), 255.0f), m2), s2);
}

int preprocess_images(const uint8_t* rgb, const void* desc, int B, int S, int max_H, const int32_t* coef, uint8_t* tmp,
                      const float* mean3, const float* std3, float* out, hipStream_t s) {
    if (B <= 0 || S <= 0 || max_H <= 0) return PNP_ERR_ARG;
    const PreImage* d = reinterpret_cast<const PreImage*>(desc);
    hipLaunchKernelGGL(pre_resize_h_kernel, dim3((S + 63) / 64, (max_H + 3) / 4, B), dim3(256), 0, s, rgb, d, S, coef, tmp);
    hipLaunchKernelGGL(pre_resize_v_kernel, dim3((S + 63) / 64, (S + 3) / 4, B), dim3(256), 0, s, tmp, d, S, coef, mean3[0],
                       mean3[1], mean3[2], std3[0], std3[1], std3[2], out);
    return hipGetLastError() == hipSuccess ? PNP_OK : PNP_ERR_HIP;
}

__global__ __launch_bounds__(256) void unary_kernel(const float* __restrict__ maps, const PostDesc* __restrict__ desc,
                                                    float* __restrict__ unary, int group) {
    extern __shared__ __attribute__((aligned(16))) float utile[];
    const int b = blockIdx.y;
    const PostDesc d = desc[b];
    const int n = d.H * d.W, K = d.K, ldt = K + 1, R4 = d.Kp >> 2;
    const int f0 = group * d.Kg, f1 = f0 + K;
    const int c_lo = f0 >> 2, c_hi = group == d.G - 1 ? R4 : (f1 + 3) >> 2, nc = c_hi - c_lo;
    const float* m = maps + d.off;
    f32x4* u4 = reinterpret_cast<f32x4*>(unary + d.qoff);
    const int tid = threadIdx.x;
    for (int p0 = blockIdx.x * 256; p0 < n; p0 += gridDim.x * 256) {
        const int np = (n - p0) < 256 ? (n - p0) : 256;
        if (tid < np) {
            const int i = p0 + tid;
            const float* mi = m + i;
            float mx = mi[0];
            int k = 1;
            for (; k + 8 <= K; k += 8) {
                float v[8];
#pragma unroll
                for (int u = 0; u < 8; u++) v[u] = mi[(size_t)(k + u) * n];
#pragma unroll
                for (int u = 0; u < 8; u++)
                    if (v[u] > mx || v[u] != v[u]) mx = v[u];
            }
            for (; k < K; k++) {
                const float v = mi[(size_t)k * n];
                if (v > mx || v != v) mx = v;
            }
            float s = 0.f;
            float* row = utile + tid * ldt;
            for (k = 0; k + 8 <= K; k += 8) {
                float v[8];
#pragma unroll
                for (int u = 0; u < 8; u++) v[u] = mi[(size_t)(k + u) * n];
#pragma unroll
                for (int u = 0; u < 8; u++) {
                    const float e = pnp_expf(__fsub_rn(v[u], mx));
                    row[k + u] = e;
                    s = __fadd_rn(s, e);
                }
            }
            for (; k < K; k++) {
                const float e = pnp_expf(__fsub_rn(mi[(size_t)k * n], mx));
                row[k] = e;
                s = __fadd_rn(s, e);
            }
            for (int k = 0; k < K; k++) {
                float p = __fdiv_rn(row[k], s);
                if (p < 1e-5f) p = 1e-5f;
                else if (p > 1.0f) p = 1.0f;
                row[k] = -pnp_logf(p);
            }
        }
        __syncthreads();
        for (int item = tid; item < np * nc; item += 256) {
            const int pl = item / nc, c = c_lo + (item - pl * nc);
            const float* r = utile + pl * ldt;
            f32x4* dst = u4 + (size_t)(p0 + pl) * R4 + c;
            f32x4 v = {0.f, 0.f, 0.f, 0.f};
            if (4 * c < f0) v = *dst;
#pragma unroll
            for (int j = 0; j < 4; j++) {
                const int f = 4 * c + j;
                if (f >= f0) v[j] = f < f1 ? r[f - f0] : 0.f;
            }
            *dst = v;
        }
        __syncthreads();
    }
}

__global__ __launch_bounds__(256) void unary_wide_kernel(const float* __restrict__ maps, const PostDesc* __restrict__ desc,
                                                         float* __restrict__ unary, int group) {
    __shared__ float tiles[4][64][33];
    const int b = blockIdx.y;
    const int n = desc[b].H * desc[b].W, K = desc[b].K, R4 = desc[b].Kp >> 2, G = desc[b].G;
    const int f0 = group * desc[b].Kg, f1 = f0 + K;
    const int c_lo = f0 >> 2, c_hi = group == G - 1 ? R4 : (f1 + 3) >> 2;
    const float* m = maps + desc[b].off;
    f32x4* u4 = reinterpret_cast<f32x4*>(unary + desc[b].qoff);
    const int wave = threadIdx.x >> 6, lane = threadIdx.x & 63;
    float (*tile)[33] = tiles[wave];
    for (int p0 = (blockIdx.x * 4 + wave) * 64; p0 < n; p0 += gridDim.x * 256) {
        const int i = p0 + lane < n ? p0 + lane : n - 1;
        const float* mi = m + i;
        float mx = mi[0];
        int k = 1;
        for (; k + 8 <= K; k += 8) {
            float v[8];
#pragma unroll
            for (int u = 0; u < 8; u++) v[u] = mi[(size_t)(k + u) * n];
#pragma unroll
            for (int u = 0; u < 8; u++)
                if (v[u] > mx || v[u] != v[u]) mx = v[u];
        }
        for (; k < K; k++) {
            const float v = mi[(size_t)k * n];
            if (v > mx || v != v) mx = v;
        }
        float s = 0.f;
        for (k = 0; k + 8 <= K; k += 8) {
            float v[8];
#pragma unroll
            for (int u = 0; u < 8; u++) v[u] = mi[(size_t)(k + u) * n];
#pragma unroll
            for (int u = 0; u < 8; u++) s = __fadd_rn(s, pnp_expf(__fsub_rn(v[u], mx)));
        }
        for (; k < K; k++) s = __fadd_rn(s, pnp_expf(__fsub_rn(mi[(size_t)k * n], mx)));
        for (int cb = c_lo; cb < c_hi; cb += 8) {
            const int fb = 4 * cb;
            const int ka = (fb > f0 ? fb : f0) - f0, kb = (fb + 32 < f1 ? fb + 32 : f1) - f0;
            for (k = ka; k < kb; k += 8) {
                float v[8];
#pragma unroll
                for (int u = 0; u < 8; u++) v[u] = k + u < kb ? mi[(size_t)(k + u) * n] : 0.f;
#pragma unroll
                for (int u = 0; u < 8; u++) {
                    if (k + u < kb) {
                        float p = __fdiv_rn(pnp_expf(__fsub_rn(v[u], mx)), s);
                        if (p < 1e-5f) p = 1e-5f;
                        else if (p > 1.0f) p = 1.0f;
                        tile[lane][f0 + k + u - fb] = -pnp_logf(p);
                    }
                }
            }
            __builtin_amdgcn_wave_barrier();
            const int ncb = c_hi - cb < 8 ? c_hi - cb : 8;
            for (int item = lane; item < 64 * ncb; item += 64) {
                const int pl = item / ncb, c = item - pl * ncb;
                if (p0 + pl >= n) continue;
                f32x4* dst = u4 + (size_t)(p0 + pl) * R4 + cb + c;
                f32x4 v = {0.f, 0.f, 0.f, 0.f};
                if (4 * (cb + c) < f0) v = *dst;
#pragma unroll
                for (int j = 0; j < 4; j++) {
                    const int f = fb + 4 * c + j;
                    if (f >= f0) v[j] = f < f1 ? tile[pl][f - fb] : 0.f;
                }
                *dst = v;
            }
            __builtin_amdgcn_wave_barrier();
        }
    }
}

__global__ void argmax_kernel(const float* __restrict__ q, const PostDesc* __restrict__ desc, const int32_t* __restrict__ lut,
                              int lut_stride, uint8_t* __restrict__ labels, const size_t* __restrict__ label_off,
                              int pixel_major, int group) {
    const int b = blockIdx.y;
    const PostDesc d = desc[b];
    const int n = d.H * d.W, K = d.K, Kp = d.Kp;
    const float* p = q + (pixel_major ? d.qoff : d.off);
    for (int i = blockIdx.x * blockDim.x + threadIdx.x; i < n; i += gridDim.x * blockDim.x) {
        int best = 0;
        float bv = pixel_major ? p[(size_t)i * Kp + group * d.Kg] : p[i];
        if (pixel_major) {
            const int f0 = group * d.Kg;
            const f32x4* row = reinterpret_cast<const f32x4*>(p + (size_t)i * Kp);
            for (int c = f0 >> 2; c < (f0 + K + 3) >> 2; c++) {
                const f32x4 v4 = row[c];
#pragma unroll
                for (int j = 0; j < 4; j++) {
                    const int k = c * 4 + j - f0;
                    const float v = v4[j];
                    if (k >= 1 && k < K && bv == bv && (v > bv || v != v)) { best = k; bv = v; }
                }
            }
        } else {
            for (int k = 1; k < K; k++) {
                const float v = p[(size_t)k * n + i];
                if (bv == bv && (v > bv || v != v)) { best = k; bv = v; }
            }
        }
        labels[label_off[b] + i] = (uint8_t)lut[b * lut_stride + best];
    }
}

__global__ __launch_bounds__(256) void hist_kernel(const uint8_t* __restrict__ labels, const float* __restrict__ gt,
                                                   const PostDesc* __restrict__ desc, const size_t* __restrict__ label_off,
                                                   unsigned long long* __restrict__ hist, int n_class) {
    __shared__ unsigned int bins[8192];
    const int b = blockIdx.y;
    const PostDesc d = desc[b];
    const int n = d.H * d.W, nb = n_class * n_class;
    const bool use_lds = nb <= 8192;
    const int copies = nb * 4 <= 8192 ? 4 : nb * 2 <= 8192 ? 2 : 1;
    unsigned int* const mybins = bins + ((threadIdx.x >> 6) % copies) * nb;
    if (use_lds) {
        for (int i = threadIdx.x; i < nb * copies; i += 256) bins[i] = 0;
        __syncthreads();
    }
    for (int i = blockIdx.x * blockDim.x + threadIdx.x; i < n; i += gridDim.x * blockDim.x) {
        const float g = gt[label_off[b] + i];
        if (g >= 0.f && g < (float)n_class) {
            const int bin = (int)g * n_class + labels[label_off[b] + i];
            if (bin < nb) {
                if (use_lds) atomicAdd(&mybins[bin], 1u);
                else atomicAdd(&hist[bin], 1ULL);
            }
        }
    }
    if (use_lds) {
        __syncthreads();
        for (int i = threadIdx.x; i < nb; i += 256) {
            unsigned int t = bins[i];
            for (int c = 1; c < copies; c++) t += bins[c * nb + i];
            if (t) atomicAdd(&hist[i], (unsigned long long)t);
        }
    }
}

static inline int ok() { return hipGetLastError() == hipSuccess ? PNP_OK : PNP_ERR_HIP; }

int gradcam_gather(const float* P, const float* dP, const int64_t* mask, int ld_mask, float* out, int B, int nheads,
                   int head, int L, int Nst, int PP, hipStream_t s) {
    const int total = B * (L - 1) * PP;
    if (total <= 0) return PNP_ERR_ARG;
    hipLaunchKernelGGL(gradcam_gather_kernel, dim3((total + 255) / 256), dim3(256), 0, s, P, dP, mask, ld_mask, out, B,
                       nheads, head, L, Nst, PP);
    return ok();
}

int drop_step(const float* G, float* g0, float* agg, uint8_t* dropped, int32_t* picks, int iter, int B, int T, int PP,
              int npick, int max_picks, hipStream_t s) {
    if (PP * sizeof(float) > 48 * 1024) return PNP_ERR_ARG;
    const int nb = (T * PP + 1023) / 1024 < 256 ? (T * PP + 1023) / 1024 : 256;
    hipLaunchKernelGGL(drop_accumulate_kernel, dim3(nb, B), dim3(256), 0, s, G, g0, agg, dropped, iter, T, PP);
    hipLaunchKernelGGL(drop_step_kernel, dim3(B), dim3(256), PP * sizeof(float), s, G, dropped, picks, iter, T, PP, npick,
                       max_picks);
    return ok();
}

int merge_tokens(const float* src, const int32_t* cls_off, const int32_t* tok_idx, const int32_t* cls_div,
                 const int32_t* img_cls_off, float* out, int B, int T, int PP, int Cmax, hipStream_t s) {
    hipLaunchKernelGGL(merge_tokens_kernel, dim3(Cmax, B), dim3(256), 0, s, src, cls_off, tok_idx, cls_div, img_cls_off,
                       out, T, PP, Cmax);
    return ok();
}

int threshold_maps(const float* merged, const int32_t* img_cls_off, float* out, float threshold, int B, int PP, int Cmax,
                   hipStream_t s) {
    hipLaunchKernelGGL(threshold_kernel, dim3(Cmax, B), dim3(256), 0, s, merged, img_cls_off, out, threshold, PP, Cmax);
    return ok();
}

int upsample_maps(const float* src, const PostDesc* desc, float* maps, int B, int P, int Cmax, int maxHW, hipStream_t s) {
    const int nb = (maxHW + 255) / 256 < 64 ? (maxHW + 255) / 256 : 64;
    hipLaunchKernelGGL(upsample_kernel, dim3(nb, Cmax, B), dim3(256), 0, s, src, desc, maps, P, Cmax);
    return ok();
}

int minmax_normalize(float* maps, const PostDesc* desc, float* stats, int B, int Kmax, int maxHW, int class_channels_only,
                     hipStream_t s) {
    hipLaunchKernelGGL(minmax_kernel, dim3(Kmax, B), dim3(256), 0, s, maps, desc, stats, Kmax, class_channels_only);
    const int nb = (maxHW + 255) / 256 < 64 ? (maxHW + 255) / 256 : 64;
    hipLaunchKernelGGL(normalize_kernel, dim3(nb, Kmax, B), dim3(256), 0, s, maps, desc, stats, Kmax, class_channels_only);
    return ok();
}

int background_channel(float* maps, const PostDesc* desc, int B, int maxHW, hipStream_t s) {
    const int nb = (maxHW + 255) / 256 < 128 ? (maxHW + 255) / 256 : 128;
    hipLaunchKernelGGL(background_kernel, dim3(nb, B), dim3(256), 0, s, maps, desc);
    return ok();
}

int blur_maps(const float* in, float* tmp, float* out, const PostDesc* desc, const double* wts, const int32_t* wt_off,
              int B, int Kmax, int maxH, int maxW, int max_radius, hipStream_t s) {
    auto lds_for = [&](int n, size_t& l0, size_t& l1) {
        l0 = (size_t)(max_radius + 4) * sizeof(double) + (size_t)(32 * n + 2 * max_radius) * 64 * sizeof(float);
        l1 = (size_t)(max_radius + 4) * sizeof(double) + (size_t)32 * ((64 * n + 2 * max_radius) | 1) * sizeof(float);
    };
    size_t lds0, lds1;
    lds_for(1, lds0, lds1);
    int nt = lds0 > 80 * 1024 ? 4 : 1;
    lds_for(nt, lds0, lds1);
    while (nt > 1 && (lds0 > 120 * 1024 || lds1 > 120 * 1024)) lds_for(--nt, lds0, lds1);
    if (lds0 > 160 * 1024 || lds1 > 160 * 1024) return PNP_ERR_ARG;
    int nt0 = nt, nt1 = nt;
    while (nt0 > 1 && 32 * (nt0 - 1) >= maxH) nt0--;
    while (nt1 > 1 && 64 * (nt1 - 1) >= maxW) nt1--;
    lds_for(nt0, lds0, lds1);
    size_t d0, d1;
    lds_for(nt1, d0, d1);
    lds1 = d1;
    static std::atomic<uint32_t> opted0{0}, opted1{0};
    if (lds_opt_in(opted0, reinterpret_cast<const void*>(blur_axis_kernel<0>), 160 * 1024) != PNP_OK) return PNP_ERR_HIP;
    if (lds_opt_in(opted1, reinterpret_cast<const void*>(blur_axis_kernel<1>), 160 * 1024) != PNP_OK) return PNP_ERR_HIP;
    const int tiles0 = ((maxW + 63) / 64) * ((maxH + 32 * nt0 - 1) / (32 * nt0));
    const int tiles1 = ((maxW + 64 * nt1 - 1) / (64 * nt1)) * ((maxH + 31) / 32);
    hipLaunchKernelGGL(blur_axis_kernel<0>, dim3(tiles0, Kmax, B), dim3(256 * nt0), lds0, s, in, tmp, desc, wts, wt_off, max_radius, nt0);
    hipLaunchKernelGGL(blur_axis_kernel<1>, dim3(tiles1, Kmax, B), dim3(256 * nt1), lds1, s, tmp, out, desc, wts, wt_off, max_radius, nt1);
    return ok();
}

int unary_from_maps(const float* maps, const PostDesc* desc, float* unary, int B, int maxHW, int max_kp, int group, hipStream_t s) {
    const int nb = (maxHW + 255) / 256 < 256 ? (maxHW + 255) / 256 : 256;
    const size_t smem = (size_t)256 * (max_kp + 1) * sizeof(float);
    static std::atomic<uint32_t> opted{0};
    if (lds_opt_in(opted, reinterpret_cast<const void*>(unary_kernel), 160 * 1024) != PNP_OK) return PNP_ERR_HIP;
    if (max_kp >= 32) {
        const int nbw = (maxHW + 255) / 256 < 2048 ? (maxHW + 255) / 256 : 2048;
        hipLaunchKernelGGL(unary_wide_kernel, dim3(nbw, B), dim3(256), 0, s, maps, desc, unary, group);
        return ok();
    }
    hipLaunchKernelGGL(unary_kernel, dim3(nb, B), dim3(256), smem, s, maps, desc, unary, group);
    return ok();
}

int argmax_remap(const float* q, const PostDesc* desc, const int32_t* lut, int lut_stride, uint8_t* labels,
                 const size_t* label_off, int pixel_major, int group, int B, int maxHW, hipStream_t s) {
    const int nb = (maxHW + 255) / 256 < 256 ? (maxHW + 255) / 256 : 256;
    hipLaunchKernelGGL(argmax_kernel, dim3(nb, B), dim3(256), 0, s, q, desc, lut, lut_stride, labels, label_off, pixel_major, group);
    return ok();
}

int confusion_hist(const uint8_t* labels, const float* gt, const PostDesc* desc, const size_t* label_off,
                   unsigned long long* hist, int n_class, int B, int maxHW, hipStream_t s) {
    const int cap = n_class * n_class <= 8192 ? 32 : 256;
    const int nb = (maxHW + 255) / 256 < cap ? (maxHW + 255) / 256 : cap;
    hipLaunchKernelGGL(hist_kernel, dim3(nb, B), dim3(256), 0, s, labels, gt, desc, label_off, hist, n_class);
    return ok();
}

}
```

Baseline: 218.8.

## Fuse blur min/max stats into blur kernel and defer normalization to consumers

The second blur pass now reduces per-channel min/max with ordered-integer atomics, which replaces the separate minmax and normalize kernels. Normalization is applied lazily inside the unary and argmax kernels, and only materialised when the maps are read out for debugging. The unary kernel can also write the initial Q, so the first CRF update is skipped. The blur's x-axis tile load is also reorganised by wave and row. The cost is extra divides in the consumers, atomics in the blur, and more complex NaN/stat handling.

```diff
diff --git a/pnp-ovss_amd/csrc/engine.hip b/pnp-ovss_amd/csrc/engine.hip
--- a/pnp-ovss_amd/csrc/engine.hip
+++ b/pnp-ovss_amd/csrc/engine.hip
@@ -161,6 +161,8 @@
         size_t val_cap = 0;
         int lut_cap = 0, cls_cap = 0, tok_cap = 0, wts_cap = 0;
         bool maps_in_2 = false;
+        bool norm_pending = false;
+        hipStream_t norm_stream = nullptr;
     } post;
 
     GemmProfile* gemm_prof = nullptr;
@@ -1302,6 +1304,7 @@
     hipStream_t s = (hipStream_t)stream;
     const int B = b->B;
     p.prepared = false;
+    p.norm_pending = false;
     p.desc.assign(B, PostDesc{});
     std::vector<size_t>& label_off = p.h_label_off;
     std::vector<int32_t>& wt_off = p.h_wt_off;
@@ -1450,6 +1453,7 @@
     if (scale01) KCHK(e, minmax_normalize(p.maps, p.d_desc, p.stats, p.B, p.Cmax, p.maxHW, 1, s));
     KCHK(e, background_channel(p.maps, p.d_desc, p.B, p.maxHW, s));
     p.maps_in_2 = false;
+    p.norm_pending = false;
     return PNP_OK;
 }
 
@@ -1457,17 +1461,27 @@
     POST_READY(e);
     auto& p = e->post;
     hipStream_t s = (hipStream_t)stream;
-    KCHK(e, blur_maps(p.maps, p.maps3, p.maps2, p.d_desc, p.d_wts, p.d_wt_off, p.B, p.Kmax, p.maxH, p.maxW, p.max_radius, s));
-    KCHK(e, minmax_normalize(p.maps2, p.d_desc, p.stats, p.B, p.Kmax, p.maxHW, 0, s));
+    KCHK(e, blur_maps(p.maps, p.maps3, p.maps2, p.d_desc, p.d_wts, p.d_wt_off, p.stats, p.B, p.Kmax, p.maxH, p.maxW, p.max_radius, s));
     p.maps_in_2 = true;
+    p.norm_pending = true;
+    p.norm_stream = s;
+    return PNP_OK;
+}
+
+static int post_materialise_norm(pnp_engine* e) {
+    auto& p = e->post;
+    if (!p.norm_pending) return PNP_OK;
+    KCHK(e, normalize_blurred(p.maps2, p.d_desc, p.stats, p.B, p.Kmax, p.maxHW, p.norm_stream));
+    HIPCHK(e, hipStreamSynchronize(p.norm_stream));
+    p.norm_pending = false;
     return PNP_OK;
 }
 
 static int crf_iterate_body(pnp_engine* e, const PostDesc* desc, int kp_max, int32_t iters, float pos_w, float bi_w, hipStream_t s,
-                            const CrfLabelOut& labels);
+                            const CrfLabelOut& labels, bool have_q0);
 
 static int crf_iterate(pnp_engine* e, const PostDesc* desc, int kp_max, int32_t iters, float pos_w, float bi_w, hipStream_t s,
-                       const CrfLabelOut& labels = CrfLabelOut()) {
+                       bool have_q0, const CrfLabelOut& labels = CrfLabelOut()) {
     auto& pf = e->crf_prof;
     const bool timed = pf.on && pf.used < 4096;
     if (timed) {
@@ -1479,7 +1493,7 @@
         }
         (void)hipEventRecord(pf.ev0[pf.used], s);
     }
-    const int r = crf_iterate_body(e, desc, kp_max, iters, pos_w, bi_w, s, labels);
+    const int r = crf_iterate_body(e, desc, kp_max, iters, pos_w, bi_w, s, labels, have_q0);
     if (timed) {
         (void)hipEventRecord(pf.ev1[pf.used], s);
         pf.used++;
@@ -1499,13 +1513,14 @@
 }
 
 static int crf_iterate_body(pnp_engine* e, const PostDesc* desc, int kp_max, int32_t iters, float pos_w, float bi_w, hipStream_t s,
-                            const CrfLabelOut& labels) {
+                            const CrfLabelOut& labels, bool have_q0) {
     auto& p = e->post;
     const int groups = desc == p.d_desc_pair ? 2 : 1;
     for (int c0 = 0; c0 < p.B; c0 += p.chunk) {
         const int n = std::min(p.chunk, p.B - c0);
-        KCHK(e, crf_update(p.lat[0], p.lat[1], desc, c0, n, p.vga, p.va, p.norm[0], p.norm[1], p.unary, p.Q, pos_w, bi_w, 0,
-                           p.maxHW, kp_max, groups, s));
+        if (!have_q0)
+            KCHK(e, crf_update(p.lat[0], p.lat[1], desc, c0, n, p.vga, p.va, p.norm[0], p.norm[1], p.unary, p.Q, pos_w, bi_w, 0,
+                               p.maxHW, kp_max, groups, s));
         for (int it = 0; it < iters; it++) {
             const float *rg = nullptr, *rb = nullptr;
             KCHK(e, crf_filter(p.lat[0], desc, c0, n, p.Q, p.vga, p.vgb, &rg, kp_max, s));
@@ -1526,8 +1541,9 @@
         return fail(e, PNP_ERR_ARG, "lattices are built for sxy=3 / sxy=50, srgb=5 (PnP.py:1036-1041)");
     hipStream_t s = (hipStream_t)stream;
     const float* maps = p.maps_in_2 ? p.maps2 : p.maps;
-    KCHK(e, unary_from_maps(maps, p.d_desc, p.unary, p.B, p.maxHW, p.maxKp, 0, s));
-    return crf_iterate(e, p.d_desc, p.Kpmax, iters, pos_w, bi_w, s);
+    const float* stats = p.maps_in_2 && p.norm_pending ? p.stats : nullptr;
+    KCHK(e, unary_from_maps(maps, p.d_desc, p.unary, p.Q, stats, p.Kmax, p.B, p.maxHW, p.maxKp, 0, s));
+    return crf_iterate(e, p.d_desc, p.Kpmax, iters, pos_w, bi_w, s, unary_writes_q0(p.maxKp));
 }
 
 extern "C" int pnp_remap_hist(pnp_engine* e, int32_t from_crf, uint8_t* d_labels, unsigned long long* d_hist, int32_t n_class,
@@ -1537,7 +1553,8 @@
     if (!d_labels) return fail(e, PNP_ERR_ARG, "d_labels is null");
     hipStream_t s = (hipStream_t)stream;
     const float* src = from_crf ? p.Q : (p.maps_in_2 ? p.maps2 : p.maps);
-    KCHK(e, argmax_remap(src, p.d_desc, p.d_lut, p.lut_stride, d_labels, p.d_label_off, from_crf ? 1 : 0, 0, p.B, p.maxHW, s));
+    const float* stats = !from_crf && p.maps_in_2 && p.norm_pending ? p.stats : nullptr;
+    KCHK(e, argmax_remap(src, p.d_desc, p.d_lut, p.lut_stride, d_labels, p.d_label_off, from_crf ? 1 : 0, 0, stats, p.Kmax, p.B, p.maxHW, s));
     if (d_hist && p.d_gt) KCHK(e, confusion_hist(d_labels, p.d_gt, p.d_desc, p.d_label_off, d_hist, n_class, p.B, p.maxHW, s));
     return PNP_OK;
 }
@@ -1579,7 +1596,7 @@
         if (r) return r;
         r = pnp_blur_minmax(e, stream);
         if (r) return r;
-        KCHK(e, unary_from_maps(p.maps2, p.d_desc_pair, p.unary, p.B, p.maxHW, p.maxKp, grp, s));
+        KCHK(e, unary_from_maps(p.maps2, p.d_desc_pair, p.unary, p.Q, p.norm_pending ? p.stats : nullptr, p.Kmax, p.B, p.maxHW, p.maxKp, grp, s));
     }
     CrfLabelOut lout;
     lout.lab[0] = d_labels_1drop;
@@ -1587,7 +1604,7 @@
     lout.lut = p.d_lut;
     lout.lut_stride = p.lut_stride;
     lout.label_off = p.d_label_off;
-    int r = crf_iterate(e, p.d_desc_pair, p.Kpmax_pair, 10, 7.0f, 10.0f, s, lout);
+    int r = crf_iterate(e, p.d_desc_pair, p.Kpmax_pair, 10, 7.0f, 10.0f, s, unary_writes_q0(p.maxKp), lout);
     if (r) return r;
     for (int grp = 0; grp < 2; grp++) {
         uint8_t* lab = grp == 0 ? d_labels_1drop : d_labels_ndrop;
@@ -1621,7 +1638,10 @@
         const size_t mk = (size_t)p.max_total_pix * p.maxK * 4;
         const size_t mq = (size_t)p.max_total_pix * p.maxKp * 4 * p.groups_cap;
         if (n == "merged") return set(p.merged, (size_t)p.maxB * p.maxK * e->PP * 4);
-        if (n == "maps") return set(p.maps_in_2 ? p.maps2 : p.maps, mk);
+        if (n == "maps") {
+            if (p.maps_in_2 && post_materialise_norm(e) != PNP_OK) return PNP_ERR_HIP;
+            return set(p.maps_in_2 ? p.maps2 : p.maps, mk);
+        }
         if (n == "maps_pre_blur") return set(p.maps, mk);
         if (n == "unary") return set(p.unary, mq);
         if (n == "crf_q") return set(p.Q, mq);
diff --git a/pnp-ovss_amd/csrc/kernels.h b/pnp-ovss_amd/csrc/kernels.h
--- a/pnp-ovss_amd/csrc/kernels.h
+++ b/pnp-ovss_amd/csrc/kernels.h
@@ -90,12 +90,16 @@
                      hipStream_t s);
 int background_channel(float* maps, const PostDesc* desc, int B, int maxHW, hipStream_t s);
 int blur_maps(const float* in, float* tmp, float* out, const PostDesc* desc, const double* wts, const int32_t* wt_off,
-              int B, int Kmax, int maxH, int maxW, int max_radius, hipStream_t s);
+              float* stats, int B, int Kmax, int maxH, int maxW, int max_radius, hipStream_t s);
 int preprocess_images(const uint8_t* rgb, const void* desc, int B, int S, int max_H, const int32_t* coef, uint8_t* tmp,
                       const float* mean3, const float* std3, float* out, hipStream_t s);
-int unary_from_maps(const float* maps, const PostDesc* desc, float* unary, int B, int maxHW, int max_kp, int group, hipStream_t s);
+int normalize_blurred(float* maps, const PostDesc* desc, const float* stats, int B, int Kmax, int maxHW, hipStream_t s);
+bool unary_writes_q0(int max_kp);
+int unary_from_maps(const float* maps, const PostDesc* desc, float* unary, float* Q, const float* stats, int stats_ld, int B,
+                    int maxHW, int max_kp, int group, hipStream_t s);
 int argmax_remap(const float* q, const PostDesc* desc, const int32_t* lut, int lut_stride, uint8_t* labels,
-                 const size_t* label_off, int pixel_major, int group, int B, int maxHW, hipStream_t s);
+                 const size_t* label_off, int pixel_major, int group, const float* stats, int stats_ld, int B, int maxHW,
+                 hipStream_t s);
 int confusion_hist(const uint8_t* labels, const float* gt, const PostDesc* desc, const size_t* label_off,
                    unsigned long long* hist, int n_class, int B, int maxHW, hipStream_t s);
 
diff --git a/pnp-ovss_amd/csrc/pipeline_kernels.hip b/pnp-ovss_amd/csrc/pipeline_kernels.hip
--- a/pnp-ovss_amd/csrc/pipeline_kernels.hip
+++ b/pnp-ovss_amd/csrc/pipeline_kernels.hip
@@ -223,15 +223,34 @@
     }
 }
 
+constexpr uint32_t STAT_NAN = 0xffffffffu;
+__device__ __forceinline__ uint32_t f32_ordered(float v) {
+    const uint32_t u = __float_as_uint(v);
+    return u ^ ((u >> 31) ? 0xffffffffu : 0x80000000u);
+}
+__device__ __forceinline__ float ordered_f32(uint32_t o) { return __uint_as_float(o ^ ((o >> 31) ? 0x80000000u : 0xffffffffu)); }
+__device__ __forceinline__ void ordered_stats_load(const uint32_t* __restrict__ st, float& mn, float& den) {
+    const uint32_t lo = st[0], hi = st[1];
+    float mx;
+    if (hi == STAT_NAN) mn = mx = __uint_as_float(0x7fc00000u);
+    else { mn = ordered_f32(lo); mx = ordered_f32(hi); }
+    den = __fsub_rn(mx, mn);
+}
+
 __global__ void normalize_kernel(float* __restrict__ maps, const PostDesc* __restrict__ desc, const float* __restrict__ stats,
-                                 int Kmax, int first_k_is_class) {
+                                 int Kmax, int first_k_is_class, int ordered) {
     const int b = blockIdx.z, k = blockIdx.y;
     const PostDesc d = desc[b];
     const int kk = first_k_is_class ? k + d.has_bg : k;
     if (kk >= d.K) return;
     if (first_k_is_class && d.C == 1) return;
-    const float mn = stats[((size_t)b * Kmax + kk) * 2], mx = stats[((size_t)b * Kmax + kk) * 2 + 1];
-    const float den = __fsub_rn(mx, mn);
+    float mn, den;
+    if (ordered) {
+        ordered_stats_load(reinterpret_cast<const uint32_t*>(stats) + ((size_t)b * Kmax + kk) * 2, mn, den);
+    } else {
+        mn = stats[((size_t)b * Kmax + kk) * 2];
+        den = __fsub_rn(stats[((size_t)b * Kmax + kk) * 2 + 1], mn);
+    }
     float* m = maps + d.off + (size_t)kk * d.H * d.W;
     const int n = d.H * d.W;
     for (int i = blockIdx.x * blockDim.x + threadIdx.x; i < n; i += gridDim.x * blockDim.x)
@@ -314,7 +333,8 @@
 template <int AXIS>
 __global__ __launch_bounds__(1024) void blur_axis_kernel(const float* __restrict__ in, float* __restrict__ out,
                                                         const PostDesc* __restrict__ desc, const double* __restrict__ wts,
-                                                        const int32_t* __restrict__ wt_off, int max_radius, int NT) {
+                                                        const int32_t* __restrict__ wt_off, int max_radius, int NT,
+                                                        uint32_t* __restrict__ stats) {
     constexpr int axis = AXIS;
     constexpr int TH = 32, TW = 64;
     extern __shared__ __attribute__((aligned(16))) double tile[];
@@ -334,6 +354,13 @@
     const int sub = tid >> 8, t = tid & 255;
     for (int j = tid; j <= radius; j += nthr) wl[j] = w[j];
     const int colsP = (TWe + 2 * radius) | 1;
+    uint32_t* const st = stats + ((size_t)b * gridDim.y + k) * 2;
+    if (AXIS == 0 && blockIdx.x == 0 && tid == 0) {
+        st[0] = 0xffffffffu;
+        st[1] = 0u;
+    }
+    float vmn = INFINITY, vmx = -INFINITY;
+    bool vnan = false;
     for (int tl = blockIdx.x; tl < tiles_x * tiles_y; tl += gridDim.x) {
         const int ty = tl / tiles_x, tx = tl - ty * tiles_x;
         const int y0 = ty * THe, x0 = tx * TWe;
@@ -388,21 +415,32 @@
                 }
             }
         } else {
-            const int total = TH * colsP;
-            constexpr int NF = 16;
-            for (int i0 = tid; i0 < total; i0 += NF * nthr) {
-                float v[NF];
-#pragma unroll
-                for (int u = 0; u < NF; u++) {
-                    const int i = i0 + u * nthr;
-                    const int r = i / colsP, c = i - r * colsP;
-                    const int y = y0 + r < H ? y0 + r : H - 1;
-                    v[u] = i < total ? src[(size_t)y * W + reflect_fast(x0 - radius + c, W)] : 0.f;
-                }
-#pragma unroll
-                for (int u = 0; u < NF; u++) {
-                    const int i = i0 + u * nthr;
-                    if (i < total) xs[i] = v[u];
+            const int nw = nthr >> 6, lane = tid & 63;
+            const int wave = __builtin_amdgcn_readfirstlane(tid >> 6);
+            constexpr int NR = 8;
+            for (int c0 = lane; c0 < colsP; c0 += 128) {
+                const int c1 = c0 + 64;
+                const bool has1 = c1 < colsP;
+                const int xa = reflect_fast(x0 - radius + c0, W);
+                const int xb = has1 ? reflect_fast(x0 - radius + c1, W) : xa;
+                for (int r0 = wave; r0 < TH; r0 += NR * nw) {
+                    float va[NR], vb[NR];
+#pragma unroll
+                    for (int u = 0; u < NR; u++) {
+                        const int r = r0 + nw * u;
+                        const int y = y0 + r < H ? y0 + r : H - 1;
+                        const float* row = src + (size_t)y * W;
+                        va[u] = r < TH ? row[xa] : 0.f;
+                        vb[u] = r < TH ? row[xb] : 0.f;
+                    }
+#pragma unroll
+                    for (int u = 0; u < NR; u++) {
+                        const int r = r0 + nw * u;
+                        if (r < TH) {
+                            xs[r * colsP + c0] = va[u];
+                            if (has1) xs[r * colsP + c1] = vb[u];
+                        }
+                    }
                 }
             }
             __syncthreads();
@@ -421,8 +459,43 @@
                         for (int i = 0; i < 8; i++)
                             if (x0 + cg * 8 + i < W) o[i] = (float)acc[i];
                     }
-                }
-            }
+#pragma unroll
+                    for (int i = 0; i < 8; i++) {
+                        const float v = (float)acc[i];
+                        if (x0 + cg * 8 + i < W) {
+                            vnan |= (v != v);
+                            vmn = fminf(vmn, v);
+                            vmx = fmaxf(vmx, v);
+                        }
+                    }
+                }
+            }
+        }
+    }
+    if constexpr (AXIS == 1) {
+        __syncthreads();
+        float* const smn = xs;
+        float* const smx = xs + 16;
+        int* const snan = reinterpret_cast<int*>(xs + 32);
+        for (int o = 32; o > 0; o >>= 1) {
+            vmn = fminf(vmn, __shfl_xor(vmn, o, 64));
+            vmx = fmaxf(vmx, __shfl_xor(vmx, o, 64));
+        }
+        const int anynan = __any(vnan) ? 1 : 0;
+        if ((tid & 63) == 0) { smn[tid >> 6] = vmn; smx[tid >> 6] = vmx; snan[tid >> 6] = anynan; }
+        __syncthreads();
+        if (tid == 0) {
+            int nn = 0;
+            for (int wv = 0; wv < (nthr >> 6); wv++) {
+                vmn = fminf(vmn, smn[wv]);
+                vmx = fmaxf(vmx, smx[wv]);
+                nn |= snan[wv];
+            }
+            if (vmn <= vmx) {
+                atomicMin(st, f32_ordered(vmn));
+                atomicMax(st + 1, f32_ordered(vmx));
+            }
+            if (nn) atomicMax(st + 1, STAT_NAN);
         }
     }
 }
@@ -489,50 +562,70 @@
 }
 
 __global__ __launch_bounds__(256) void unary_kernel(const float* __restrict__ maps, const PostDesc* __restrict__ desc,
-                                                    float* __restrict__ unary, int group) {
+                                                    float* __restrict__ unary, float* __restrict__ Q,
+                                                    const uint32_t* __restrict__ stats, int stats_ld, int group) {
     extern __shared__ __attribute__((aligned(16))) float utile[];
     const int b = blockIdx.y;
     const PostDesc d = desc[b];
     const int n = d.H * d.W, K = d.K, ldt = K + 1, R4 = d.Kp >> 2;
+    float* const s_mn = utile + 256 * ldt;
+    float* const s_den = s_mn + K;
     const int f0 = group * d.Kg, f1 = f0 + K;
     const int c_lo = f0 >> 2, c_hi = group == d.G - 1 ? R4 : (f1 + 3) >> 2, nc = c_hi - c_lo;
     const float* m = maps + d.off;
     f32x4* u4 = reinterpret_cast<f32x4*>(unary + d.qoff);
+    f32x4* q4 = Q ? reinterpret_cast<f32x4*>(Q + d.qoff) : nullptr;
     const int tid = threadIdx.x;
+    const bool nrm = stats != nullptr;
+    if (nrm) {
+        for (int k = tid; k < K; k += 256) ordered_stats_load(stats + ((size_t)b * stats_ld + k) * 2, s_mn[k], s_den[k]);
+        __syncthreads();
+    }
     for (int p0 = blockIdx.x * 256; p0 < n; p0 += gridDim.x * 256) {
         const int np = (n - p0) < 256 ? (n - p0) : 256;
+        auto write_rows = [&](f32x4* dst4) {
+            for (int item = tid; item < np * nc; item += 256) {
+                const int pl = item / nc, c = c_lo + (item - pl * nc);
+                const float* r = utile + pl * ldt;
+                f32x4* dst = dst4 + (size_t)(p0 + pl) * R4 + c;
+                f32x4 v = {0.f, 0.f, 0.f, 0.f};
+                if (4 * c < f0) v = *dst;
+#pragma unroll
+                for (int j = 0; j < 4; j++) {
+                    const int f = 4 * c + j;
+                    if (f >= f0) v[j] = f < f1 ? r[f - f0] : 0.f;
+                }
+                *dst = v;
+            }
+        };
         if (tid < np) {
             const int i = p0 + tid;
             const float* mi = m + i;
+            float* row = utile + tid * ldt;
             float mx = mi[0];
+            if (nrm) mx = __fdiv_rn(__fsub_rn(mx, s_mn[0]), s_den[0]);
+            row[0] = mx;
             int k = 1;
             for (; k + 8 <= K; k += 8) {
                 float v[8];
 #pragma unroll
                 for (int u = 0; u < 8; u++) v[u] = mi[(size_t)(k + u) * n];
 #pragma unroll
-                for (int u = 0; u < 8; u++)
+                for (int u = 0; u < 8; u++) {
+                    if (nrm) v[u] = __fdiv_rn(__fsub_rn(v[u], s_mn[k + u]), s_den[k + u]);
+                    row[k + u] = v[u];
                     if (v[u] > mx || v[u] != v[u]) mx = v[u];
+                }
             }
             for (; k < K; k++) {
-                const float v = mi[(size_t)k * n];
+                float v = mi[(size_t)k * n];
+                if (nrm) v = __fdiv_rn(__fsub_rn(v, s_mn[k]), s_den[k]);
+                row[k] = v;
                 if (v > mx || v != v) mx = v;
             }
             float s = 0.f;
-            float* row = utile + tid * ldt;
-            for (k = 0; k + 8 <= K; k += 8) {
-                float v[8];
-#pragma unroll
-                for (int u = 0; u < 8; u++) v[u] = mi[(size_t)(k + u) * n];
-#pragma unroll
-                for (int u = 0; u < 8; u++) {
-                    const float e = pnp_expf(__fsub_rn(v[u], mx));
-                    row[k + u] = e;
-                    s = __fadd_rn(s, e);
-                }
-            }
-            for (; k < K; k++) {
-                const float e = pnp_expf(__fsub_rn(mi[(size_t)k * n], mx));
+            for (k = 0; k < K; k++) {
+                const float e = pnp_expf(__fsub_rn(row[k], mx));
                 row[k] = e;
                 s = __fadd_rn(s, e);
             }
@@ -544,26 +637,36 @@
             }
         }
         __syncthreads();
-        for (int item = tid; item < np * nc; item += 256) {
-            const int pl = item / nc, c = c_lo + (item - pl * nc);
-            const float* r = utile + pl * ldt;
-            f32x4* dst = u4 + (size_t)(p0 + pl) * R4 + c;
-            f32x4 v = {0.f, 0.f, 0.f, 0.f};
-            if (4 * c < f0) v = *dst;
-#pragma unroll
-            for (int j = 0; j < 4; j++) {
-                const int f = 4 * c + j;
-                if (f >= f0) v[j] = f < f1 ? r[f - f0] : 0.f;
-            }
-            *dst = v;
-        }
-        __syncthreads();
+        write_rows(u4);
+        __syncthreads();
+        if (q4) {
+            if (tid < np) {
+                float* row = utile + tid * ldt;
+                float mt = -row[0];
+                for (int k = 1; k < K; k++) {
+                    const float v = -row[k];
+                    if (v > mt || v != v) mt = v;
+                }
+                float s = 0.f;
+                for (int k = 0; k < K; k++) {
+                    const float e = pnp_expf(__fsub_rn(-row[k], mt));
+                    row[k] = e;
+                    s = __fadd_rn(s, e);
+                }
+                for (int k = 0; k < K; k++) row[k] = __fdiv_rn(row[k], s);
+            }
+            __syncthreads();
+            write_rows(q4);
+            __syncthreads();
+        }
     }
 }
 
 __global__ __launch_bounds__(256) void unary_wide_kernel(const float* __restrict__ maps, const PostDesc* __restrict__ desc,
-                                                         float* __restrict__ unary, int group) {
+                                                         float* __restrict__ unary, const uint32_t* __restrict__ stats,
+                                                         int stats_ld, int group) {
     __shared__ float tiles[4][64][33];
+    __shared__ float s_mn[256], s_den[256];
     const int b = blockIdx.y;
     const int n = desc[b].H * desc[b].W, K = desc[b].K, R4 = desc[b].Kp >> 2, G = desc[b].G;
     const int f0 = group * desc[b].Kg, f1 = f0 + K;
@@ -572,39 +675,48 @@
     f32x4* u4 = reinterpret_cast<f32x4*>(unary + desc[b].qoff);
     const int wave = threadIdx.x >> 6, lane = threadIdx.x & 63;
     float (*tile)[33] = tiles[wave];
+    const bool nrm = stats != nullptr;
+    if (nrm) {
+        for (int k = threadIdx.x; k < K; k += 256) ordered_stats_load(stats + ((size_t)b * stats_ld + k) * 2, s_mn[k], s_den[k]);
+        __syncthreads();
+    }
+    auto ld = [&](const float* mi, int k) {
+        const float v = mi[(size_t)k * n];
+        return nrm ? __fdiv_rn(__fsub_rn(v, s_mn[k]), s_den[k]) : v;
+    };
     for (int p0 = (blockIdx.x * 4 + wave) * 64; p0 < n; p0 += gridDim.x * 256) {
         const int i = p0 + lane < n ? p0 + lane : n - 1;
         const float* mi = m + i;
-        float mx = mi[0];
+        float mx = ld(mi, 0);
         int k = 1;
         for (; k + 8 <= K; k += 8) {
             float v[8];
 #pragma unroll
-            for (int u = 0; u < 8; u++) v[u] = mi[(size_t)(k + u) * n];
+            for (int u = 0; u < 8; u++) v[u] = ld(mi, k + u);
 #pragma unroll
             for (int u = 0; u < 8; u++)
                 if (v[u] > mx || v[u] != v[u]) mx = v[u];
         }
         for (; k < K; k++) {
-            const float v = mi[(size_t)k * n];
+            const float v = ld(mi, k);
             if (v > mx || v != v) mx = v;
         }
         float s = 0.f;
         for (k = 0; k + 8 <= K; k += 8) {
             float v[8];
 #pragma unroll
-            for (int u = 0; u < 8; u++) v[u] = mi[(size_t)(k + u) * n];
+            for (int u = 0; u < 8; u++) v[u] = ld(mi, k + u);
 #pragma unroll
             for (int u = 0; u < 8; u++) s = __fadd_rn(s, pnp_expf(__fsub_rn(v[u], mx)));
         }
-        for (; k < K; k++) s = __fadd_rn(s, pnp_expf(__fsub_rn(mi[(size_t)k * n], mx)));
+        for (; k < K; k++) s = __fadd_rn(s, pnp_expf(__fsub_rn(ld(mi, k), mx)));
         for (int cb = c_lo; cb < c_hi; cb += 8) {
             const int fb = 4 * cb;
             const int ka = (fb > f0 ? fb : f0) - f0, kb = (fb + 32 < f1 ? fb + 32 : f1) - f0;
             for (k = ka; k < kb; k += 8) {
                 float v[8];
 #pragma unroll
-                for (int u = 0; u < 8; u++) v[u] = k + u < kb ? mi[(size_t)(k + u) * n] : 0.f;
+                for (int u = 0; u < 8; u++) v[u] = k + u < kb ? ld(mi, k + u) : 0.f;
 #pragma unroll
                 for (int u = 0; u < 8; u++) {
                     if (k + u < kb) {
@@ -637,14 +749,21 @@
 
 __global__ void argmax_kernel(const float* __restrict__ q, const PostDesc* __restrict__ desc, const int32_t* __restrict__ lut,
                               int lut_stride, uint8_t* __restrict__ labels, const size_t* __restrict__ label_off,
-                              int pixel_major, int group) {
+                              int pixel_major, int group, const uint32_t* __restrict__ stats, int stats_ld) {
+    __shared__ float s_mn[256], s_den[256];
     const int b = blockIdx.y;
     const PostDesc d = desc[b];
     const int n = d.H * d.W, K = d.K, Kp = d.Kp;
     const float* p = q + (pixel_major ? d.qoff : d.off);
+    const bool nrm = stats != nullptr && !pixel_major;
+    if (nrm) {
+        for (int k = threadIdx.x; k < K; k += blockDim.x) ordered_stats_load(stats + ((size_t)b * stats_ld + k) * 2, s_mn[k], s_den[k]);
+        __syncthreads();
+    }
     for (int i = blockIdx.x * blockDim.x + threadIdx.x; i < n; i += gridDim.x * blockDim.x) {
         int best = 0;
         float bv = pixel_major ? p[(size_t)i * Kp + group * d.Kg] : p[i];
+        if (nrm) bv = __fdiv_rn(__fsub_rn(bv, s_mn[0]), s_den[0]);
         if (pixel_major) {
             const int f0 = group * d.Kg;
             const f32x4* row = reinterpret_cast<const f32x4*>(p + (size_t)i * Kp);
@@ -659,7 +778,8 @@
             }
         } else {
             for (int k = 1; k < K; k++) {
-                const float v = p[(size_t)k * n + i];
+                float v = p[(size_t)k * n + i];
+                if (nrm) v = __fdiv_rn(__fsub_rn(v, s_mn[k]), s_den[k]);
                 if (bv == bv && (v > bv || v != v)) { best = k; bv = v; }
             }
         }
@@ -745,7 +865,13 @@
                      hipStream_t s) {
     hipLaunchKernelGGL(minmax_kernel, dim3(Kmax, B), dim3(256), 0, s, maps, desc, stats, Kmax, class_channels_only);
     const int nb = (maxHW + 255) / 256 < 64 ? (maxHW + 255) / 256 : 64;
-    hipLaunchKernelGGL(normalize_kernel, dim3(nb, Kmax, B), dim3(256), 0, s, maps, desc, stats, Kmax, class_channels_only);
+    hipLaunchKernelGGL(normalize_kernel, dim3(nb, Kmax, B), dim3(256), 0, s, maps, desc, stats, Kmax, class_channels_only, 0);
+    return ok();
+}
+
+int normalize_blurred(float* maps, const PostDesc* desc, const float* stats, int B, int Kmax, int maxHW, hipStream_t s) {
+    const int nb = (maxHW + 255) / 256 < 64 ? (maxHW + 255) / 256 : 64;
+    hipLaunchKernelGGL(normalize_kernel, dim3(nb, Kmax, B), dim3(256), 0, s, maps, desc, stats, Kmax, 0, 1);
     return ok();
 }
 
@@ -756,7 +882,7 @@
 }
 
 int blur_maps(const float* in, float* tmp, float* out, const PostDesc* desc, const double* wts, const int32_t* wt_off,
-              int B, int Kmax, int maxH, int maxW, int max_radius, hipStream_t s) {
+              float* stats, int B, int Kmax, int maxH, int maxW, int max_radius, hipStream_t s) {
     auto lds_for = [&](int n, size_t& l0, size_t& l1) {
         l0 = (size_t)(max_radius + 4) * sizeof(double) + (size_t)(32 * n + 2 * max_radius) * 64 * sizeof(float);
         l1 = (size_t)(max_radius + 4) * sizeof(double) + (size_t)32 * ((64 * n + 2 * max_radius) | 1) * sizeof(float);
@@ -777,31 +903,38 @@
     static std::atomic<uint32_t> opted0{0}, opted1{0};
     if (lds_opt_in(opted0, reinterpret_cast<const void*>(blur_axis_kernel<0>), 160 * 1024) != PNP_OK) return PNP_ERR_HIP;
     if (lds_opt_in(opted1, reinterpret_cast<const void*>(blur_axis_kernel<1>), 160 * 1024) != PNP_OK) return PNP_ERR_HIP;
+    uint32_t* const st = reinterpret_cast<uint32_t*>(stats);
     const int tiles0 = ((maxW + 63) / 64) * ((maxH + 32 * nt0 - 1) / (32 * nt0));
     const int tiles1 = ((maxW + 64 * nt1 - 1) / (64 * nt1)) * ((maxH + 31) / 32);
-    hipLaunchKernelGGL(blur_axis_kernel<0>, dim3(tiles0, Kmax, B), dim3(256 * nt0), lds0, s, in, tmp, desc, wts, wt_off, max_radius, nt0);
-    hipLaunchKernelGGL(blur_axis_kernel<1>, dim3(tiles1, Kmax, B), dim3(256 * nt1), lds1, s, tmp, out, desc, wts, wt_off, max_radius, nt1);
-    return ok();
-}
-
-int unary_from_maps(const float* maps, const PostDesc* desc, float* unary, int B, int maxHW, int max_kp, int group, hipStream_t s) {
+    hipLaunchKernelGGL(blur_axis_kernel<0>, dim3(tiles0, Kmax, B), dim3(256 * nt0), lds0, s, in, tmp, desc, wts, wt_off, max_radius, nt0, st);
+    hipLaunchKernelGGL(blur_axis_kernel<1>, dim3(tiles1, Kmax, B), dim3(256 * nt1), lds1, s, tmp, out, desc, wts, wt_off, max_radius, nt1, st);
+    return ok();
+}
+
+bool unary_writes_q0(int max_kp) { return max_kp < 32; }
+
+int unary_from_maps(const float* maps, const PostDesc* desc, float* unary, float* Q, const float* stats, int stats_ld, int B,
+                    int maxHW, int max_kp, int group, hipStream_t s) {
+    const uint32_t* st = reinterpret_cast<const uint32_t*>(stats);
     const int nb = (maxHW + 255) / 256 < 256 ? (maxHW + 255) / 256 : 256;
-    const size_t smem = (size_t)256 * (max_kp + 1) * sizeof(float);
+    const size_t smem = ((size_t)256 * (max_kp + 1) + 2 * max_kp) * sizeof(float);
     static std::atomic<uint32_t> opted{0};
     if (lds_opt_in(opted, reinterpret_cast<const void*>(unary_kernel), 160 * 1024) != PNP_OK) return PNP_ERR_HIP;
     if (max_kp >= 32) {
         const int nbw = (maxHW + 255) / 256 < 2048 ? (maxHW + 255) / 256 : 2048;
-        hipLaunchKernelGGL(unary_wide_kernel, dim3(nbw, B), dim3(256), 0, s, maps, desc, unary, group);
+        hipLaunchKernelGGL(unary_wide_kernel, dim3(nbw, B), dim3(256), 0, s, maps, desc, unary, st, stats_ld, group);
         return ok();
     }
-    hipLaunchKernelGGL(unary_kernel, dim3(nb, B), dim3(256), smem, s, maps, desc, unary, group);
+    hipLaunchKernelGGL(unary_kernel, dim3(nb, B), dim3(256), smem, s, maps, desc, unary, Q, st, stats_ld, group);
     return ok();
 }
 
 int argmax_remap(const float* q, const PostDesc* desc, const int32_t* lut, int lut_stride, uint8_t* labels,
-                 const size_t* label_off, int pixel_major, int group, int B, int maxHW, hipStream_t s) {
+                 const size_t* label_off, int pixel_major, int group, const float* stats, int stats_ld, int B, int maxHW,
+                 hipStream_t s) {
     const int nb = (maxHW + 255) / 256 < 256 ? (maxHW + 255) / 256 : 256;
-    hipLaunchKernelGGL(argmax_kernel, dim3(nb, B), dim3(256), 0, s, q, desc, lut, lut_stride, labels, label_off, pixel_major, group);
+    hipLaunchKernelGGL(argmax_kernel, dim3(nb, B), dim3(256), 0, s, q, desc, lut, lut_stride, labels, label_off, pixel_major, group,
+                       reinterpret_cast<const uint32_t*>(stats), stats_ld);
     return ok();
 }
 
```

Result: no change. 219.8, median of 6 (+0.5%).
